# JakeKurtz/MC-Path-Tracer

Hardware: AMD Instinct MI355X
Metric: Mray/s (extend+shade) at 1080p x256spp depth5; fraction of HBM roofline (higher is better)
Workload: dtype f32

## Files before the change

include/mcpt.h:

```cpp
#ifndef MCPT_H
#define MCPT_H
#include <stdint.h>

#ifdef __cplusplus
extern "C" {
#endif

#define MCPT_ABI_VERSION 1

enum {
    MCPT_OK = 0,
    MCPT_E_INVALID = -1,
    MCPT_E_HIP = -2,
    MCPT_E_IO = -3,
    MCPT_E_NOMEM = -4,
    MCPT_E_NODEVICE = -5
};

typedef struct mcpt_config {
    uint64_t seed;
    int32_t spp;
    int32_t max_depth;
    int32_t rr_depth;
    int32_t tile_w;
// ... 71 lines not shown
    float *Ld;
    float *light_o, *light_d, *bvis_o, *bvis_d;
    uint8_t *queued;
} mcpt_path_view;

typedef struct mcpt_soa_view {
    const float *ray_o;
    const float *ray_d;
    float *hit_pos_t;
    float *hit_nrm_mat;
    int32_t *hit_tri;
    uint8_t *visible;
    uint32_t *steps;
    mcpt_path_view *paths;
} mcpt_soa_view;

typedef struct mcpt_ctx mcpt_ctx;
typedef struct mcpt_scene mcpt_scene;

int mcpt_create(int device, const mcpt_config *cfg, mcpt_ctx **out);
void mcpt_destroy(mcpt_ctx *ctx);
const char *mcpt_last_error(const mcpt_ctx *ctx);
int mcpt_scene_upload(mcpt_ctx *ctx, const mcpt_scene_desc *desc);
#define MCPT_GPU_BVH_LBVH 0
#define MCPT_GPU_BVH_PLOC 1
int mcpt_scene_upload_gpu_bvh(mcpt_ctx *ctx, const mcpt_scene_desc *desc);
int mcpt_set_gpu_bvh_builder(mcpt_ctx *ctx, int32_t builder);
int mcpt_camera_set(mcpt_ctx *ctx, const mcpt_camera *cam);
int mcpt_film_resize(mcpt_ctx *ctx, uint32_t w, uint32_t h, uint32_t tile_w, uint32_t tile_h);
int mcpt_film_clear(mcpt_ctx *ctx);
int mcpt_set_path_slots(mcpt_ctx *ctx, uint32_t slots);
int mcpt_set_trace_partitions(mcpt_ctx *ctx, uint32_t nparts);
int mcpt_set_work_counters(mcpt_ctx *ctx, int32_t on);
int mcpt_set_skip_discarded(mcpt_ctx *ctx, int32_t on);
int mcpt_set_tiles(mcpt_ctx *ctx, const uint32_t *tile_xy, uint32_t ntiles);
int mcpt_set_compact_paths(mcpt_ctx *ctx, int32_t on);
int mcpt_wavefront_step(mcpt_ctx *ctx, uint32_t tile_x, uint32_t tile_y, mcpt_stage_stats *st);
int mcpt_iterate(mcpt_ctx *ctx, uint32_t iterations, mcpt_stage_stats *st);
int mcpt_render(mcpt_ctx *ctx, mcpt_stage_stats *st);
int mcpt_stage_run(mcpt_ctx *ctx, int stage, const mcpt_soa_view *in, mcpt_soa_view *out, uint32_t n);
int mcpt_film_read(mcpt_ctx *ctx, float *Ld_rgb, uint32_t *samples);
int mcpt_film_read_device(mcpt_ctx *ctx, void *d_Ld_rgb, void *d_samples);
int mcpt_film_pack_tiles(mcpt_ctx *ctx, void *d_out, uint32_t *npix);
int mcpt_film_unpack_tiles(mcpt_ctx *ctx, const void *d_in, const uint32_t *tile_xy, uint32_t ntiles);
int mcpt_film_tonemap_rgba8(mcpt_ctx *ctx, float exposure, uint8_t *out);
int mcpt_film_size(const mcpt_ctx *ctx, uint32_t *w, uint32_t *h);
int mcpt_gather(mcpt_ctx *const *ctxs, int32_t n, int32_t root);
int mcpt_film_write_png(mcpt_ctx *ctx, float exposure, const char *path);
int mcpt_film_write_pfm(mcpt_ctx *ctx, const char *path);
int mcpt_image_write_png(const char *path, uint32_t w, uint32_t h, const uint8_t *rgba8);
int mcpt_image_write_pfm(const char *path, uint32_t w, uint32_t h, const float *rgb);
int mcpt_guides_render(mcpt_ctx *ctx, uint32_t nsamples);
int mcpt_guides_read(mcpt_ctx *ctx, float *albedo_rgb, float *normal_xyz, float *depth, uint32_t *count);
typedef struct mcpt_denoise_params {
    int32_t passes;
    float sigma_color;
    float sigma_normal, sigma_albedo, sigma_depth;
} mcpt_denoise_params;
int mcpt_denoise_default_params(mcpt_denoise_params *p);
int mcpt_denoise_run(mcpt_ctx *ctx, uint32_t w, uint32_t h, const float *rgb, const uint32_t *samples,
                     const float *albedo, const float *normal, const float *depth, const mcpt_denoise_params *p,
                     float *out_rgb);
int mcpt_film_denoise(mcpt_ctx *ctx, const mcpt_denoise_params *p);
int mcpt_denoised_read(mcpt_ctx *ctx, float *rgb);
int mcpt_denoised_read_device(mcpt_ctx *ctx, void *d_rgb);
int mcpt_denoised_tonemap_rgba8(mcpt_ctx *ctx, float exposure, uint8_t *out);
int mcpt_denoised_write_png(mcpt_ctx *ctx, float exposure, const char *path);
int mcpt_debug_denoise_ms(const mcpt_ctx *ctx, float *out10);
typedef struct mcpt_denoise_guided_params {
    int32_t passes;
    float sigma_lum;
    float lum_eps;
    float sigma_color;
    float sigma_normal, sigma_albedo, sigma_depth;
} mcpt_denoise_guided_params;
int mcpt_denoise_guided_default_params(mcpt_denoise_guided_params *p);
int mcpt_denoise_guided_run(mcpt_ctx *ctx, uint32_t w, uint32_t h, const float *rgb, const uint32_t *samples,
                            const float *variance, const float *albedo, const float *normal, const float *depth,
                            const mcpt_denoise_guided_params *p, float *out_rgb, float *out_variance);
int mcpt_film_denoise_guided(mcpt_ctx *ctx, const mcpt_denoise_guided_params *p);
int mcpt_denoised_variance_read(mcpt_ctx *ctx, float *var);
int mcpt_set_sample_budget(mcpt_ctx *ctx, const uint32_t *budget);
int mcpt_sample_budget_read(mcpt_ctx *ctx, uint32_t *out);
int mcpt_set_spp(mcpt_ctx *ctx, int32_t spp);
int mcpt_film_error(mcpt_ctx *ctx);
int mcpt_film_error_read(mcpt_ctx *ctx, float *out4);
int mcpt_error_run(mcpt_ctx *ctx, uint32_t w, uint32_t h, uint32_t slots, const float *Ld_slots,
                   const uint32_t *samples_slots, float *out4);
int mcpt_debug_film_read_slot(mcpt_ctx *ctx, uint32_t slot, float *Ld_rgb, uint32_t *samples);
typedef struct mcpt_sample_budget_params {
    float target_rel_err;
    float lum_floor;
    uint32_t min_spp, max_spp;
} mcpt_sample_budget_params;
int mcpt_sample_budget_default_params(mcpt_sample_budget_params *p);
int mcpt_budget_from_error(mcpt_ctx *ctx, const mcpt_sample_budget_params *p, uint64_t *out3);
int64_t mcpt_debug_adaptive_bytes(const mcpt_ctx *ctx);
int mcpt_debug_adaptive_ms(const mcpt_ctx *ctx, float *out2);
int mcpt_set_seed(mcpt_ctx *ctx, uint64_t seed);
int mcpt_camera_view_proj(const mcpt_camera *cam, float *out16);
typedef struct mcpt_temporal_params {
    float pos_tol;
    float nrm_tol;
    float max_history;
    float alpha_min;
} mcpt_temporal_params;
int mcpt_temporal_default_params(mcpt_temporal_params *p);
int mcpt_film_temporal(mcpt_ctx *ctx, const mcpt_temporal_params *p);
int mcpt_temporal_reset(mcpt_ctx *ctx);
int mcpt_temporal_read(mcpt_ctx *ctx, float *rgb, float *nsamples, float *variance, float *position);
int mcpt_temporal_denoise(mcpt_ctx *ctx, const mcpt_denoise_guided_params *p);
int mcpt_temporal_run(mcpt_ctx *ctx, uint32_t w, uint32_t h, const float *rgb, const uint32_t *samples,
                      const float *variance, const float *position, const float *normal, const float *depth,
                      const float *hcol, const float *hpos, const float *hnrm, const float *vp_prev16,
                      const mcpt_temporal_params *p, float *out_col, float *out_vl, float *out_hcol, float *out_hpos,
                      float *out_hnrm);
int64_t mcpt_debug_temporal_bytes(const mcpt_ctx *ctx);
int mcpt_debug_temporal_ms(const mcpt_ctx *ctx, float *out1);
typedef struct mcpt_variance_params {
    int32_t radius;
    float sigma_normal, sigma_albedo, sigma_depth;
    float min_neff;
} mcpt_variance_params;
int mcpt_variance_default_params(mcpt_variance_params *p);
int mcpt_variance_run(mcpt_ctx *ctx, uint32_t w, uint32_t h, const float *rgb, const uint32_t *samples,
                      const float *variance, const float *albedo, const float *normal, const float *depth,
                      const mcpt_variance_params *p, float *out_variance);
int mcpt_set_variance_fill(mcpt_ctx *ctx, const mcpt_variance_params *p);
int mcpt_debug_variance_ms(const mcpt_ctx *ctx, float *out1);
int mcpt_sync(mcpt_ctx *ctx);
int mcpt_device_name(mcpt_ctx *ctx, char *buf, int32_t len);
int mcpt_debug_queue_rays(mcpt_ctx *ctx, int which, float *ray_o, float *ray_d, uint32_t *n_inout);
float mcpt_debug_last_stage_ms(const mcpt_ctx *ctx);
int mcpt_debug_tiny_lds_stack(mcpt_ctx *ctx, int32_t on);
float mcpt_debug_last_build_ms(const mcpt_ctx *ctx);
float mcpt_debug_last_env_build_ms(const mcpt_ctx *ctx);
int mcpt_debug_env_tables(mcpt_ctx *ctx, float *marginal_y, float *conds_y, float *pdf, int32_t *flags);
int mcpt_debug_node_layout(const mcpt_ctx *ctx);
typedef struct mcpt_bvh_info {
    int32_t npairs;
    int32_t root_ref;
    int32_t depth;
    int32_t width;
    int32_t layout;
    int32_t ntri;
    int32_t tri_f4;
    int32_t gpu_built;
    int32_t rounds;
    float root_mn[3], root_mx[3];
    float cull_p;
} mcpt_bvh_info;
int mcpt_debug_bvh_read(mcpt_ctx *ctx, float *nodes, float *tris, mcpt_bvh_info *info);
int mcpt_debug_occ_stats(const mcpt_ctx *ctx, uint64_t *resolved, int32_t *enabled);
int mcpt_debug_ray_counts(const mcpt_ctx *ctx, uint64_t *out);
int mcpt_debug_primary_stats(const mcpt_ctx *ctx, double *out4);
int mcpt_debug_discard_stats(const mcpt_ctx *ctx, uint64_t *out4);
int mcpt_debug_trace_profile(mcpt_ctx *ctx, uint64_t *out12, int reset);
int mcpt_debug_shade_sections(mcpt_ctx *ctx, uint64_t *out, int n, int reset);
int mcpt_debug_quot(mcpt_ctx *ctx, const float *a, const float *b, uint32_t n, float *out);
int mcpt_debug_hbm_copy(mcpt_ctx *ctx, uint64_t bytes, uint32_t iters, double *gbps);

mcpt_scene *mcpt_scene_new(void);
void mcpt_scene_free(mcpt_scene *s);
int mcpt_scene_load_glb(mcpt_scene *s, const char *path, const float *xform16);
int mcpt_scene_add_mesh(mcpt_scene *s, int32_t ntri, const float *v0, const float *v1, const float *v2,
                        const float *n0, const float *n1, const float *n2, const float *base_rgb);
int mcpt_scene_set_env_hdr(mcpt_scene *s, const char *path, int32_t mode);
#define MCPT_ENV_DEVICE_TABLES 1
int mcpt_scene_set_env_hdr_ex(mcpt_scene *s, const char *path, int32_t mode, uint32_t flags);
int mcpt_scene_set_env_color(mcpt_scene *s, const float *rgb, float ls);
int mcpt_scene_add_dir_light(mcpt_scene *s, const float *dir, const float *rgb, float ls);
int mcpt_scene_transform(mcpt_scene *s, const float *xform16);
int mcpt_scene_make_proxy(mcpt_scene *s, int32_t config_id, const char *asset_dir);
int mcpt_scene_build(mcpt_scene *s, int32_t max_prims_in_node);
#define MCPT_BVH_REFERENCE 0
#define MCPT_BVH_SAH3 1
typedef struct mcpt_bvh_params {
    int32_t builder;
    int32_t max_prims;
    int32_t buckets;
    float trav_cost;
    float isect_cost;
} mcpt_bvh_params;
int mcpt_scene_build_ex(mcpt_scene *s, const mcpt_bvh_params *p);
int mcpt_scene_get_desc(const mcpt_scene *s, mcpt_scene_desc *out);
int mcpt_scene_bvh_depth(const mcpt_scene *s);
int mcpt_camera_make(const mcpt_camera_params *p, mcpt_camera *out);

#ifdef __cplusplus
}
#endif
#endif
```

mc-path-tracer_amd/csrc/kernels.hip:

```cpp
#include <hip/hip_runtime.h>
#include <stdint.h>
#include <stdlib.h>
#include <string.h>
#include <algorithm>

#include "device/mcpt_core.hpp"
#include "device/primary_beam.hpp"
#include "kernels.hpp"

using namespace mcpt;

namespace mcpt_dev {

template <int NQ>
__device__ inline void block_push(const bool (&want)[NQ], uint32_t* const (&counters)[NQ], uint32_t (&slot)[NQ],
                                  uint32_t (&total)[NQ]) {
    __shared__ uint32_t s_wave[NQ][kBlock / 64];
    __shared__ uint32_t s_base[NQ];
    __shared__ uint32_t s_tot[NQ];
    const int lane = threadIdx.x & 63, wave = threadIdx.x >> 6;
    uint32_t prefix[NQ];
#pragma unroll
    for (int q = 0; q < NQ; q++) {
        uint64_t m = __ballot(want[q]);
// ... 135 lines not shown
    float bx0 = nx ? mxx : mnx, bx1 = nx ? mnx : mxx;
    float by0 = ny ? mxy : mny, by1 = ny ? mny : mxy;
    float bz0 = nz ? mxz : mnz, bz1 = nz ? mnz : mxz;
    float tmin = (bx0 - o.x) * inv.x;
    float tmax = (bx1 - o.x) * inv.x;
    float tymin = (by0 - o.y) * inv.y;
    float tymax = (by1 - o.y) * inv.y;
    float tzmin = (bz0 - o.z) * inv.z;
    float tzmax = (bz1 - o.z) * inv.z;
    bool miss = (tmin > tymax) || (tymin > tmax);
    float a = (tymin > tmin) ? tymin : tmin;
    float b = (tymax < tmax) ? tymax : tmax;
    miss = miss || (a > tzmax) || (tzmin > b);
    t0 = (tzmin > a) ? tzmin : a;
    t1 = (tzmax < b) ? tzmax : b;
    return !miss;
}
constexpr float K_INF_F = __builtin_huge_valf();
#ifndef MCPT_OCC_LAYOUT
#define MCPT_OCC_LAYOUT 0
#endif
constexpr int kEnd = -1;

__device__ inline float cull_iota(const DevScene& sc, V3 d, V3 inv) {
    const float ax = __builtin_fabsf(inv.x), ay = __builtin_fabsf(inv.y), az = __builtin_fabsf(inv.z);
    if (!(ax < K_INF_F && ay < K_INF_F && az < K_INF_F)) return -K_INF_F;
    const float n2 = d.x * d.x + d.y * d.y + d.z * d.z;
    if (!sc.cull_ok || !(n2 <= kCullNormMax)) return -3.4028235e38f;
    const float io = __builtin_fmaxf(__builtin_fmaxf(ax, ay), az) * kCullSlackF;
    return io * sc.cull_p <= 1.f ? io : -io;
}
__device__ inline bool keep_box(float t0, float t1, float m, float cut, float& key) {
    key = t0 - __builtin_fabsf(m);
    return !(m >= 0.f && __builtin_fmaf(t1, kCullBehindF, m) < 0.f) && !(key > cut);
}

typedef float f2v __attribute__((ext_vector_type(2)));
__device__ inline void pair_slab(float4 qx, float4 qy, float4 qz, V3 o, V3 inv, float& t0a, float& t1a, float& t0b,
                                 float& t1b) {
    const f2v ox = {o.x, o.x}, oy = {o.y, o.y}, oz = {o.z, o.z};
    const f2v ix = {inv.x, inv.x}, iy = {inv.y, inv.y}, iz = {inv.z, inv.z};
    const f2v ax = (f2v{qx.x, qx.y} - ox) * ix, bx = (f2v{qx.z, qx.w} - ox) * ix;
    const f2v ay = (f2v{qy.x, qy.y} - oy) * iy, by = (f2v{qy.z, qy.w} - oy) * iy;
    const f2v az = (f2v{qz.x, qz.y} - oz) * iz, bz = (f2v{qz.z, qz.w} - oz) * iz;
    t0a = __builtin_fmaxf(__builtin_fmaxf(__builtin_fminf(ax.x, bx.x), __builtin_fminf(ay.x, by.x)),
                          __builtin_fminf(az.x, bz.x));
    t1a = __builtin_fminf(__builtin_fminf(__builtin_fmaxf(ax.x, bx.x), __builtin_fmaxf(ay.x, by.x)),
                          __builtin_fmaxf(az.x, bz.x));
    t0b = __builtin_fmaxf(__builtin_fmaxf(__builtin_fminf(ax.y, bx.y), __builtin_fminf(ay.y, by.y)),
                          __builtin_fminf(az.y, bz.y));
    t1b = __builtin_fminf(__builtin_fminf(__builtin_fmaxf(ax.y, bx.y), __builtin_fmaxf(ay.y, by.y)),
                          __builtin_fmaxf(az.y, bz.y));
}

__device__ inline void quad_axis(const float4& mn, const float4& mx, float o, float inv, float (&lo)[4],
                                 float (&hi)[4], bool first) {
    const f2v oo = {o, o}, ii = {inv, inv};
    const f2v a0 = (f2v{mn.x, mn.y} - oo) * ii, a1 = (f2v{mn.z, mn.w} - oo) * ii;
    const f2v b0 = (f2v{mx.x, mx.y} - oo) * ii, b1 = (f2v{mx.z, mx.w} - oo) * ii;
    const float l[4] = {__builtin_fminf(a0.x, b0.x), __builtin_fminf(a0.y, b0.y), __builtin_fminf(a1.x, b1.x),
                        __builtin_fminf(a1.y, b1.y)};
    const float h[4] = {__builtin_fmaxf(a0.x, b0.x), __builtin_fmaxf(a0.y, b0.y), __builtin_fmaxf(a1.x, b1.x),
                        __builtin_fmaxf(a1.y, b1.y)};
#pragma unroll
    for (int k = 0; k < 4; k++) {
        lo[k] = first ? l[k] : __builtin_fmaxf(lo[k], l[k]);
        hi[k] = first ? h[k] : __builtin_fminf(hi[k], h[k]);
    }
}

__device__ inline f2v pk_slab(f2v q, f2v p) {
    f2v r;
    __asm__("v_pk_add_f32 %0, %1, %2 op_sel_hi:[1,0] neg_lo:[0,1] neg_hi:[0,1]\n\t"
            "v_pk_mul_f32 %0, %0, %2 op_sel:[0,1] op_sel_hi:[1,1]"
            : "=&v"(r)
            : "v"(q), "v"(p));
    return r;
}
__device__ inline void box_t(float ax, float bx, float ay, float by, float az, float bz, float& t0, float& t1) {
    float m0, m1, m2, n0, n1, n2;
    __asm__("v_min_f32 %2, %8, %9\n\t"
            "v_min_f32 %3, %10, %11\n\t"
            "v_min_f32 %4, %12, %13\n\t"
            "v_max_f32 %5, %8, %9\n\t"
            "v_max_f32 %6, %10, %11\n\t"
            "v_max_f32 %7, %12, %13\n\t"
            "v_max3_f32 %0, %2, %3, %4\n\t"
            "v_min3_f32 %1, %5, %6, %7"
            : "=v"(t0), "=v"(t1), "=&v"(m0), "=&v"(m1), "=&v"(m2), "=&v"(n0), "=&v"(n1), "=&v"(n2)
            : "v"(ax), "v"(bx), "v"(ay), "v"(by), "v"(az), "v"(bz));
}
__device__ inline void pair_slab2(float4 qx, float4 qy, float4 qz, f2v px, f2v py, f2v pz, float& t0a, float& t1a,
                                  float& t0b, float& t1b) {
    const f2v ax = pk_slab(f2v{qx.x, qx.y}, px), bx = pk_slab(f2v{qx.z, qx.w}, px);
    const f2v ay = pk_slab(f2v{qy.x, qy.y}, py), by = pk_slab(f2v{qy.z, qy.w}, py);
    const f2v az = pk_slab(f2v{qz.x, qz.y}, pz), bz = pk_slab(f2v{qz.z, qz.w}, pz);
    box_t(ax.x, bx.x, ay.x, by.x, az.x, bz.x, t0a, t1a);
    box_t(ax.y, bx.y, ay.y, by.y, az.y, bz.y, t0b, t1b);
}
__device__ inline float vmin(float a, float b) {
    float r;
    __asm__("v_min_f32 %0, %1, %2" : "=v"(r) : "v"(a), "v"(b));
    return r;
}
__device__ inline float vmax(float a, float b) {
    float r;
    __asm__("v_max_f32 %0, %1, %2" : "=v"(r) : "v"(a), "v"(b));
    return r;
}
__device__ inline void quad_axis2(const float4& mn, const float4& mx, f2v p, float (&lo)[4], float (&hi)[4], bool first) {
    const f2v a0 = pk_slab(f2v{mn.x, mn.y}, p), a1 = pk_slab(f2v{mn.z, mn.w}, p);
    const f2v b0 = pk_slab(f2v{mx.x, mx.y}, p), b1 = pk_slab(f2v{mx.z, mx.w}, p);
    const float l[4] = {vmin(a0.x, b0.x), vmin(a0.y, b0.y), vmin(a1.x, b1.x), vmin(a1.y, b1.y)};
    const float h[4] = {vmax(a0.x, b0.x), vmax(a0.y, b0.y), vmax(a1.x, b1.x), vmax(a1.y, b1.y)};
#pragma unroll
    for (int k = 0; k < 4; k++) {
        lo[k] = first ? l[k] : vmax(lo[k], l[k]);
        hi[k] = first ? h[k] : vmin(hi[k], h[k]);
    }
}

__device__ inline bool ray_misses_scene(const DevScene& sc, V3 o, V3 d) {
    if (!(d.x == d.x && d.y == d.y && d.z == d.z) || (d.x == 0.f && d.y == 0.f && d.z == 0.f)) return true;
    if (o.x >= sc.root_mn[0] && o.x <= sc.root_mx[0] && o.y >= sc.root_mn[1] && o.y <= sc.root_mx[1] &&
        o.z >= sc.root_mn[2] && o.z <= sc.root_mx[2])
        return false;
    const V3 inv = v3(1.f / d.x, 1.f / d.y, 1.f / d.z);
    const float m = sc.root_w * cull_iota(sc, d, inv);
    float t0, t1, key;
    return !(slab(sc.root_mn[0], sc.root_mn[1], sc.root_mn[2], sc.root_mx[0], sc.root_mx[1], sc.root_mx[2], o, inv,
                  inv.x < 0.f, inv.y < 0.f, inv.z < 0.f, t0, t1) &&
             keep_box(t0, t1, m, K_INF_F, key));
}

__device__ inline void hit_record(const DevScene& sc, V3 o, V3 d, int tri, V3& pos, V3& nrm, int& mat, float& t_out) {
    const float4* tp = sc.tri + kTriF4 * tri;
    const float4 w0 = tp[0], w1 = tp[1], w2 = tp[2];
    const float4* sp4 = sc.tri_sh + 3 * tri;
    const float4 s0 = sp4[0], s1 = sp4[1], s2 = sp4[2];
    __asm__ volatile("" ::"v"(w0.x), "v"(w0.y), "v"(w0.z), "v"(w0.w), "v"(w1.x), "v"(w1.y), "v"(w1.z), "v"(w1.w),
                     "v"(w2.x), "v"(s0.x), "v"(s0.y), "v"(s0.z), "v"(s0.w), "v"(s1.x), "v"(s1.y), "v"(s1.z),
                     "v"(s1.w), "v"(s2.x), "v"(s2.y));
    float t, u, v;
    tri_test(o, d, v3(w0.x, w0.y, w0.z), v3(w0.w, w1.x, w1.y), v3(w1.z, w1.w, w2.x), t, u, v);
    const V3 n0 = v3(s0.x, s0.y, s0.z), n1 = v3(s0.w, s1.x, s1.y), n2 = v3(s1.z, s1.w, s2.x);
    const float w = (1.f - u) - v;
    nrm = normalize((n1 * u + n2 * v) + n0 * w);
    nrm = normalize(nrm);
    pos = o + d * t;
    mat = __float_as_int(s2.y);
    t_out = t;
}

__device__ inline uint32_t occ_index(const DevScene& sc, V3 o, V3 d) {
    const float gm = (float)(sc.occ_g - 1), bm = (float)(sc.occ_b - 1), hb = 0.5f * (float)sc.occ_b;
    const uint32_t cx = (uint32_t)__builtin_fminf(__builtin_fmaxf((o.x - sc.root_mn[0]) * sc.occ_inv[0], 0.f), gm);
    const uint32_t cy = (uint32_t)__builtin_fminf(__builtin_fmaxf((o.y - sc.root_mn[1]) * sc.occ_inv[1], 0.f), gm);
    const uint32_t cz = (uint32_t)__builtin_fminf(__builtin_fmaxf((o.z - sc.root_mn[2]) * sc.occ_inv[2], 0.f), gm);
    const float ax = __builtin_fabsf(d.x), ay = __builtin_fabsf(d.y), az = __builtin_fabsf(d.z);
    uint32_t face;
    float u, v, m;
    if (ax >= ay && ax >= az) {
        face = d.x < 0.f ? 1u : 0u; u = d.y; v = d.z; m = ax;
    } else if (ay >= az) {
        face = d.y < 0.f ? 3u : 2u; u = d.x; v = d.z; m = ay;
    } else {
        face = d.z < 0.f ? 5u : 4u; u = d.x; v = d.y; m = az;
    }
    const float r = hb * __builtin_amdgcn_rcpf(m);
    const uint32_t ub = (uint32_t)__builtin_fminf(__builtin_fmaxf(u * r + hb, 0.f), bm);
    const uint32_t vb = (uint32_t)__builtin_fminf(__builtin_fmaxf(v * r + hb, 0.f), bm);
    const uint32_t G = (uint32_t)sc.occ_g, B = (uint32_t)sc.occ_b;
#if MCPT_OCC_LAYOUT == 1
    return (((face * B + ub) * B + vb) * G + cz) * G * G + cy * G + cx;
#else
    return ((((cz * G + cy) * G + cx) * 6u + face) * B + ub) * B + vb;
#endif
}

__device__ inline bool occ_test(V3 o, V3 d, V3 inv, float io, float4 bmn, float4 bmx, float4 r2, float4 r3) {
    const float ax = (bmn.x - o.x) * inv.x, bx = (bmx.x - o.x) * inv.x;
    const float ay = (bmn.y - o.y) * inv.y, by = (bmx.y - o.y) * inv.y;
    const float az = (bmn.z - o.z) * inv.z, bz = (bmx.z - o.z) * inv.z;
    const float t0 = __builtin_fmaxf(__builtin_fmaxf(__builtin_fminf(ax, bx), __builtin_fminf(ay, by)),
                                     __builtin_fminf(az, bz));
    const float t1 = __builtin_fminf(__builtin_fminf(__builtin_fmaxf(ax, bx), __builtin_fmaxf(ay, by)),
                                     __builtin_fmaxf(az, bz));
    float key;
    if (!(t0 <= t1) || !keep_box(t0, t1, bmn.w * io, K_INF_F, key)) return false;
    float th;
    return tri_test_t(o, d, v3(bmx.w, r2.x, r2.y), v3(r2.z, r2.w, r3.x), v3(r3.y, r3.z, r3.w), th) && !(th < 0.f) &&
           th < K_HUGE;
}
__device__ inline uint2 occ_entry(const DevScene& sc, uint32_t cell) {
    const uint2* e = reinterpret_cast<const uint2*>(sc.occ) + cell;
    if constexpr (MCPT_NT & 16) {
        typedef uint32_t u2v_t __attribute__((ext_vector_type(2)));
        const u2v_t v = __builtin_nontemporal_load(reinterpret_cast<const u2v_t*>(e));
        return make_uint2(v.x, v.y);
    } else {
        return *e;
    }
}
__device__ inline bool occ_hit1(const DevScene& sc, V3 o, V3 d, uint2 e) {
    const bool v0 = e.x < sc.ntri, v1 = e.y < sc.ntri;
    if (!(v0 || v1)) return false;
    const float4* p0 = sc.occ_rec + kOccRecF4 * (size_t)(v0 ? e.x : 0u);
    const float4* p1 = sc.occ_rec + kOccRecF4 * (size_t)(v1 ? e.y : 0u);
    const float4 bn0 = p0[0], bx0 = p0[1], r20 = p0[2], r30 = p0[3];
    const float4 bn1 = p1[0], bx1 = p1[1], r21 = p1[2], r31 = p1[3];
    const V3 inv = v3(1.f / d.x, 1.f / d.y, 1.f / d.z);
    if (!(__builtin_fabsf(inv.x) < K_INF_F && __builtin_fabsf(inv.y) < K_INF_F && __builtin_fabsf(inv.z) < K_INF_F))
        return false;
    const float io = cull_iota(sc, d, inv);
    return (v0 && occ_test(o, d, inv, io, bn0, bx0, r20, r30)) || (v1 && occ_test(o, d, inv, io, bn1, bx1, r21, r31));
}

struct MatOut {
    bool want_ext, want_l, want_b, trivial_ext, vis_ray, need_cb;
    bool skip_ext;
    bool doomed_inplace;
    uint32_t trivial_any;
    uint2 el, eb;
    V3 n, wo, wi_b;
    int matid, light_id;
    uint32_t flags;
    float rrz;
};

template <bool FIXED>
__device__ inline MatOut material(const ShadeArgs& a, uint32_t pid, uint32_t pix, uint32_t sidx, uint32_t len,
                                 V3 beta_store, int32_t htri, float4* stage, bool occ_on, bool no_cont) {
    const DevScene& sc = a.scene;
    const uint2 none = make_uint2(kOccEmpty, kOccEmpty);
    MatOut mo{};
    mo.el = mo.eb = none;
    MCPT_MARK("m_hit");
    const Rng r{rng_key(a.seed, pix, sidx), len};
    const V3 ro = xyz(ld_s(a.p.ray_o + pid)), rdir = xyz(ld_s(a.p.ray_d + pid));
    V3 pos, n;
    int mat;
    float t_hit;
    hit_record(sc, ro, rdir, htri, pos, n, mat, t_hit);
    const V3 wo = -rdir;
    const Mat m = load_mat(sc.mats + 8 * mat);
    uint32_t nf = 0;
    V3 rr;
    if (no_cont) {
        rr = v3(0.f, 0.f, 0.f);
        st_s(a.p.beta + pid, f4(beta_store, 0.f));
        mo.skip_ext = true;
    } else {
        MCPT_MARK("m_cont");
        V3 wi_s = brdf_sample_wi<FIXED>(m, n, wo, r, SL_CONT_E0, r(SL_CONT_LOBE) < 0.5f);
        float pdf_s;
        V3 f_s;
        brdf_f_pdf(m, n, wi_s, wo, f_s, pdf_s);
        if ((f_s.x == 0.f && f_s.y == 0.f && f_s.z == 0.f) || pdf_s == 0.f) nf |= F_FZERO;
        rr = f_s / pdf_s;
        const V3 new_o = pos + n * 0.001f;
        st_s(a.p.beta + pid, f4(beta_store, rr.x));
        bool doomed = false;
        if (FIXED || !a.skip) {
            doomed = len + 1u > (uint32_t)a.max_depth;
            if (!doomed && len + 1u > (uint32_t)a.rr_depth) {
                const Rng r1{r.key, len + 1u};
                float q;
                doomed = rr_terminates(r1, FIXED ? (beta_store * rr).y : beta_store.y, q);
            }
        }
        if (doomed && a.skip) {
            mo.skip_ext = true;
        } else {
            st_s(a.p.ray_o + pid, f4(new_o, 0.f));
            st_s(a.p.ray_d + pid, f4(wi_s, 0.f));
            mo.want_ext = true;
            if (ray_misses_scene(sc, new_o, wi_s)) {
                a.p.hit_tri[pid] = -1;
                mo.want_ext = false;
                mo.trivial_ext = true;
                mo.doomed_inplace = doomed;
            }
        }
    }
    MCPT_MARK("m_light");
    int l_id = (int)(r(SL_LIGHT) * (float)(sc.nlights - 0) + (float)0);
    const int light_id = (l_id == sc.nlights) ? 0 : l_id;
    const bool delta = light_id > 0;
    const float sel = FIXED ? 1.f / (float)sc.nlights : 1.f;
    {
        V3 ldir, Li_l;
        float pdfl_x;
        const float4* lt = sc.env.ltab[FIXED ? 1 : 0];
        if (light_id == 0 && lt) {
            int cx, cy;
            env_cell<FIXED>(sc.env, r, cx, cy);
            const float4 t0 = lt[(int64_t)cy * (sc.env.w + 1) + cx + 1];
            const float2 rs = sc.env.lrow[FIXED ? 1 : 0][cy], cs = sc.env.lcol[FIXED ? 1 : 0][cx + 1];
            ldir = v3(cs.y * rs.x, rs.y, cs.x * rs.x);
            pdfl_x = t0.w;
            Li_l = xyz(t0);
        } else {
            if (light_id == 0) ldir = env_dir<FIXED>(sc.env, r);
            else ldir = ld3(sc.dirs + 7 * (light_id - 1), 0);
            light_L_pdf<FIXED>(sc, light_id, ldir, Li_l, pdfl_x);
        }
        V3 f_l;
        float pdf_bl;
        brdf_f_pdf(m, n, ldir, wo, f_l, pdf_bl);
        if (FIXED) pdfl_x = pdfl_x * sel;
        float pdfb_y = !delta ? pdf_bl : (FIXED ? 0.f : 1.f);
        float wL = power_heuristic(pdfl_x, pdfb_y);
        V3 cL = ((f_l * Li_l) * wL) / pdfl_x;
        if (wL > 0.f && pdfl_x > 0.f) nf |= F_CONDL;
        st_s(a.p.nee0 + pid, f4(cL, rr.y));
        const V3 so_l = pos + n * 0.01f;
        if (ray_misses_scene(sc, so_l, ldir)) {
            a.p.vis[2 * pid] = 1;
            mo.trivial_any++;
        } else {
            stage[0 * kBlock + threadIdx.x] = f4(so_l, __uint_as_float(2 * pid));
            stage[1 * kBlock + threadIdx.x] = f4(ldir, 0.f);
            mo.want_l = true;
            if (occ_on) mo.el = occ_entry(sc, occ_index(sc, so_l, ldir));
        }
    }
    MCPT_MARK("m_bsdir");
    if (!delta) {
        const V3 wi_b = brdf_sample_wi<FIXED>(m, n, wo, r, SL_MAT_E0, r(SL_MAT_LOBE) < 0.5f);
        const V3 so_b = pos + wi_b * 0.001f;
        nf |= F_HASVIS;
        mo.vis_ray = true;
        mo.need_cb = true;
        mo.wi_b = wi_b;
        if (ray_misses_scene(sc, so_b, wi_b)) {
            a.p.vis[2 * pid + 1] = 1;
            mo.trivial_any++;
        } else {
            if (occ_on) mo.eb = occ_entry(sc, occ_index(sc, so_b, wi_b));
            stage[2 * kBlock + threadIdx.x] = f4(so_b, __uint_as_float(2 * pid + 1));
            stage[3 * kBlock + threadIdx.x] = f4(wi_b, 0.f);
            mo.want_b = true;
        }
    }
    MCPT_MARK("m_ret");
    mo.n = n;
    mo.wo = wo;
    mo.matid = mat;
    mo.light_id = light_id;
    mo.rrz = rr.z;
    mo.flags = nf | ((len + 1) << F_LEN_SHIFT) | (sidx << F_SIDX_SHIFT);
    return mo;
}
template <bool FIXED>
__device__ inline void material_brdf_terms(const ShadeArgs& a, uint32_t pid, const MatOut& mo) {
    const DevScene& sc = a.scene;
    V3 cB = v3(0.f, 0.f, 0.f);
    uint32_t nf = mo.flags;
    if (mo.need_cb) {
        const Mat m = load_mat(sc.mats + 8 * mo.matid);
        V3 f_b;
        float pdfb_x;
        brdf_f_pdf(m, mo.n, mo.wi_b, mo.wo, f_b, pdfb_x);
        V3 Li_b;
        float pdfl_y;
        light_L_pdf<FIXED>(sc, mo.light_id, mo.wi_b, Li_b, pdfl_y);
        if (FIXED) pdfl_y = pdfl_y * (1.f / (float)sc.nlights);
        float wB = power_heuristic(pdfb_x, pdfl_y);
        cB = ((f_b * Li_b) * wB) / pdfb_x;
        if (wB > 0.f && pdfb_x > 0.f) nf |= F_CONDB;
    }
    st_s(a.p.nee1 + pid, f4(cB, mo.rrz));
    st_s(a.p.flags + pid, nf);
}

#ifndef MCPT_SHADE_WPE
#define MCPT_SHADE_WPE 8
#endif
#if MCPT_SHADE_WPE > 0
#define MCPT_SHADE_ATTR __attribute__((amdgpu_waves_per_eu(MCPT_SHADE_WPE, MCPT_SHADE_WPE)))
#else
#define MCPT_SHADE_ATTR
#endif
#ifndef MCPT_MAT_WPE
#define MCPT_MAT_WPE 4
#endif
#ifdef MCPT_MAT_WPE
#define MCPT_MAT_ATTR __attribute__((amdgpu_waves_per_eu(MCPT_MAT_WPE, MCPT_MAT_WPE)))
#else
#define MCPT_MAT_ATTR
#endif
struct VBlk { int x0, y0; uint32_t loc0, sr, li0, done; };
__device__ inline VBlk vblock_of(const ShadeArgs& a, int vb) {
    const int tile_px = a.tile_w * a.tile_h;
    const int bpt = (tile_px + kBlock - 1) / kBlock;
    const int per_slot = a.ntiles * bpt;
    const int slot = a.slots > 1 ? vb / per_slot : 0;
    const int bs = vb - slot * per_slot;
    const int tile = bs / bpt;
    const int bib = bs - tile * bpt;
    const int li0 = bib * kBlock;
    const int2 t = a.tiles[tile];
    VBlk r;
    if (a.tile_w % kBlock == 0) {
        const int row = li0 / a.tile_w;
        r.x0 = t.x * a.tile_w + (li0 - row * a.tile_w);
        r.y0 = t.y * a.tile_h + row;
    } else {
        r.x0 = t.x * a.tile_w;
        r.y0 = t.y * a.tile_h;
    }
    r.loc0 = a.compact ? (uint32_t)(a.tile_base ? a.tile_base[tile] : tile) * (uint32_t)tile_px + (uint32_t)li0 : 0u;
    r.sr = (uint32_t)slot | ((uint32_t)min(tile_px - li0, kBlock) << 8);
    r.li0 = (uint32_t)li0;
    const uint32_t ntx = (uint32_t)((a.W + a.tile_w - 1) / a.tile_w), nty = (uint32_t)((a.H + a.tile_h - 1) / a.tile_h);
    r.done = (((uint32_t)slot * nty + (uint32_t)t.y) * ntx + (uint32_t)t.x) * (uint32_t)bpt + (uint32_t)bib;
    return r;
}
__device__ inline uint32_t udiv_small(uint32_t n, uint32_t d, float rcp) {
    uint32_t q = (uint32_t)((float)n * rcp);
    if (n - __umul24(q, d) >= d) q++;
    return q;
}

template <bool FIXED, bool MAP>
__device__ __attribute__((always_inline)) inline void shade_vblock(const ShadeArgs& a, int vb, const VBlk& v) {
    const DevScene& sc = a.scene;
    const int slot = (int)(v.sr & 0xffu);
    const int lane = threadIdx.x & 63;
    bool valid = (int)threadIdx.x < (int)(v.sr >> 8);
    uint32_t pid = 0, pix = 0;
    int x = 0, y = 0;
    if (valid) {
        if (a.tile_w % kBlock == 0) {
            x = v.x0 + (int)threadIdx.x;
            y = v.y0;
        } else {
            const int li = (int)v.li0 + (int)threadIdx.x;
            x = v.x0 + li % a.tile_w;
            y = v.y0 + li / a.tile_w;
        }
        valid = x < a.W - 1 && y < a.H - 1;
        pix = (uint32_t)y * (uint32_t)a.W + (uint32_t)x;
        pid = (uint32_t)slot * a.npx + (a.compact ? v.loc0 + threadIdx.x : pix);
    }
    MCPT_MARK("load");
    bool gen_ext = false, gen_trivial = false, gen_prim = false, prim_res = false, cont = false;
    bool no_cont = false;
    bool dd = false, dd_vis = false;
    bool d_logic = false, d_nee = false, d_gen = false;
    (void)d_logic; (void)d_nee; (void)d_gen;
    uint32_t cont_len = 0, cont_sidx = 0;
    int32_t cont_htri = -1;
    V3 beta_store = v3(0.f, 0.f, 0.f);
    bool bg = false;
    V3 bg_film = v3(0.f, 0.f, 0.f), bg_dir = bg_film;
    bool finished = true;
    if (valid) {
        const uint32_t fl = ld_s(a.p.flags + pid);
        const int32_t htri = ld_s(a.p.hit_tri + pid);
        const float4 b4 = ld_s(a.p.beta + ((((fl >> F_LEN_SHIFT) & 0xffu) > 1u) ? pid : 0u));
        const uint32_t len = (fl >> F_LEN_SHIFT) & 0xffu;
        const bool need_rd = len == 1 && htri < 0;
        const bool need_nee = len <= (uint32_t)a.max_depth && len > 1;
        const bool need_ld = !(fl & F_DEAD) && (need_rd || need_nee);
        const V3 ld4 = ld3f4(a.p.Ld + (need_ld ? pid : 0u));
        const V3 rd = ld3f4(a.p.ray_d + (need_rd ? pid : 0u));
        const float4 n0 = ld_s(a.p.nee0 + (need_nee ? pid : 0u)), n1 = ld_s(a.p.nee1 + (need_nee ? pid : 0u));
        const uchar2 vv = reinterpret_cast<const uchar2*>(a.p.vis)[need_nee ? pid : 0u];
        bool dead = (fl & F_DEAD) != 0;
        uint32_t spp;
        if constexpr (MAP) spp = a.budget[pix];
        else spp = (uint32_t)a.spp;
        uint32_t sidx = fl >> F_SIDX_SHIFT;
        uint32_t samples = a.slots > 1 ? udiv_small(sidx - (uint32_t)slot, (uint32_t)a.slots, a.slots_rcp) : sidx;
        if (!dead && sidx < spp) {
            MCPT_MARK("logic");
            d_logic = true;
            d_nee = need_nee;
            const Rng r{rng_key(a.seed, pix, sidx), len};
            const bool found = htri >= 0;
            const V3 B = len == 1 ? v3(1.f, 1.f, 1.f) : xyz(b4);
            V3 film = ld4;
            bool terminate = false;
            beta_store = B;
            if (len == 1) {
                if (found) {
                    film = film + v3(0.f, 0.f, 0.f) * B;
                } else {
                    bg = true;
                    bg_film = film;
                    bg_dir = rd;
// ... 30 lines not shown
                            __float_as_uint(film.y) != __float_as_uint(ld4.y) ||
                            __float_as_uint(film.z) != __float_as_uint(ld4.z)))
                st_s(a.p.Ld + pid, f4(film, 0.f));
            if (a.skip && !terminate) {
                if (len + 1u > (uint32_t)a.max_depth) {
                    int l_id = (int)(r(SL_LIGHT) * (float)(sc.nlights - 0) + (float)0);
                    dd = true;
                    dd_vis = !(((l_id == sc.nlights) ? 0 : l_id) > 0);
                    terminate = true;
                } else if (!FIXED && len + 1u > (uint32_t)a.rr_depth) {
                    const Rng r1{r.key, len + 1u};
                    float q;
                    no_cont = rr_terminates(r1, beta_store.y, q);
                }
            }
            if (terminate) {
                dead = true;
                samples++;
                sidx += (uint32_t)a.slots;
                st_s(a.p.samples + pid, samples);
            } else {
                cont = true;
                cont_len = len;
                cont_sidx = sidx;
                cont_htri = htri;
            }
        }
        uint32_t nflags = fl;
        if (dead) nflags = F_DEAD | (sidx << F_SIDX_SHIFT);
        if (dead && sidx < spp) {
            MCPT_MARK("generate");
            d_gen = true;
            V3 new_o = ld3f4(a.cam_px + pix), new_d;
            if (a.cam.lens_radius > 0.f) {
                const Rng r0{rng_key(a.seed, pix, sidx), 0u};
                gen_ray_lens(a.cam, new_o, r0, new_o, new_d);
            } else {
                new_d = ld3f4(a.cam_dir + pix);
            }
            nflags = (1u << F_LEN_SHIFT) | (sidx << F_SIDX_SHIFT);
            st_s(a.p.ray_o + pid, f4(new_o, 0.f));
            st_s(a.p.ray_d + pid, f4(new_d, 0.f));
            gen_ext = true;
            if (ray_misses_scene(sc, new_o, new_d)) {
                a.p.hit_tri[pid] = -1;
                gen_ext = false;
                gen_trivial = true;
            } else if (a.prim_cnt) {
                const uint32_t pc = a.prim_cnt[pix];
                if (pc != 0u && __builtin_fminf(__builtin_fminf(__builtin_fabsf(new_d.x), __builtin_fabsf(new_d.y)),
                                                __builtin_fabsf(new_d.z)) >= 1e-30f) {
                    gen_ext = false;
                    prim_res = true;
                    if (pc == 1u) {
                        a.p.hit_tri[pid] = -1;
                        gen_trivial = true;
                    } else {
                        gen_prim = true;
                    }
                }
            }
        }
        MCPT_MARK("flags");
        if (!cont && nflags != fl) st_s(a.p.flags + pid, nflags);
        finished = dead && !(sidx < spp);
    }
    SHADE_DIAG(SD_WAVES, true);
    SHADE_DIAG(SD_VALID, valid);
    SHADE_DIAG(SD_LOGIC, d_logic);
    SHADE_DIAG(SD_NEE, d_nee);
    SHADE_DIAG(SD_GEN, d_gen);
    SHADE_DIAG(SD_CONT, cont);
    SHADE_DIAG(SD_BG, bg);
    MCPT_MARK("push");
    const int shard = vb % kShards;
    uint32_t* sc_ctr = a.cnt->shard[shard];
    {
        bool want[3] = {gen_ext, cont, gen_prim};
        uint32_t* ctr[3] = {sc_ctr + C_EXT, sc_ctr + C_MAT, sc_ctr + C_PRIM};
        uint32_t slot[3], total[3];
        block_push<3>(want, ctr, slot, total);
        if (gen_ext) st_q(a.ext_q + shard * a.ext_cap + slot[0], pid);
        if (gen_prim) a.prim_q[shard * a.ext_cap + slot[2]] = make_uint2(pid, pix);
        if (cont) {
            const uint32_t qi = shard * a.ext_cap + slot[1];
            st_s(a.mat_rec + qi, make_uint4(pid, pix, cont_sidx | (no_cont ? kRecNoCont : 0u) | (cont_len << kRecLenShift),
                                            (uint32_t)cont_htri));
            st_s(a.mat_beta + qi, f4(beta_store, 0.f));
        }
    }
    uint32_t n_ext = ((gen_ext || gen_trivial || gen_prim) ? 1u : 0u) + (dd ? 1u : 0u);
    for (int off = 32; off > 0; off >>= 1) n_ext += __shfl_xor(n_ext, off);
    if (lane == 0 && n_ext) atomicAdd(sc_ctr + C_EXT_RAYS, n_ext);
    if (a.skip) {
        const uint32_t n_dd = (uint32_t)__popcll(__ballot(dd)), n_ddv = (uint32_t)__popcll(__ballot(dd_vis));
        if (lane == 0 && n_dd) {
            atomicAdd(sc_ctr + C_ANY_RAYS, n_dd + n_ddv);
            if (n_ddv) atomicAdd(sc_ctr + C_VIS, n_ddv);
            atomicAdd(sc_ctr + C_SKIP_EXT, n_dd);
            atomicAdd(sc_ctr + C_SKIP_ANY, n_dd + n_ddv);
            atomicAdd(sc_ctr + C_SKIP_MAT, n_dd);
        }
    }
    if (a.prim_cnt) {
        const uint32_t n_prim = (uint32_t)__popcll(__ballot(prim_res));
        if (lane == 0 && n_prim) atomicAdd(sc_ctr + C_PRIM_RAYS, n_prim);
    }
    MCPT_MARK("background");
    if (bg) {
        const int nbg = FIXED ? 1 : sc.nlights;
        V3 film = bg_film;
        for (int i = 0; i < nbg; i++) film = film + env_L(sc.env, bg_dir) * v3(1.f, 1.f, 1.f);
        if (__float_as_uint(film.x) != __float_as_uint(bg_film.x) || __float_as_uint(film.y) != __float_as_uint(bg_film.y) ||
            __float_as_uint(film.z) != __float_as_uint(bg_film.z))
            a.p.Ld[pid] = f4(film, 0.f);
    }
    MCPT_MARK("done");
    if (a.blk_done && __syncthreads_and(finished ? 1 : 0) && threadIdx.x == 0) a.blk_done[v.done] = 1;
    MCPT_MARK("end");
}

template <bool FIXED, bool MAP>
__global__ __launch_bounds__(kBlock) MCPT_SHADE_ATTR void k_shade(ShadeArgs a) {
    if (a.cnt->idle) return;
    __shared__ uint64_t s_live[kBlock / 64];
    const uint32_t G = gridDim.x, nvb = a.shade_vblocks;
    const uint32_t mine = (nvb - blockIdx.x + G - 1) / G;
    const uint32_t k = threadIdx.x;
    bool live = false;
    __shared__ VBlk s_vb[kBlock];
    if (k < mine) {
        const VBlk v = vblock_of(a, (int)(blockIdx.x + k * G));
        live = !a.blk_done || a.blk_done[v.done] == 0;
        s_vb[k] = v;
    }
    const uint64_t m = __ballot(live);
    if ((threadIdx.x & 63) == 0) s_live[threadIdx.x >> 6] = m;
    __syncthreads();
    for (uint32_t j = 0; j < mine; j++) {
        if (!((s_live[j >> 6] >> (j & 63)) & 1ull)) continue;
        shade_vblock<FIXED, MAP>(kernarg_fresh<ShadeArgs>(), (int)(blockIdx.x + j * G), s_vb[j]);
    }
}

template <bool FIXED>
__global__ __launch_bounds__(kBlock) MCPT_MAT_ATTR void k_material(ShadeArgs a_kernarg) {
    (void)a_kernarg;
    const ShadeArgs& a = kernarg_fresh<ShadeArgs>();
    if (a.cnt->idle) return;
    const uint32_t shard = blockIdx.x % kShards, w_in = blockIdx.x / kShards, bps = gridDim.x / kShards;
    uint32_t* sc_ctr = a.cnt->shard[shard];
    const uint32_t n = sc_ctr[C_MAT];
    const int lane = threadIdx.x & 63;
    uint32_t n_ext = 0, n_any = 0, n_vis = 0, n_occ = 0, occ_try = 0, n_skip = 0, n_inpl = 0;
    const bool occ_on = a.scene.occ && a.scene.occ_gate[0] == 0 && a.scene.occ_gate[2] != 0;
    __shared__ float4 s_any[4][kBlock];
    for (uint32_t base = w_in * kBlock; base < n; base += bps * kBlock) {
        const ShadeArgs& a = kernarg_fresh<ShadeArgs>();
        const uint32_t i = base + threadIdx.x;
        MatOut mo{};
        uint32_t mpid = 0;
        bool occ_l = false, occ_b = false, try_l = false, try_b = false;
        if (i < n) {
            const uint4 q = ld_s(a.mat_rec + shard * a.ext_cap + i);
            const float4 b4 = ld_s(a.mat_beta + shard * a.ext_cap + i);
            mpid = q.x;
            mo = material<FIXED>(a, mpid, q.y, q.z & (kRecNoCont - 1u), q.z >> kRecLenShift, xyz(b4), (int32_t)q.w,
                                 &s_any[0][0], occ_on, (q.z & kRecNoCont) != 0u);
            MCPT_MARK("m_occ");
            if (occ_on) {
                try_l = mo.want_l;
                try_b = mo.want_b;
                const V3 ol = xyz(s_any[0][threadIdx.x]), dl = xyz(s_any[1][threadIdx.x]);
                const V3 ob = xyz(s_any[2][threadIdx.x]), db = xyz(s_any[3][threadIdx.x]);
                if (mo.want_l) occ_l = occ_hit1(a.scene, ol, dl, mo.el);
                if (mo.want_b) occ_b = occ_hit1(a.scene, ob, db, mo.eb);
                if (occ_l) {
                    a.p.vis[2 * mpid] = 0;
                    mo.want_l = false;
                    mo.trivial_any++;
                }
                if (occ_b) {
                    a.p.vis[2 * mpid + 1] = 0;
                    mo.want_b = false;
                    mo.need_cb = false;
                    mo.trivial_any++;
                }
            }
            MCPT_MARK("m_bterms");
            material_brdf_terms<FIXED>(a, mpid, mo);
        }
        MCPT_MARK("m_push");
        bool want[3] = {mo.want_ext, mo.want_l, mo.want_b};
        uint32_t* ctr[3] = {sc_ctr + C_EXT, sc_ctr + C_ANY, sc_ctr + C_ANY};
        uint32_t slot[3], total[3];
        block_push<3>(want, ctr, slot, total);
        if (mo.want_ext) st_q(a.ext_q + shard * a.ext_cap + slot[0], mpid);
        if (mo.want_l) {
            const uint32_t k = shard * a.any_cap + slot[1];
            if constexpr (MCPT_NT & 8) {
                st_s(a.p.sray_o + k, s_any[0][threadIdx.x]);
                st_s(a.p.sray_d + k, s_any[1][threadIdx.x]);
            } else {
                a.p.sray_o[k] = s_any[0][threadIdx.x];
                a.p.sray_d[k] = s_any[1][threadIdx.x];
            }
        }
        if (mo.want_b) {
            const uint32_t k = shard * a.any_cap + slot[2];
            if constexpr (MCPT_NT & 8) {
                st_s(a.p.sray_o + k, s_any[2][threadIdx.x]);
                st_s(a.p.sray_d + k, s_any[3][threadIdx.x]);
            } else {
                a.p.sray_o[k] = s_any[2][threadIdx.x];
                a.p.sray_d[k] = s_any[3][threadIdx.x];
            }
        }
        MCPT_MARK("m_count");
        n_occ += (uint32_t)(__popcll(__ballot(occ_l)) + __popcll(__ballot(occ_b)));
        occ_try += (uint32_t)(__popcll(__ballot(try_l)) + __popcll(__ballot(try_b)));
        n_ext += (uint32_t)__popcll(__ballot(mo.want_ext || mo.trivial_ext || mo.skip_ext));
        n_skip += (uint32_t)__popcll(__ballot(mo.skip_ext));
        n_inpl += (uint32_t)__popcll(__ballot(mo.doomed_inplace));
        n_any += (uint32_t)(__popcll(__ballot(mo.want_l)) + __popcll(__ballot(mo.want_b)) +
                            __popcll(__ballot(mo.trivial_any >= 1u)) + __popcll(__ballot(mo.trivial_any >= 2u)));
        n_vis += (uint32_t)__popcll(__ballot(mo.vis_ray));
    }
    if (lane == 0) {
        if (n_ext) atomicAdd(sc_ctr + C_EXT_RAYS, n_ext);
        if (n_any) atomicAdd(sc_ctr + C_ANY_RAYS, n_any);
        if (n_vis) atomicAdd(sc_ctr + C_VIS, n_vis);
        if (n_occ) atomicAdd(sc_ctr + C_OCC, n_occ);
        if (occ_try) atomicAdd(sc_ctr + C_OCC_TRY, occ_try);
        if (n_skip) atomicAdd(sc_ctr + C_SKIP_EXT, n_skip);
        if (n_inpl) atomicAdd(sc_ctr + C_SKIP_INPLACE, n_inpl);
    }
}

__device__ inline uint32_t wave_scan_incl(uint32_t x) {
    x += (uint32_t)__builtin_amdgcn_update_dpp(0, (int)x, 0x111, 0xf, 0xf, false);
    x += (uint32_t)__builtin_amdgcn_update_dpp(0, (int)x, 0x112, 0xf, 0xf, false);
    x += (uint32_t)__builtin_amdgcn_update_dpp(0, (int)x, 0x114, 0xf, 0xf, false);
    x += (uint32_t)__builtin_amdgcn_update_dpp(0, (int)x, 0x118, 0xf, 0xf, false);
    x += (uint32_t)__builtin_amdgcn_update_dpp(0, (int)x, 0x142, 0xa, 0xf, false);
    x += (uint32_t)__builtin_amdgcn_update_dpp(0, (int)x, 0x143, 0xc, 0xf, false);
    return x;
}

__device__ inline void wave_stats(uint32_t* stats, int lane, uint32_t nodes, uint32_t tests, uint32_t hits) {
    if (!stats) return;
    for (int off = 32; off > 0; off >>= 1) {
        nodes += __shfl_xor(nodes, off);
        tests += __shfl_xor(tests, off);
        hits += __shfl_xor(hits, off);
    }
    if (lane == 0) {
        uint32_t* st = stats + (blockIdx.x % kShards) * C_WORDS;
        atomicAdd(st + 0, nodes);
        atomicAdd(st + 1, tests);
        atomicAdd(st + 2, hits);
    }
}

#ifndef MCPT_NODE_STEPS
#define MCPT_NODE_STEPS 4
#endif
#ifndef MCPT_TRI_SHARE
#define MCPT_TRI_SHARE 0
#endif
constexpr int kShareMaxStack = 8;
constexpr int kNodeSteps = MCPT_NODE_STEPS;
#ifndef MCPT_GRAB_MAX
#define MCPT_GRAB_MAX 0
#endif
constexpr int kGrabMax = MCPT_GRAB_MAX;
#ifndef MCPT_ANY_FIRST
#define MCPT_ANY_FIRST 0
#endif
constexpr bool kAnyFirst = MCPT_ANY_FIRST != 0;
#ifndef MCPT_NODE_MIN_LANES2
#define MCPT_NODE_MIN_LANES2 32
#endif
#ifndef MCPT_NODE_MIN_LANES2_DEEP
#define MCPT_NODE_MIN_LANES2_DEEP 0
#endif
#ifndef MCPT_NODE_MIN_LANES4
#define MCPT_NODE_MIN_LANES4 24
#endif

#ifndef MCPT_TRACE_WPE
#define MCPT_TRACE_WPE 7
#endif
#ifndef MCPT_TRACE_WPE_DEEP
#define MCPT_TRACE_WPE_DEEP 7
#endif
#ifndef MCPT_TRACE_WPE4
#define MCPT_TRACE_WPE4 6
#endif
#define MCPT_TRACE_WPE_OF(kW, kS) \
    ((kW) == 4 ? MCPT_TRACE_WPE4 : ((kS) > ::mcpt_dev::kLdsStack ? MCPT_TRACE_WPE_DEEP : MCPT_TRACE_WPE))
#define MCPT_TRACE_ATTR \
    __attribute__((amdgpu_waves_per_eu(MCPT_TRACE_WPE_OF(kW, kLdsStack), MCPT_TRACE_WPE_OF(kW, kLdsStack))))
template <int kW, int kLdsStack, bool kCount>
__global__ __launch_bounds__(kTraceBlock) MCPT_TRACE_ATTR void k_trace(TraceArgs a) {
    if (a.idle && *a.idle) return;
    constexpr bool kShare = MCPT_TRI_SHARE != 0 && kLdsStack <= kShareMaxStack;
    __shared__ int2 stk[kLdsStack][kTraceBlock];
    __shared__ uint64_t s_key[kShare ? kTraceBlock : 1];
    const int lane = threadIdx.x;
    const uint32_t nsh = (uint32_t)a.nshards, nparts = a.nparts;
    uint32_t home = 0;
    if (nparts > 1) {
        uint32_t xcc;
        __asm__ volatile("s_getreg_b32 %0, hwreg(HW_REG_XCC_ID)" : "=s"(xcc));
        const uint32_t nd = a.ndies >= 1 && a.ndies <= nparts && nparts % a.ndies == 0 ? a.ndies : nparts;
        home = (xcc & 15u) % nd + nd * ((blockIdx.x / nd) % (nparts / nd));
    }
    __shared__ uint32_t s_tot[kMaxParts];
    if (lane < kMaxParts) s_tot[lane] = 0;
    __syncthreads();
    if ((uint32_t)lane < nsh) {
        uint32_t n = 0;
#pragma unroll
        for (int k = 0; k < 2; k++) {
            const TraceSet& ts = a.set[k];
            n += ts.count_ptr ? ts.count_ptr[lane * C_WORDS] : (lane == 0 ? ts.count : 0u);
        }
        if (n) atomicAdd(&s_tot[lane % nparts], n);
    }
    __syncthreads();
    __shared__ uint32_t s_pre[129];
    uint32_t part = home, spart = 0, T = 0;
    uint32_t* grab = a.grab;
    bool more = false;
    auto enter = [&](uint32_t p) {
        part = __builtin_amdgcn_readfirstlane(p);
        spart = __builtin_amdgcn_readfirstlane(nsh > part ? (nsh - part + nparts - 1) / nparts : 0u);
        uint32_t base = 0;
#pragma unroll 1
        for (uint32_t h = 0; h < 2; h++) {
            const uint32_t e = (uint32_t)lane + 64u * h;
            const bool k1 = kAnyFirst ? e < spart : e >= spart;
            const uint32_t j = e >= spart ? e - spart : e;
            uint32_t ne = 0;
            if (e < 2 * spart) {
                const TraceSet& ts = k1 ? a.set[1] : a.set[0];
                const uint32_t sh = part + j * nparts;
                ne = ts.count_ptr ? ts.count_ptr[sh * C_WORDS] : (sh == 0 ? ts.count : 0u);
            }
            const uint32_t inc = wave_scan_incl(ne);
            s_pre[e] = base + inc - ne;
            base += __builtin_amdgcn_readlane(inc, 63);
        }
        T = __builtin_amdgcn_readfirstlane(base);
        if (lane == 0) s_pre[128] = T;
        __syncthreads();
        grab = a.grab + part * C_WORDS;
        more = T > 0;
    };
    enter(home);
    const DevScene& sc = a.scene;
    const bool occ_rec = sc.occ && sc.occ_gate[0] <= 1u;

    uint32_t tot_n = 0, tot_t = 0, tot_h = 0, tot_n1 = 0, tot_t1 = 0, tot_h1 = 0;
    uint32_t ph[kPhaseWords] = {};
    uint64_t drained = 0;
    for (;;) {
    uint32_t buf_lo = 0, buf_hi = 0, last_p = 0;
    bool act = false;
    uint32_t rid = 0;
    f2v px = {0.f, 0.f}, py = px, pz = px;
    V3 d = v3(0.f, 0.f, 0.f);
#define RAY_O v3(px.x, py.x, pz.x)
#define RAY_INV v3(px.y, py.y, pz.y)
    int ref = kEnd, leaf = kEnd, sp = 0, tri = -1;
    float best = K_HUGE, cut = K_HUGE, io = K_INF_F;
    uint32_t bsid = 0;
    int2 spill[kMaxStack - kLdsStack];
    auto pop = [&]() -> int {
        while (sp > 0) {
            sp--;
            int2 e;
            if (sp < kLdsStack) {
                e = stk[sp][lane];
            } else {
                e = spill[sp - kLdsStack];
// ... 529 lines not shown
__global__ void k_cam_table(mcpt::CamView cam, int W, int H, float4* px, float4* dir) {
    const uint32_t i = blockIdx.x * blockDim.x + threadIdx.x;
    if (i >= (uint32_t)W * (uint32_t)H) return;
    const int x = (int)(i % (uint32_t)W), y = (int)(i / (uint32_t)W);
    V3 o, d;
    gen_ray_pixel(cam, W, H, x, y, o, d);
    px[i] = f4(cam.lens_radius > 0.f ? gen_ray_focal(cam, o, d) : o, 0.f);
    dir[i] = f4(d, 0.f);
}
void launch_cam_table(const mcpt::CamView& cam, int W, int H, float4* px, float4* dir, hipStream_t s) {
    const uint32_t n = (uint32_t)W * (uint32_t)H;
    if (n) hipLaunchKernelGGL(k_cam_table, dim3((n + 255) / 256), dim3(256), 0, s, cam, W, H, px, dir);
}

__global__ void k_env_pack(float4* tex, const float* __restrict__ pdf, size_t n) {
    const size_t i = (size_t)blockIdx.x * blockDim.x + threadIdx.x;
    if (i < n) tex[i].w = pdf[i];
}
void launch_env_pack(float4* tex, const float* pdf, size_t n, hipStream_t s) {
    if (n) hipLaunchKernelGGL(k_env_pack, dim3((unsigned)((n + 255) / 256)), dim3(256), 0, s, tex, pdf, n);
}

template <bool FIXED>
__global__ void k_env_table(EnvView e, float4* out, float2* row, float2* col) {
    const int i = blockIdx.x * blockDim.x + threadIdx.x;
    const int W1 = e.w + 1;
    if (i < e.h) {
        float st, ct;
        spherical_theta(env_cell_v<FIXED>(e, i), st, ct);
        row[i] = make_float2(st, ct);
    }
    if (i < W1) {
        const int x = i - 1;
        float sp, cp;
        spherical_phi(env_cell_u<FIXED>(e, FIXED && x < 0 ? 0 : x), sp, cp);
        col[i] = make_float2(sp, cp);
    }
    if (i >= W1 * e.h) return;
    const int y = i / W1, x = i - y * W1 - 1;
    const V3 d = env_cell_dir<FIXED>(e, FIXED && x < 0 ? 0 : x, y);
    V3 L;
    float pdf;
    env_L_pdf<FIXED>(e, d, L, pdf);
    out[i] = make_float4(L.x, L.y, L.z, pdf);
}
void launch_env_table(const EnvView& e, bool fixed_mode, float4* out, float2* row, float2* col, hipStream_t s) {
    const int n = (e.w + 1) * e.h;
    if (fixed_mode) hipLaunchKernelGGL(k_env_table<true>, dim3((n + 255) / 256), dim3(256), 0, s, e, out, row, col);
    else hipLaunchKernelGGL(k_env_table<false>, dim3((n + 255) / 256), dim3(256), 0, s, e, out, row, col);
}

__global__ void k_hit_record(HitRecordArgs a) {
    const uint32_t i = blockIdx.x * blockDim.x + threadIdx.x;
    if (i >= a.n) return;
    const int tri = a.tri[i];
    if (tri < 0) {
        a.hit_p[i] = make_float4(0.f, 0.f, 0.f, K_HUGE);
        a.hit_n[i] = make_float4(0.f, 0.f, 0.f, __int_as_float(-1));
        a.scene_tri[i] = -1;
        return;
    }
    a.scene_tri[i] = __float_as_int(a.scene.tri[kTriF4 * tri + 2].y);
    V3 pos, nrm;
    int mat;
    float t;
    hit_record(a.scene, xyz(a.ro[i]), xyz(a.rd[i]), tri, pos, nrm, mat, t);
    a.hit_p[i] = make_float4(pos.x, pos.y, pos.z, t);
    a.hit_n[i] = make_float4(nrm.x, nrm.y, nrm.z, __int_as_float(mat));
}

__global__ void k_clear(ClearArgs a) {
    const uint32_t i = blockIdx.x * blockDim.x + threadIdx.x;
    if (i >= a.n) return;
    a.flags[i] = F_DEAD | ((i / a.npx) << F_SIDX_SHIFT);
    a.samples[i] = 0;
    a.Ld[i] = make_float4(0.f, 0.f, 0.f, 0.f);
}

__global__ void k_resolve(ResolveArgs a) {
    const uint32_t i = blockIdx.x * blockDim.x + threadIdx.x;
    if (i >= a.n) return;
    uint32_t o = i;
    if (a.tiles) {
        const uint32_t tpx = (uint32_t)(a.tile_w * a.tile_h), ti = i / tpx, li = i - ti * tpx;
        const int2 t = a.tiles[ti];
        const uint32_t x = (uint32_t)t.x * a.tile_w + li % (uint32_t)a.tile_w, y = (uint32_t)t.y * a.tile_h + li / (uint32_t)a.tile_w;
        if (x >= (uint32_t)a.W || y >= (uint32_t)a.H) return;
        o = y * (uint32_t)a.W + x;
    }
    float4 L = a.Ld[i];
    uint32_t n = a.samples[i];
    for (int k = 1; k < a.slots; k++) {
        const float4 l = a.Ld[(size_t)k * a.n + i];
        L = make_float4(L.x + l.x, L.y + l.y, L.z + l.z, 0.f);
        n += a.samples[(size_t)k * a.n + i];
    }
    a.out_Ld[o] = L;
    a.out_samples[o] = n;
}

__global__ void k_tonemap(TonemapArgs a) {
    const uint32_t i = blockIdx.x * blockDim.x + threadIdx.x;
    if (i >= a.n) return;
    float4 L = a.Ld[i];
    float s = (float)a.samples[i];
    V3 c = v3(L.x / s, L.y / s, L.z / s);
    c = c * a.exposure;
    c = v3(c.x / (c.x + 1.0f), c.y / (c.y + 1.0f), c.z / (c.z + 1.0f));
    float cc[3] = {255 * c.x, 255 * c.y, 255 * c.z};
    uchar4 o;
    unsigned char b[3];
    for (int k = 0; k < 3; k++) {
        float v = cc[k];
        b[k] = (v == v && v >= 0.f && v < 4294967296.f) ? (unsigned char)(unsigned int)v : (unsigned char)0;
    }
    o.x = b[0]; o.y = b[1]; o.z = b[2]; o.w = 255;
    a.out[i] = o;
}

#ifndef MCPT_OCC_BACKOFF0
#define MCPT_OCC_BACKOFF0 15
#endif
__global__ void k_accumulate(CounterBlock* c, uint32_t nparts, uint32_t* occ_gate) {
    if (c->idle) return;
    const int t = threadIdx.x;
    uint32_t v[C_STATS + 6];
#pragma unroll
    for (int k = 0; k < C_STATS + 6; k++) {
        v[k] = c->shard[t][k];
        c->shard[t][k] = 0;
    }
    c->last_ext_shard[t] = v[C_EXT];
    __shared__ uint32_t s_part[kMaxParts];
    if (t < kMaxParts) s_part[t] = 0;
    __syncthreads();
    atomicAdd(&s_part[t % nparts], v[C_EXT] + v[C_ANY]);
    __syncthreads();
    uint32_t g = 0;
    if (t < kMaxParts) g = c->grab[t][0];
    const bool short_part = t < (int)nparts && g < s_part[t];
#pragma unroll
    for (int k = 0; k < C_STATS + 6; k++)
        for (int off = 32; off > 0; off >>= 1) v[k] += __shfl_xor(v[k], off);
    if (__ballot(short_part) != 0 && t == 0) c->trace_short += 1;
    if (t < kMaxParts) c->grab[t][0] = 0;
    uint32_t phw[kPhaseWords];
#pragma unroll
    for (int k = 0; k < kPhaseWords; k++) {
        phw[k] = c->shard[t][C_PH + k];
        c->shard[t][C_PH + k] = 0;
        for (int off = 32; off > 0; off >>= 1) phw[k] += __shfl_xor(phw[k], off);
    }
    uint32_t er = c->shard[t][C_EXT_RAYS], ar = c->shard[t][C_ANY_RAYS], oc = c->shard[t][C_OCC],
             ot = c->shard[t][C_OCC_TRY], pr = c->shard[t][C_PRIM_RAYS];
    const int skw[4] = {C_SKIP_EXT, C_SKIP_ANY, C_SKIP_MAT, C_SKIP_INPLACE};
    uint32_t sk[4];
#pragma unroll
    for (int k = 0; k < 4; k++) {
        sk[k] = c->shard[t][skw[k]];
        if (sk[k]) c->shard[t][skw[k]] = 0;
        for (int off = 32; off > 0; off >>= 1) sk[k] += __shfl_xor(sk[k], off);
    }
    c->shard[t][C_PRIM] = 0;
    c->shard[t][C_PRIM_RAYS] = 0;
    c->shard[t][C_EXT_RAYS] = 0;
    c->shard[t][C_ANY_RAYS] = 0;
    c->shard[t][C_MAT] = 0;
    c->shard[t][C_OCC] = 0;
    c->shard[t][C_OCC_TRY] = 0;
    for (int off = 32; off > 0; off >>= 1) {
        er += __shfl_xor(er, off);
        ar += __shfl_xor(ar, off);
        oc += __shfl_xor(oc, off);
        ot += __shfl_xor(ot, off);
        pr += __shfl_xor(pr, off);
    }
    if (t == 0) {
        c->tot_ext += er;
        c->tot_prim += pr;
        for (int k = 0; k < 4; k++) c->tot_skip[k] += sk[k];
        c->tot_any += ar;
        c->tot_occ += oc;
        if (occ_gate) {
            if (occ_gate[0]) {
                occ_gate[0]--;
            } else if (!occ_gate[2]) {
                if (v[C_ANY]) occ_gate[2] = 1;
            } else if (ot >= 4096u) {
                if ((unsigned long long)oc * kOccMinRate < ot) {
                    occ_gate[1] = occ_gate[1] ? min(2u * occ_gate[1] + 1u, 255u) : (uint32_t)MCPT_OCC_BACKOFF0;
                    occ_gate[0] = occ_gate[1];
                } else {
                    occ_gate[1] = 0;
                }
            }
        }
        c->tot_vis += v[C_VIS];
        c->tot_ext_q += v[C_EXT];
        c->tot_any_q += v[C_ANY];
        c->last_ext = v[C_EXT];
        c->last_live = er;
        if (er == 0) c->idle = 1;
        for (int k = 0; k < 6; k++) c->tot_stats[k] += v[C_STATS + k];
        for (int k = 0; k < kPhaseWords; k++) c->tot_phase[k] += phw[k];
    }
}

__global__ void k_pack(PackArgs a) {
    const int tile_px = a.tile_w * a.tile_h;
    const uint32_t i = blockIdx.x * blockDim.x + threadIdx.x;
    if (i >= (uint32_t)(a.ntiles * tile_px)) return;
    const int tile = i / tile_px, li = i % tile_px;
    int2 t = a.tiles[tile];
    int x = t.x * a.tile_w + li % a.tile_w, y = t.y * a.tile_h + li / a.tile_w;
    float4 o = make_float4(0.f, 0.f, 0.f, __uint_as_float(0u));
    if (x < a.W && y < a.H) {
        uint32_t pid = (uint32_t)y * a.W + x;
        float4 L = a.Ld[pid];
        o = make_float4(L.x, L.y, L.z, __uint_as_float(a.samples[pid]));
    }
    a.out[i] = o;
}

__global__ void k_unpack(UnpackArgs a) {
    const int tile_px = a.tile_w * a.tile_h;
    const uint32_t i = blockIdx.x * blockDim.x + threadIdx.x;
    if (i >= (uint32_t)(a.ntiles * tile_px)) return;
    const int tile = i / tile_px, li = i % tile_px;
    const int2 t = a.tiles[tile];
    const int x = t.x * a.tile_w + li % a.tile_w, y = t.y * a.tile_h + li / a.tile_w;
    if (x >= a.W || y >= a.H) return;
    const uint32_t pid = (uint32_t)y * a.W + x;
    const float4 v = a.in[i];
    a.Ld[pid] = make_float4(v.x, v.y, v.z, 0.f);
    a.samples[pid] = __float_as_uint(v.w);
}

static uint32_t env_u32(const char* name, int def, int lo, int hi) {
    const char* e = getenv(name);
    int v = e ? atoi(e) : def;
    return (uint32_t)std::min(hi, std::max(lo, v));
}
int launch_geometry(int dev, LaunchGeom& g) {
    int cus = 0, nx = 1, per_cu = 0, mat0 = 0, mat1 = 0, sh0 = 0;
    if (hipDeviceGetAttribute(&cus, hipDeviceAttributeMultiprocessorCount, dev) != hipSuccess) return -1;
    if (hipDeviceGetAttribute(&nx, hipDeviceAttributeNumberOfXccs, dev) != hipSuccess) nx = 1;
    int occ[2][2] = {};
    if (hipOccupancyMaxActiveBlocksPerMultiprocessor(&occ[0][0], k_trace<2, kLdsStack, false>, kTraceBlock, 0) != hipSuccess ||
        hipOccupancyMaxActiveBlocksPerMultiprocessor(&occ[0][1], k_trace<2, kLdsStackDeep, false>, kTraceBlock, 0) != hipSuccess ||
        hipOccupancyMaxActiveBlocksPerMultiprocessor(&occ[1][0], k_trace<4, kLdsStack, false>, kTraceBlock, 0) != hipSuccess ||
        hipOccupancyMaxActiveBlocksPerMultiprocessor(&occ[1][1], k_trace<4, kLdsStackDeep, false>, kTraceBlock, 0) != hipSuccess ||
        hipOccupancyMaxActiveBlocksPerMultiprocessor(&mat0, k_material<false>, kBlock, 0) != hipSuccess ||
        hipOccupancyMaxActiveBlocksPerMultiprocessor(&mat1, k_material<true>, kBlock, 0) != hipSuccess ||
        hipOccupancyMaxActiveBlocksPerMultiprocessor(&sh0, k_shade<false, false>, kBlock, 0) != hipSuccess)
        return -1;
    if (cus <= 0) cus = 256;
    per_cu = 32;
    if (const char* e = getenv("MCPT_TRACE_WAVES")) per_cu = atoi(e);
    if (per_cu <= 0) per_cu = 16;
    for (int w = 0; w < 2; w++)
        for (int k = 0; k < 2; k++) g.trace_waves[w][k] = (uint32_t)(cus * std::max(1, std::min(per_cu, occ[w][k])));
    g.ndies = (uint32_t)std::max(1, nx);
    g.trace_parts = env_u32("MCPT_TRACE_PARTS", std::min(kMaxParts, 2 * std::max(1, nx)), 1, kMaxParts);
    if (const char* e = getenv("MCPT_MAT_BLOCKS_PER_CU")) {
        const int m = atoi(e);
        if (m > 0) { mat0 = std::min(mat0, m); mat1 = std::min(mat1, m); }
    }
    g.mat_blocks[0] = (uint32_t)std::max(1, cus * std::max(1, mat0) / kShards) * (uint32_t)kShards;
    g.mat_blocks[1] = (uint32_t)std::max(1, cus * std::max(1, mat1) / kShards) * (uint32_t)kShards;
    int prim = 0;
    if (hipOccupancyMaxActiveBlocksPerMultiprocessor(&prim, k_primary, kBlock, 0) != hipSuccess) return -1;
    g.prim_blocks = (uint32_t)std::max(1, cus * std::max(1, prim) / kShards) * (uint32_t)kShards;
    g.shade_grid = (uint32_t)std::max(1, cus * std::max(1, sh0)) * env_u32("MCPT_SHADE_GRID", 16, 0, 1024);
    if (getenv("MCPT_SHADE_WGS")) g.shade_grid = env_u32("MCPT_SHADE_WGS", 0, 1, 1 << 30);
    g.refill_min = env_u32("MCPT_REFILL_MIN", 0, 0, 64);
    g.tri_min = env_u32("MCPT_TRI_MIN", 16, 0, 64);
    return 0;
}
static uint32_t shade_grid(uint32_t nblocks, const LaunchGeom& g) {
    uint32_t G = g.shade_grid ? std::min(nblocks, g.shade_grid) : nblocks;
    return std::max(G, (nblocks + kBlock - 1) / kBlock);
}
void launch_shade(const ShadeArgs& args, int nblocks, const LaunchGeom& g, bool fixed_mode, hipStream_t s) {
    ShadeArgs a = args;
    a.shade_vblocks = (uint32_t)nblocks;
    const uint32_t G = shade_grid((uint32_t)nblocks, g);
    if (fixed_mode) {
        if (a.budget) hipLaunchKernelGGL((k_shade<true, true>), dim3(G), dim3(kBlock), 0, s, a);
        else hipLaunchKernelGGL((k_shade<true, false>), dim3(G), dim3(kBlock), 0, s, a);
        hipLaunchKernelGGL(k_material<true>, dim3(g.mat_blocks[1]), dim3(kBlock), 0, s, a);
    } else {
        if (a.budget) hipLaunchKernelGGL((k_shade<false, true>), dim3(G), dim3(kBlock), 0, s, a);
        else hipLaunchKernelGGL((k_shade<false, false>), dim3(G), dim3(kBlock), 0, s, a);
        hipLaunchKernelGGL(k_material<false>, dim3(g.mat_blocks[0]), dim3(kBlock), 0, s, a);
    }
}
void launch_shade_stage(bool material_stage, const ShadeArgs& args, int nblocks, const LaunchGeom& g, bool fixed_mode,
                        hipStream_t s) {
    ShadeArgs a = args;
    a.shade_vblocks = (uint32_t)nblocks;
    if (!material_stage) {
        const uint32_t G = shade_grid((uint32_t)nblocks, g);
        if (fixed_mode) hipLaunchKernelGGL((k_shade<true, false>), dim3(G), dim3(kBlock), 0, s, a);
        else hipLaunchKernelGGL((k_shade<false, false>), dim3(G), dim3(kBlock), 0, s, a);
    } else {
        if (fixed_mode) hipLaunchKernelGGL(k_material<true>, dim3(g.mat_blocks[1]), dim3(kBlock), 0, s, a);
        else hipLaunchKernelGGL(k_material<false>, dim3(g.mat_blocks[0]), dim3(kBlock), 0, s, a);
    }
}
void launch_trace(const TraceArgs& args, const LaunchGeom& g, hipStream_t s) {
    if (args.nshards <= 0) return;
    TraceArgs a = args;
    a.tri_min = g.tri_min;
    a.nparts = std::min<uint32_t>(kMaxParts, std::max<uint32_t>(1, g.trace_parts));
    a.ndies = g.ndies;
    const uint32_t nsh = (uint32_t)a.nshards;
    const int w = a.scene.width == 4 ? 1 : 0, k = a.scene.depth > kDeepTree ? 1 : 0;
    static const uint32_t kRefill[2][2] = {{20u, 32u}, {24u, 24u}};
    a.refill_min = g.refill_min ? g.refill_min : kRefill[w][k];
    const uint32_t wps = std::max<uint32_t>(1, g.trace_waves[w][k] / nsh);
    const dim3 grid(wps * nsh), block(kTraceBlock);
    if (a.tiny_stack) {
        if (w == 0) hipLaunchKernelGGL((k_trace<2, kLdsStackTiny, false>), grid, block, 0, s, a);
        else hipLaunchKernelGGL((k_trace<4, kLdsStackTiny, false>), grid, block, 0, s, a);
        return;
    }
    if (a.set[0].stats || a.set[1].stats) {
        if (w == 0 && k == 0) hipLaunchKernelGGL((k_trace<2, kLdsStack, true>), grid, block, 0, s, a);
        else if (w == 0) hipLaunchKernelGGL((k_trace<2, kLdsStackDeep, true>), grid, block, 0, s, a);
        else if (k == 0) hipLaunchKernelGGL((k_trace<4, kLdsStack, true>), grid, block, 0, s, a);
        else hipLaunchKernelGGL((k_trace<4, kLdsStackDeep, true>), grid, block, 0, s, a);
        return;
    }
    if (w == 0 && k == 0) hipLaunchKernelGGL((k_trace<2, kLdsStack, false>), grid, block, 0, s, a);
    else if (w == 0) hipLaunchKernelGGL((k_trace<2, kLdsStackDeep, false>), grid, block, 0, s, a);
    else if (k == 0) hipLaunchKernelGGL((k_trace<4, kLdsStack, false>), grid, block, 0, s, a);
    else hipLaunchKernelGGL((k_trace<4, kLdsStackDeep, false>), grid, block, 0, s, a);
}
__global__ void k_quot(const float* a, const float* b, float* out, uint32_t n) {
    const uint32_t i = blockIdx.x * blockDim.x + threadIdx.x;
    if (i >= n) return;
    float q0, q1, q2;
    quot3(a[i], 1.0f, -a[i], b[i], q0, q1, q2);
    out[i] = q0;
}
void launch_quot(const float* a, const float* b, float* out, uint32_t n, hipStream_t s) {
    if (n) hipLaunchKernelGGL(k_quot, dim3((n + 255) / 256), dim3(256), 0, s, a, b, out, n);
}

__global__ __launch_bounds__(256) void k_copy(const float4* __restrict__ src, float4* __restrict__ dst, size_t n) {
    const size_t i = (size_t)blockIdx.x * blockDim.x + threadIdx.x;
    if (i < n) dst[i] = src[i];
}
void launch_copy(const float4* src, float4* dst, size_t n, hipStream_t s) {
    if (n) hipLaunchKernelGGL(k_copy, dim3((unsigned)((n + 255) / 256)), dim3(256), 0, s, src, dst, n);
}

int wave_times(unsigned long long* out, int n) {
    (void)out;
    (void)n;
    return 0;
}
int trace_profile(unsigned long long* out, int reset) {
    (void)out;
    (void)reset;
    return 0;
}
__global__ void k_occ_records(DevScene sc, uint32_t nnodes, float4* out) {
    const uint32_t i = blockIdx.x * blockDim.x + threadIdx.x;
    auto put = [&](int ref, float mnx, float mny, float mnz, float mxx, float mxy, float mxz, float w) {
        if (ref >= 0 || ref == kEnd) return;
        const uint32_t off = (uint32_t)ref & 0xffffffu, cnt = (((uint32_t)ref >> 24) & 7u) + 1u;
        for (uint32_t k = off; k < off + cnt && k < sc.ntri; k++) {
            const float4* tr = sc.tri + kTriF4 * (size_t)k;
            const float4 a = tr[0], b = tr[1], c = tr[2];
            float4* o = out + kOccRecF4 * (size_t)k;
            o[0] = make_float4(mnx, mny, mnz, w);
            o[1] = make_float4(mxx, mxy, mxz, a.x);
            o[2] = make_float4(a.y, a.z, a.w, b.x);
            o[3] = make_float4(b.y, b.z, b.w, c.x);
        }
    };
    if (i == 0 && sc.root_ref < 0)
        put(sc.root_ref, sc.root_mn[0], sc.root_mn[1], sc.root_mn[2], sc.root_mx[0], sc.root_mx[1], sc.root_mx[2],
            sc.root_w);
    if (i >= nnodes) return;
    if (sc.width == 4) {
        const float4* nd = sc.nodes + 8 * (size_t)i;
        const float4 mnx = nd[0], mxx = nd[1], mny = nd[2], mxy = nd[3], mnz = nd[4], mxz = nd[5], rf = nd[6], wq = nd[7];
        const float* a0 = &mnx.x; const float* a1 = &mxx.x; const float* b0 = &mny.x;
        const float* b1 = &mxy.x; const float* c0 = &mnz.x; const float* c1 = &mxz.x; const float* r = &rf.x;
        const float* w = &wq.x;
        for (int k = 0; k < 4; k++) put(__float_as_int(r[k]), a0[k], b0[k], c0[k], a1[k], b1[k], c1[k], w[k]);
    } else {
        const float4* nd = sc.nodes + 4 * (size_t)i;
        const float4 q0 = nd[0], q1 = nd[1], q2 = nd[2], q3 = nd[3];
        put(__float_as_int(q3.x), q0.x, q1.x, q2.x, q0.z, q1.z, q2.z, q3.z);
        put(__float_as_int(q3.y), q0.y, q1.y, q2.y, q0.w, q1.w, q2.w, q3.w);
    }
}

__global__ void k_cull_tri(const float4* tri, uint32_t ntri, float* tw, uint32_t* pmax, int plane) {
    const uint32_t i = blockIdx.x * blockDim.x + threadIdx.x;
    if (i >= ntri) return;
    const float4* r = tri + kTriF4 * (size_t)i;
    const float4 r0 = r[0], r1 = r[1], r2 = r[2];
    double far;
    tw[i] = cull_to_float_up(cull_tri_margin(v3(r0.w, r1.x, r1.y), v3(r1.z, r1.w, r2.x), &far, plane != 0));
    if (far > 0.0) atomicMax(pmax, __float_as_uint(cull_to_float_up(far)));
}
__global__ void k_cull_pairs(float4* nodes, uint32_t npairs, const float* tw, uint32_t ntri) {
    const uint32_t i = blockIdx.x * blockDim.x + threadIdx.x;
    if (i >= npairs) return;
    const float4 q3 = nodes[4 * (size_t)i + 3];
    float w[2];
#pragma unroll
    for (int k = 0; k < 2; k++) {
        const int ref = __float_as_int(k ? q3.y : q3.x);
        float v = 0.f;
        if (ref >= 0) {
            const float4 c = nodes[4 * (size_t)ref + 3];
            v = __builtin_fmaxf(c.z, c.w);
        } else if (ref != kEnd) {
            const uint32_t off = (uint32_t)ref & 0xffffffu, cnt = (((uint32_t)ref >> 24) & 7u) + 1u;
            for (uint32_t t = off; t < off + cnt && t < ntri; t++) v = __builtin_fmaxf(v, tw[t]);
        }
        w[k] = v;
    }
    nodes[4 * (size_t)i + 3] = make_float4(q3.x, q3.y, w[0], w[1]);
}
__global__ void k_cull_zero(float4* nodes, uint32_t npairs) {
    const uint32_t i = blockIdx.x * blockDim.x + threadIdx.x;
    if (i >= npairs) return;
    float4 q3 = nodes[4 * (size_t)i + 3];
    q3.z = q3.w = 0.f;
    nodes[4 * (size_t)i + 3] = q3;
}
void launch_cull_margins(float4* nodes, uint32_t npairs, const float4* tri, uint32_t ntri, float* tri_w,
                         uint32_t* pmax, int passes, bool plane, hipStream_t s) {
    if (ntri) hipLaunchKernelGGL(k_cull_tri, dim3((ntri + 255) / 256), dim3(256), 0, s, tri, ntri, tri_w, pmax, plane ? 1 : 0);
    if (!npairs) return;
    hipLaunchKernelGGL(k_cull_zero, dim3((npairs + 255) / 256), dim3(256), 0, s, nodes, npairs);
    for (int p = 0; p < passes; p++)
        hipLaunchKernelGGL(k_cull_pairs, dim3((npairs + 255) / 256), dim3(256), 0, s, nodes, npairs, tri_w, ntri);
}
__global__ void k_occ_probes(DevScene sc, float4* ro, float4* rd, uint32_t nkeys) {
    const uint32_t key = blockIdx.x * blockDim.x + threadIdx.x;
    if (key >= nkeys) return;
    const uint32_t G = (uint32_t)sc.occ_g, B = (uint32_t)sc.occ_b;
    uint32_t t = key, cx, cy, cz, face, ub, vb;
#if MCPT_OCC_LAYOUT == 1
    cx = t % G; t /= G; cy = t % G; t /= G; cz = t % G; t /= G; vb = t % B; t /= B; ub = t % B; face = t / B;
#else
    vb = t % B; t /= B; ub = t % B; t /= B; face = t % 6u; t /= 6u; cx = t % G; t /= G; cy = t % G; cz = t / G;
#endif
    const uint32_t c[3] = {cx, cy, cz};
    float o[3];
    for (int k = 0; k < 3; k++)
        o[k] = sc.occ_inv[k] > 0.f ? sc.root_mn[k] + ((float)c[k] + 0.5f) / sc.occ_inv[k] : sc.root_mn[k];
    const float hb = 0.5f * (float)B;
    const float u = ((float)ub + 0.5f) / hb - 1.f, v = ((float)vb + 0.5f) / hb - 1.f;
    const float sg = (face & 1u) ? -1.f : 1.f;
    float d[3];
    if (face < 2u) { d[0] = sg; d[1] = u; d[2] = v; }
    else if (face < 4u) { d[0] = u; d[1] = sg; d[2] = v; }
    else { d[0] = u; d[1] = v; d[2] = sg; }
    const float inv_n = 1.f / __builtin_sqrtf(d[0] * d[0] + d[1] * d[1] + d[2] * d[2]);
    ro[key] = make_float4(o[0], o[1], o[2], 0.f);
    rd[key] = make_float4(d[0] * inv_n, d[1] * inv_n, d[2] * inv_n, 0.f);
}
void launch_occ_probes(const DevScene& sc, float4* ro, float4* rd, uint32_t nkeys, hipStream_t s) {
    if (nkeys == 0) return;
    hipLaunchKernelGGL(k_occ_probes, dim3((nkeys + 255) / 256), dim3(256), 0, s, sc, ro, rd, nkeys);
}
void launch_occ_records(const DevScene& sc, uint32_t nnodes, float4* rec, hipStream_t s) {
    hipLaunchKernelGGL(k_occ_records, dim3(nnodes / 256 + 1), dim3(256), 0, s, sc, nnodes, rec);
}
void launch_clear(const ClearArgs& a, hipStream_t s) {
    if (a.n == 0) return;
    hipLaunchKernelGGL(k_clear, dim3((a.n + 255) / 256), dim3(256), 0, s, a);
}
void launch_hit_record(const HitRecordArgs& a, hipStream_t s) {
    if (a.n == 0) return;
    hipLaunchKernelGGL(k_hit_record, dim3((a.n + 255) / 256), dim3(256), 0, s, a);
}
void launch_resolve(const ResolveArgs& a, hipStream_t s) {
    if (a.n == 0) return;
    hipLaunchKernelGGL(k_resolve, dim3((a.n + 255) / 256), dim3(256), 0, s, a);
}
void launch_tonemap(const TonemapArgs& a, hipStream_t s) {
    if (a.n == 0) return;
    hipLaunchKernelGGL(k_tonemap, dim3((a.n + 255) / 256), dim3(256), 0, s, a);
}
void launch_accumulate(CounterBlock* c, uint32_t nparts, uint32_t* occ_gate, hipStream_t s) {
    hipLaunchKernelGGL(k_accumulate, dim3(1), dim3(kShards), 0, s, c, std::min<uint32_t>(kMaxParts, std::max<uint32_t>(1, nparts)),
                       occ_gate);
}
void launch_unpack(const UnpackArgs& a, hipStream_t s) {
    const uint32_t n = (uint32_t)(a.ntiles * a.tile_w * a.tile_h);
    if (n) hipLaunchKernelGGL(k_unpack, dim3((n + 255) / 256), dim3(256), 0, s, a);
}
void launch_pack(const PackArgs& a, hipStream_t s) {
    uint32_t n = (uint32_t)(a.ntiles * a.tile_w * a.tile_h);
    if (n == 0) return;
    hipLaunchKernelGGL(k_pack, dim3((n + 255) / 256), dim3(256), 0, s, a);
}

}
```

mc-path-tracer_amd/csrc/kernels.hpp:

```cpp
#pragma once
#include <hip/hip_runtime.h>
#include <stdint.h>

#include "device/adaptive.hpp"
#include "device/denoise.hpp"
#include "device/mcpt_core.hpp"
#include "device/temporal.hpp"
#include "device/variance.hpp"

namespace mcpt_dev {

constexpr int kBlock = 256;
constexpr int kTraceBlock = 64;
#ifndef MCPT_LDS_STACK
#define MCPT_LDS_STACK 8
#endif
constexpr int kLdsStack = MCPT_LDS_STACK;
#ifndef MCPT_LDS_STACK_DEEP
#define MCPT_LDS_STACK_DEEP 10
#endif
constexpr int kLdsStackDeep = MCPT_LDS_STACK_DEEP;
constexpr int kLdsStackTiny = 2;
#ifndef MCPT_DEEP_TREE
#define MCPT_DEEP_TREE 20
#endif
constexpr int kDeepTree = MCPT_DEEP_TREE;
constexpr int kMaxStack = 64;

enum : uint32_t {
    F_DEAD = 1u,
    F_LEN_SHIFT = 1,
    F_CONDL = 1u << 9,
    F_CONDB = 1u << 10,
    F_FZERO = 1u << 11,
    F_HASVIS = 1u << 12,
    F_SIDX_SHIFT = 13
};
constexpr uint32_t kMaxSpp = 1u << (32 - F_SIDX_SHIFT);
constexpr int kRecLenShift = 24;
static_assert(kMaxSpp <= (1u << kRecLenShift), "sample index and len share a record word");
constexpr uint32_t kRecNoCont = 1u << 23;
static_assert(kMaxSpp <= kRecNoCont && kRecNoCont < (1u << kRecLenShift), "the mark lies between sample index and len");

__host__ __device__ constexpr int shade_blocks_per_tile(int tile_px, int slots) {
    return (tile_px + kBlock - 1) / kBlock * slots;
}

#ifndef MCPT_TRI_F4
#define MCPT_TRI_F4 3
#endif
constexpr int kTriF4 = MCPT_TRI_F4;

struct DevScene {
    const float4* nodes;
    const float4* tri;
    const float4* tri_sh;
    float root_mn[3], root_mx[3];
    int root_ref;
    int depth;
    int width;
    int nlights;
    const float* mats;
    const float* dirs;
    mcpt::EnvView env;
    uint32_t* occ;
    uint32_t* occ_gate;
    const float4* occ_rec;
    uint32_t ntri;
    int occ_g, occ_b;
    float occ_inv[3];
    float cull_p, root_w;
    int cull_ok;
};
constexpr uint32_t kOccEmpty = 0xffffffffu;
constexpr uint32_t kOccWays = 2;
constexpr uint32_t kOccGateWords = 3;
constexpr uint32_t kOccMinRate = 10;
__host__ __device__ constexpr size_t occ_entries(int g, int b) { return (size_t)g * g * g * 6 * b * b * kOccWays; }

struct DevPaths {
    float4 *ray_o, *ray_d, *sray_o, *sray_d, *beta, *nee0, *nee1, *Ld;
    int32_t* hit_tri;
    uint32_t *flags, *samples;
    uint8_t* vis;
};

constexpr int kShards = 64;
constexpr int kMaxParts = kShards;
enum : int { C_EXT = 0, C_ANY = 1, C_VIS = 2, C_STATS = 3, C_EXT_RAYS = 9, C_ANY_RAYS = 10, C_MAT = 11, C_OCC = 12,
              C_OCC_TRY = 13, C_PH = 14, C_SKIP_INPLACE = 25, C_PRIM = 26, C_PRIM_RAYS = 27, C_SKIP_EXT = 28,
              C_SKIP_ANY = 29, C_SKIP_MAT = 30, C_WORDS = 32 };
enum : int {
    PH_TRIPS = 0,
    PH_REFILLS = 1,
    PH_REFILL_LANES = 2,
    PH_NODE_ITERS = 3,
    PH_TRI_PHASES = 4,
    PH_TRI_LANES = 5,
    PH_TRIP_NODE = 6,
    PH_TRIP_LEAF = 7,
    PH_TRIP_IDLE = 8,
    PH_FINISH_TRIPS = 9,
    PH_POP_ITERS = 10,
    kPhaseWords = 11
};
struct CounterBlock {
    uint32_t shard[kShards][C_WORDS];
    uint32_t last_ext, last_live;
    uint32_t trace_short;
    uint32_t idle;
    uint32_t pad[28];
    uint32_t last_ext_shard[kShards];
    uint32_t grab[kMaxParts][C_WORDS];
    unsigned long long tot_ext, tot_any, tot_vis, tot_occ;
    unsigned long long tot_stats[6];
    unsigned long long tot_ext_q, tot_any_q;
    unsigned long long tot_phase[kPhaseWords];
    unsigned long long tot_prim;
    unsigned long long tot_skip[4];
};
static_assert(C_PH + kPhaseWords <= C_SKIP_INPLACE, "counter words overlap");

constexpr char kPrimaryHitsEnv[] = "MCPT_PRIMARY_HITS";
constexpr int kPrimLine = 16;
constexpr int kPrimK = kPrimLine;

struct ShadeArgs {
    DevScene scene;
    mcpt::CamView cam;
    DevPaths p;
    const int2* tiles;
    int ntiles, tile_w, tile_h, W, H;
    int spp, max_depth, rr_depth;
    int slots;
    float slots_rcp;
    uint32_t npx;
    int compact;
    const int* tile_base;
    uint64_t seed;
    uint32_t *ext_q, *any_q;
    uint4* mat_rec;
    float4* mat_beta;
    uint32_t ext_cap, any_cap;
    CounterBlock* cnt;
    uint8_t* blk_done;
    uint32_t shade_vblocks;
    const float4* cam_px;
    const float4* cam_dir;
    const uint8_t* prim_cnt;
    const uint32_t* prim_list;
    uint2* prim_q;
    int skip;
    const uint32_t* budget;
};
struct PrimaryBuildArgs {
    DevScene scene;
    mcpt::CamView cam;
    int W, H;
    const float4 *cam_px, *cam_dir;
    uint8_t* cnt;
    uint32_t* list;
    uint32_t* stats;
};

struct TraceSet {
    const float4 *ro, *rd;
    const uint32_t* queue;
    const uint32_t* count_ptr;
    uint32_t count;
    uint32_t shard_cap;
    uint32_t* stats;
    uint32_t* ray_steps;
    int prefiltered;
    int ray_at_slot;
};
struct TraceArgs {
    DevScene scene;
    TraceSet set[2];
    int nshards;
    int32_t* hit_tri;
    uint8_t* vis;
    uint32_t refill_min;
    uint32_t tri_min;
    uint32_t nparts;
    uint32_t ndies;
    uint32_t* grab;
    const uint32_t* idle;
    int tiny_stack;
    uint32_t* phase;
};

struct HitRecordArgs { DevScene scene; const float4 *ro, *rd; const int32_t* tri; float4 *hit_p, *hit_n; int32_t* scene_tri; uint32_t n; };
struct ClearArgs { uint32_t* flags; uint32_t* samples; float4* Ld; uint32_t n, npx; };
struct ResolveArgs {
    const float4* Ld; const uint32_t* samples; float4* out_Ld; uint32_t* out_samples; uint32_t n; int slots;
    const int2* tiles; int tile_w, tile_h, W, H;
};
struct TonemapArgs { const float4* Ld; const uint32_t* samples; uchar4* out; float exposure; uint32_t n; };
struct PackArgs { const float4* Ld; const uint32_t* samples; const int2* tiles; int ntiles, tile_w, tile_h, W, H; float4* out; };
struct UnpackArgs { const float4* in; const int2* tiles; int ntiles, tile_w, tile_h, W, H; float4* Ld; uint32_t* samples; };

struct LaunchGeom {
    uint32_t trace_waves[2][2];
    uint32_t trace_parts;
    uint32_t ndies;
    uint32_t mat_blocks[2];
    uint32_t prim_blocks;
    uint32_t shade_grid;
    uint32_t refill_min, tri_min;
};
int launch_geometry(int device, LaunchGeom& g);
void launch_shade(const ShadeArgs& a, int nblocks, const LaunchGeom& g, bool fixed_mode, hipStream_t s);
void launch_shade_stage(bool material_stage, const ShadeArgs& a, int nblocks, const LaunchGeom& g, bool fixed_mode,
                        hipStream_t s);
void launch_trace(const TraceArgs& a, const LaunchGeom& g, hipStream_t s);
void launch_primary(const ShadeArgs& a, const LaunchGeom& g, hipStream_t s);
void launch_primary_build(const PrimaryBuildArgs& a, hipStream_t s);
void launch_clear(const ClearArgs& a, hipStream_t s);
constexpr int kOccRecF4 = 4;
void launch_occ_records(const DevScene& sc, uint32_t nnodes, float4* rec, hipStream_t s);
void launch_occ_probes(const DevScene& sc, float4* ro, float4* rd, uint32_t nkeys, hipStream_t s);
void launch_cull_margins(float4* nodes, uint32_t npairs, const float4* tri, uint32_t ntri, float* tri_w,
                         uint32_t* pmax, int passes, bool plane, hipStream_t s);
void launch_env_pack(float4* tex, const float* pdf, size_t n, hipStream_t s);
void launch_env_table(const mcpt::EnvView& e, bool fixed_mode, float4* out, float2* row, float2* col, hipStream_t s);
size_t env_build_scratch_floats(int W, int H);
void launch_env_build(const float4* tex, int W, int H, float* scratch, float* marginal_y, float* conds_y,
                      float* pdf, hipStream_t s);
void launch_env_guides(const float* marginal_y, const float* conds_y, int W, int H, uint16_t* gm, uint16_t* gc,
                       uint32_t* bad, hipStream_t s);

struct LbvhInput { int ntri; const float *v0, *v1, *v2; const float4 *d_tri, *d_sh; };
struct LbvhOutput {
    float4 *nodes = nullptr, *tri = nullptr, *tri_sh = nullptr;
    int nnodes = 0, root_ref = 0, depth = 0, rounds = 0;
    float root_mn[3], root_mx[3];
};
__host__ __device__ constexpr uint32_t ploc_pack(uint32_t height, uint32_t count) {
    return (height < 255u ? height : 255u) | (count << 8);
}
__host__ __device__ constexpr uint32_t ploc_height(uint32_t h) { return h & 0xffu; }
__host__ __device__ constexpr uint32_t ploc_count(uint32_t h) { return h >> 8; }
__host__ __device__ constexpr uint32_t ploc_merge(uint32_t a, uint32_t b) {
    return ploc_pack((ploc_height(a) > ploc_height(b) ? ploc_height(a) : ploc_height(b)) + 1u,
                     ploc_count(a) + ploc_count(b) + 1u);
}
int build_lbvh(const LbvhInput& in, LbvhOutput& out, hipStream_t s);
int build_ploc(const LbvhInput& in, LbvhOutput& out, hipStream_t s);
int trace_profile(unsigned long long* out, int reset);
int wave_times(unsigned long long* out, int n);
int shade_sections(unsigned long long* out, int n, int reset);
void launch_cam_table(const mcpt::CamView& cam, int W, int H, float4* px, float4* dir, hipStream_t s);
void launch_quot(const float* a, const float* b, float* out, uint32_t n, hipStream_t s);
void launch_copy(const float4* src, float4* dst, size_t n, hipStream_t s);
void launch_hit_record(const HitRecordArgs& a, hipStream_t s);
void launch_tonemap(const TonemapArgs& a, hipStream_t s);
void launch_resolve(const ResolveArgs& a, hipStream_t s);
void launch_accumulate(CounterBlock* c, uint32_t nparts, uint32_t* occ_gate, hipStream_t s);
void launch_pack(const PackArgs& a, hipStream_t s);
void launch_unpack(const UnpackArgs& a, hipStream_t s);

constexpr char kDenoiseLdsEnv[] = "MCPT_DENOISE_LDS_MAX";
constexpr char kGuideChunkEnv[] = "MCPT_GUIDE_CHUNK_BYTES";
struct DenoiseArgs {
    mcpt::DenoisePass k;
    int W, H;
    const float4 *col, *gd, *al;
    float4* out;
};
struct DenoisePrepArgs {
    const float4* Ld; const uint32_t* samples; const float4 *g_alb, *g_nz;
    const float *rgb, *normal, *albedo, *depth;
    float4 *col, *gd, *al; uint32_t n;
};
struct GuideArgs {
    mcpt::CamView cam;
    const float4 *cam_px, *cam_dir;
    int W, H;
    uint64_t seed;
    uint32_t p0, np, s0, ns;
    float4 *ro, *rd;
    const float4 *hit_p, *hit_n;
    const float* mats;
    float4 *g_alb, *g_nz;
};
struct DenoiseGuidedArgs : DenoiseArgs {
    mcpt::DenoiseVar v;
};
struct DenoiseGuidedPrepArgs : DenoisePrepArgs {
    const float4* err;
    const float* variance;
    float2* vl;
};
void launch_denoise_pass(const DenoiseGuidedArgs& a, int lds_max_stride, hipStream_t s);
void launch_denoise_prep(const DenoiseGuidedPrepArgs& a, hipStream_t s);
void launch_guide_rays(const GuideArgs& a, hipStream_t s);
void launch_guide_accum(const GuideArgs& a, hipStream_t s);

struct OwnMap {
    const int32_t* own;
    int compact, tile_w, tile_h, W, H;
};
struct FilmErrorArgs {
    const float4* Ld; const uint32_t* samples; size_t stride; int slots;
    OwnMap m;
    float4* out;
};
struct BudgetArgs {
    const float4* err;
    OwnMap m;
    mcpt::BudgetParams p;
    uint32_t* budget;
    unsigned long long* cnt;
};
struct SlotImageArgs {
    const float4* Ld; const uint32_t* samples;
    OwnMap m;
    float4* out_Ld; uint32_t* out_samples;
};
void launch_film_error(const FilmErrorArgs& a, hipStream_t s);
void launch_budget(const BudgetArgs& a, hipStream_t s);
void launch_slot_image(const SlotImageArgs& a, hipStream_t s);

struct TemporalArgs {
    int W, H;
    mcpt::TemporalParams k;
    float vp_prev[16];
    const uint32_t* samples;
    const float4 *Ld, *err, *g_alb, *g_nz, *cam_px, *cam_dir;
    mcpt::CamView cam;
    const float *rgb, *variance, *position, *normal, *depth;
    const float4 *hcol, *hpos, *hnrm;
    float4* col;
    float2* vl;
    float4 *out_hcol, *out_hpos, *out_hnrm;
    const float2* vfill;
};
struct TemporalPrepArgs {
    const float4* tcol; const float2* tvl; const float4 *g_alb, *g_nz;
    float4 *col, *gd, *al; float2* vl; uint32_t n;
};
void launch_temporal(const TemporalArgs& a, hipStream_t s);
void launch_temporal_prep(const TemporalPrepArgs& a, hipStream_t s);

struct VarianceArgs {
    mcpt::VariancePass k;
    int W, H;
    const float4 *col, *gd, *al;
    float2* vl;
};
void launch_variance_spatial(const VarianceArgs& a, hipStream_t s);

}
```

mc-path-tracer_amd/csrc/runtime.cpp:

```cpp
#include <cstdio>
#include <functional>

#include "runtime_internal.hpp"

extern "C" {

const char* mcpt_last_error(const mcpt_ctx* c) { return c ? c->err.c_str() : mcpt_host::global_error(); }

int mcpt_create(int device, const mcpt_config* cfg, mcpt_ctx** out) {
    if (!out) return set_err(nullptr, MCPT_E_INVALID, "out is null");
    *out = nullptr;
    int n = 0;
    if (hipGetDeviceCount(&n) != hipSuccess || n <= 0)
        return set_err(nullptr, MCPT_E_NODEVICE, "no HIP device visible (the backend has no CPU fallback)");
    if (device < 0 || device >= n) return set_err(nullptr, MCPT_E_INVALID, "device index out of range");
    hipDeviceProp_t prop;
    if (hipGetDeviceProperties(&prop, device) != hipSuccess)
        return set_err(nullptr, MCPT_E_HIP, "hipGetDeviceProperties failed");
    if (strncmp(prop.gcnArchName, "gfx950", 6) != 0)
        return set_err(nullptr, MCPT_E_NODEVICE, std::string("device is ") + prop.gcnArchName + ", code objects are gfx950 only");
    mcpt_ctx* c = new mcpt_ctx();
    c->device = device;
    c->num_cu = prop.multiProcessorCount;
    snprintf(c->devname, sizeof(c->devname), "%s (%s, %d CUs)", prop.name, prop.gcnArchName, prop.multiProcessorCount);
// ... 398 lines not shown
            std::vector<float> leaf_w;
            if (proot >= 0 && npairs > 0) {
                HIPCHK(c, hipMemcpyAsync(&rq, dn + 4 * (size_t)proot + 3, sizeof(rq), hipMemcpyDeviceToHost, c->stream));
            } else if (proot < 0) {
                const uint32_t off = (uint32_t)proot & 0xffffffu, cnt = (((uint32_t)proot >> 24) & 7u) + 1u;
                leaf_w.resize(cnt);
                HIPCHK(c, hipMemcpyAsync(leaf_w.data(), tw + off, cnt * sizeof(float), hipMemcpyDeviceToHost, c->stream));
            }
            HIPCHK(c, hipStreamSynchronize(c->stream));
            memcpy(&cull_p, &pb, 4);
            root_w = proot >= 0 ? std::fmax(rq.z, rq.w) : 0.f;
            for (float w : leaf_w) root_w = std::fmax(root_w, w);
            free_list(c->tmp_bufs);
        }
    }
    if ((rc = dupload(c, c->scene_bufs, &dm, d->mat_params, (size_t)d->nmat * 8))) return rc;
    if ((rc = dupload(c, c->scene_bufs, &dd, d->dir_params, (size_t)d->ndir * 7))) return rc;
    s.nodes = dn; s.tri = dt; s.tri_sh = dsh; s.mats = dm; s.dirs = dd;
    const size_t tree_pairs = gpu_bvh ? (size_t)lb.nnodes : pn.size() / 4;
    uint32_t nnodes = (uint32_t)tree_pairs;
    int width = tree_pairs * 64 > ((size_t)32 << 20) ? 4 : 2;
    if (const char* we = getenv("MCPT_BVH_WIDTH"))
        if ((we[0] == '2' || we[0] == '4') && we[1] == 0) width = we[0] - '0';
    int quad_root = 0, quad_push = 0;
    if (width == 4) {
        std::vector<float4> pairs;
        int proot;
        if (gpu_bvh && d->ntri > 0) {
            pairs.resize((size_t)lb.nnodes * 4);
            if (lb.nnodes) HIPCHK(c, hipMemcpy(pairs.data(), lb.nodes, pairs.size() * sizeof(float4), hipMemcpyDeviceToHost));
            proot = lb.root_ref;
        } else {
            pairs.resize(pn.size());
            if (!pn.empty()) HIPCHK(c, hipMemcpy(pairs.data(), dn, pairs.size() * sizeof(float4), hipMemcpyDeviceToHost));
            proot = N > 0 ? ref_of(0) : 0;
        }
        std::vector<float4> quads;
        int max_push = 0;
        if (d->ntri > 0) {
            pairs_to_quads(pairs, proot, quads, quad_root, max_push);
            if (max_push > kMaxStack) return set_err(c, MCPT_E_INVALID, "4-wide BVH needs more than 64 stack entries");
            quad_push = max_push;
            float4* dq;
            if ((rc = dupload(c, c->scene_bufs, &dq, quads.data(), quads.size()))) return rc;
            s.nodes = dq;
            nnodes = (uint32_t)(quads.size() / 8);
        }
    }
    s.nlights = 1 + d->ndir;
    if (gpu_bvh && d->ntri > 0) {
        for (int k = 0; k < 3; k++) { s.root_mn[k] = lb.root_mn[k]; s.root_mx[k] = lb.root_mx[k]; }
        s.root_ref = width == 4 ? (lb.root_ref < 0 ? lb.root_ref : quad_root) : lb.root_ref;
    } else if (N > 0) {
        for (int k = 0; k < 3; k++) { s.root_mn[k] = d->bmin[k]; s.root_mx[k] = d->bmax[k]; }
        s.root_ref = width == 4 ? (ref_of(0) < 0 ? ref_of(0) : quad_root) : ref_of(0);
    } else {
        for (int k = 0; k < 3; k++) { s.root_mn[k] = 1.f; s.root_mx[k] = -1.f; }
        s.root_ref = 0;
    }
    s.env.mode = d->env_mode;
    for (int k = 0; k < 3; k++) s.env.color[k] = d->env_color[k];
    s.env.ls = d->env_ls;
    s.env.w = d->env_w;
    s.env.h = d->env_h;
    s.env.tex = nullptr;
    s.env.guide_m = s.env.guide_c = nullptr;
    s.env.ltab[0] = s.env.ltab[1] = nullptr;
    s.env.lrow[0] = s.env.lrow[1] = nullptr;
    s.env.lcol[0] = s.env.lcol[1] = nullptr;
    if (d->env_mode == 1) {
        float4* tx;
        float *my, *cy, *pd;
        const int W = d->env_w, H = d->env_h;
        size_t WH = (size_t)W * H;
        if ((rc = dupload(c, c->scene_bufs, &tx, reinterpret_cast<const float4*>(d->env_tex), WH))) return rc;
        c->env_device_built = !d->env_marginal_y;
        c->last_env_build_ms = 0.f;
        if (!c->env_device_built) {
            if ((rc = dupload(c, c->scene_bufs, &my, d->env_marginal_y, (size_t)H))) return rc;
            if ((rc = dupload(c, c->scene_bufs, &cy, d->env_conds_y, WH))) return rc;
            if ((rc = dupload(c, c->scene_bufs, &pd, d->env_pdf, WH))) return rc;
        } else {
            if ((rc = dalloc(c, c->scene_bufs, &my, (size_t)H)) || (rc = dalloc(c, c->scene_bufs, &cy, WH)) ||
                (rc = dalloc(c, c->scene_bufs, &pd, WH)))
                return rc;
            float* scratch = nullptr;
            hipError_t e = hipMalloc(&scratch, mcpt_dev::env_build_scratch_floats(W, H) * sizeof(float));
            if (e != hipSuccess) return set_err(c, MCPT_E_NOMEM, std::string("hipMalloc: ") + hipGetErrorString(e));
            HIPCHK(c, hipEventRecord(ev(c, 0), c->stream));
            mcpt_dev::launch_env_build(tx, W, H, scratch, my, cy, pd, c->stream);
            HIPCHK(c, hipEventRecord(ev(c, 1), c->stream));
            e = hipGetLastError();
            if (e == hipSuccess) e = hipStreamSynchronize(c->stream);
            (void)hipFree(scratch);
            if (e != hipSuccess) return set_err(c, MCPT_E_HIP, std::string("env build: ") + hipGetErrorString(e));
            float ms = 0.f;
            HIPCHK(c, hipEventElapsedTime(&ms, ev(c, 0), ev(c, 1)));
            c->last_env_build_ms = ms;
        }
        s.env.tex = tx; s.env.marginal_y = my; s.env.conds_y = cy; s.env.pdf = pd;
        mcpt_dev::launch_env_pack(tx, pd, WH, c->stream);
        HIPCHK(c, hipGetLastError());
        s.env.guide_m = s.env.guide_c = nullptr;
        c->env_guides = false;
        if (W <= 65535 && H <= 65535) {
            const size_t G1 = mcpt::kEnvGuide + 1;
            uint16_t *dgm, *dgc;
            uint32_t* dbad;
            if ((rc = dalloc(c, c->scene_bufs, &dgm, G1)) || (rc = dalloc(c, c->scene_bufs, &dgc, (size_t)H * G1)) ||
                (rc = dalloc(c, c->scene_bufs, &dbad, 1)))
                return rc;
            HIPCHK(c, hipMemsetAsync(dbad, 0, sizeof(uint32_t), c->stream));
            mcpt_dev::launch_env_guides(my, cy, W, H, dgm, dgc, dbad, c->stream);
            HIPCHK(c, hipGetLastError());
            uint32_t bad = 1;
            HIPCHK(c, hipMemcpyAsync(&bad, dbad, sizeof(bad), hipMemcpyDeviceToHost, c->stream));
            HIPCHK(c, hipStreamSynchronize(c->stream));
            bool ok = bad == 0;
            if (const char* g = std::getenv("MCPT_ENV_GUIDES")) ok = ok && g[0] != '0';
            if (ok) {
                s.env.guide_m = dgm;
                s.env.guide_c = dgc;
                c->env_guides = true;
            }
        }
        if ((size_t)(d->env_w + 1) * d->env_h < ((size_t)1 << 28)) {
            const size_t ne = (size_t)(d->env_w + 1) * d->env_h;
            float4 *lt0, *lt1;
            float2 *rc0, *rc1;
            const size_t nrc = (size_t)d->env_h + d->env_w + 1;
            if ((rc = dalloc(c, c->scene_bufs, &lt0, ne)) || (rc = dalloc(c, c->scene_bufs, &lt1, ne)) ||
                (rc = dalloc(c, c->scene_bufs, &rc0, nrc)) || (rc = dalloc(c, c->scene_bufs, &rc1, nrc)))
                return rc;
            launch_env_table(s.env, false, lt0, rc0, rc0 + d->env_h, c->stream);
            launch_env_table(s.env, true, lt1, rc1, rc1 + d->env_h, c->stream);
            HIPCHK(c, hipGetLastError());
            HIPCHK(c, hipStreamSynchronize(c->stream));
            s.env.ltab[0] = lt0;
            s.env.ltab[1] = lt1;
            s.env.lrow[0] = rc0;
            s.env.lrow[1] = rc1;
            s.env.lcol[0] = rc0 + d->env_h;
            s.env.lcol[1] = rc1 + d->env_h;
        }
    }
    s.depth = width == 4 ? quad_push : c->pair_depth;
    s.width = width;
    s.cull_p = cull_p;
    s.root_w = root_w;
    s.cull_ok = cull_ok ? 1 : 0;
    s.ntri = (uint32_t)d->ntri;
    s.occ = nullptr;
    s.occ_rec = nullptr;
    {
        int G = 24, B = 12;
        if (const char* e = getenv("MCPT_OCC_G")) G = atoi(e);
        if (const char* e = getenv("MCPT_OCC_B")) B = atoi(e);
        const bool occ_want = G > 0 && G <= 64 && B > 0 && B <= 64 && (uint64_t)G * G * G * 6 * B * B <= 0xffffffffull;
        float4* lbx = nullptr;
        if (d->ntri > 0 && c->occ_nest_ok && (occ_want || c->prim.on)) {
            void* q = nullptr;
            if (hipMalloc(&q, kOccRecF4 * (size_t)d->ntri * sizeof(float4)) == hipSuccess) {
                c->scene_bufs.push_back(q);
                lbx = (float4*)q;
            } else {
                (void)hipGetLastError();
                if (occ_want) return set_err(c, MCPT_E_NOMEM, "hipMalloc: occluder records");
            }
        }
        if (lbx) {
            HIPCHK(c, hipMemsetAsync(lbx, 0xff, kOccRecF4 * (size_t)d->ntri * sizeof(float4), c->stream));
            launch_occ_records(s, nnodes, lbx, c->stream);
            HIPCHK(c, hipGetLastError());
            HIPCHK(c, hipStreamSynchronize(c->stream));
            s.occ_rec = lbx;
        }
        if (occ_want && lbx) {
            uint32_t* occ;
            const size_t ne = occ_entries(G, B);
            if ((rc = dalloc(c, c->scene_bufs, &occ, ne + kOccGateWords))) return rc;
            HIPCHK(c, hipMemsetAsync(occ, 0xff, ne * sizeof(uint32_t), c->stream));
            HIPCHK(c, hipMemsetAsync(occ + ne, 0, kOccGateWords * sizeof(uint32_t), c->stream));
            HIPCHK(c, hipStreamSynchronize(c->stream));
            s.occ = occ;
            s.occ_gate = occ + ne;
            c->occ_entries_n = ne;
            s.occ_g = G;
            s.occ_b = B;
            for (int k = 0; k < 3; k++) {
                const float ext = s.root_mx[k] - s.root_mn[k];
                s.occ_inv[k] = ext > 0.f && ext < 3.4e38f ? (float)G / ext : 0.f;
            }
        }
    }
    c->scene = s;
    c->scene_gen++;
    c->tp.ok = false;
    c->ntri = d->ntri;
    c->occ_init = nullptr;
    if (s.occ) {
        const char* pe = getenv("MCPT_OCC_PREFILL");
        if (!(pe && pe[0] == '0' && pe[1] == 0)) {
            const uint32_t nkeys = (uint32_t)(c->occ_entries_n / kOccWays);
            float4 *pro, *prd;
            uint8_t* pvis;
            free_list(c->tmp_bufs);
            if ((rc = dalloc(c, c->tmp_bufs, &pro, nkeys)) || (rc = dalloc(c, c->tmp_bufs, &prd, nkeys)) ||
                (rc = dalloc(c, c->tmp_bufs, &pvis, nkeys)) || (rc = dalloc(c, c->scene_bufs, &c->occ_init, c->occ_entries_n)))
                return rc;
            launch_occ_probes(s, pro, prd, nkeys, c->stream);
            TraceArgs ta{};
            ta.scene = s;
            ta.nshards = 1;
            TraceSet& ts = ta.set[1];
            ts.ro = pro;
            ts.rd = prd;
            ts.count = nkeys;
            ts.shard_cap = nkeys;
            ta.vis = pvis;
            ta.grab = &c->cnt->grab[0][0];
            launch_trace(ta, c->geom, c->stream);
            HIPCHK(c, hipMemsetAsync(c->cnt->grab, 0, sizeof(c->cnt->grab), c->stream));
            HIPCHK(c, hipMemcpyAsync(c->occ_init, s.occ, c->occ_entries_n * sizeof(uint32_t), hipMemcpyDeviceToDevice,
                                     c->stream));
            const uint32_t warm[kOccGateWords] = {0u, 0u, 1u};
            HIPCHK(c, hipMemcpyAsync(s.occ_gate, warm, sizeof(warm), hipMemcpyHostToDevice, c->stream));
            HIPCHK(c, hipGetLastError());
            HIPCHK(c, hipStreamSynchronize(c->stream));
            free_list(c->tmp_bufs);
        }
    }
    if (c->has_scene_before) c->film_stale = true;
    c->has_scene = true;
    return MCPT_OK;
}

int mcpt_scene_upload(mcpt_ctx* c, const mcpt_scene_desc* d) { return scene_upload(c, d, false); }
int mcpt_scene_upload_gpu_bvh(mcpt_ctx* c, const mcpt_scene_desc* d) { return scene_upload(c, d, true); }
int mcpt_set_gpu_bvh_builder(mcpt_ctx* c, int32_t builder) {
    if (!c || (builder != MCPT_GPU_BVH_LBVH && builder != MCPT_GPU_BVH_PLOC))
        return set_err(c, MCPT_E_INVALID, "unknown GPU BVH builder");
    c->gpu_bvh_builder = builder;
    return MCPT_OK;
}
float mcpt_debug_last_build_ms(const mcpt_ctx* c) { return c ? c->last_build_ms : -1.f; }
float mcpt_debug_last_env_build_ms(const mcpt_ctx* c) { return c ? c->last_env_build_ms : -1.f; }

int mcpt_debug_env_tables(mcpt_ctx* c, float* marginal_y, float* conds_y, float* pdf, int32_t* flags) {
    if (!c) return set_err(c, MCPT_E_INVALID, "null context");
    if (!c->has_scene || c->scene.env.mode != 1 || !c->scene.env.tex) return set_err(c, MCPT_E_INVALID, "no HRDI scene uploaded");
    const mcpt::EnvView& e = c->scene.env;
    const size_t WH = (size_t)e.w * e.h;
    HIPCHK(c, hipSetDevice(c->device));
    HIPCHK(c, hipStreamSynchronize(c->stream));
    if (marginal_y) HIPCHK(c, hipMemcpy(marginal_y, e.marginal_y, (size_t)e.h * sizeof(float), hipMemcpyDeviceToHost));
    if (conds_y) HIPCHK(c, hipMemcpy(conds_y, e.conds_y, WH * sizeof(float), hipMemcpyDeviceToHost));
    if (pdf) HIPCHK(c, hipMemcpy(pdf, e.pdf, WH * sizeof(float), hipMemcpyDeviceToHost));
    if (flags) *flags = (c->env_device_built ? 1 : 0) | (c->env_guides ? 2 : 0);
    return MCPT_OK;
}
int mcpt_debug_node_layout(const mcpt_ctx* c) { return c ? c->node_layout : MCPT_E_INVALID; }
int mcpt_debug_bvh_read(mcpt_ctx* c, float* nodes, float* tris, mcpt_bvh_info* info) {
    if (!c) return set_err(c, MCPT_E_INVALID, "null context");
    if (!c->has_scene) return set_err(c, MCPT_E_INVALID, "no scene uploaded");
    const DevScene& s = c->scene;
    if (info) {
        info->npairs = (int32_t)c->pair_count;
        info->root_ref = c->pair_root;
        info->depth = c->pair_depth;
        info->width = s.width;
        info->layout = c->node_layout;
        info->ntri = (int32_t)s.ntri;
        info->tri_f4 = kTriF4;
        info->gpu_built = c->pair_gpu_built ? 1 : 0;
        info->rounds = c->ploc_rounds;
        for (int k = 0; k < 3; k++) { info->root_mn[k] = s.root_mn[k]; info->root_mx[k] = s.root_mx[k]; }
        info->cull_p = s.cull_p;
    }
    HIPCHK(c, hipSetDevice(c->device));
    HIPCHK(c, hipStreamSynchronize(c->stream));
    if (nodes && c->pair_count)
        HIPCHK(c, hipMemcpy(nodes, c->pair_nodes, (size_t)c->pair_count * 4 * sizeof(float4), hipMemcpyDeviceToHost));
    if (tris && s.ntri)
        HIPCHK(c, hipMemcpy(tris, s.tri, (size_t)s.ntri * kTriF4 * sizeof(float4), hipMemcpyDeviceToHost));
    return MCPT_OK;
}
int mcpt_debug_ray_counts(const mcpt_ctx* c, uint64_t* out) {
    if (!c || !out) return MCPT_E_INVALID;
    const CounterBlock& t = c->totals;
    const bool ok = c->totals_ok;
    out[0] = ok ? t.tot_ext : 0;
    out[1] = ok ? t.tot_ext_q : 0;
    out[2] = ok ? t.tot_any : 0;
    out[3] = ok ? t.tot_any_q : 0;
    out[4] = ok ? t.tot_occ : 0;
    return MCPT_OK;
}
int mcpt_debug_primary_stats(const mcpt_ctx* c, double* out4) {
    if (!c || !out4) return MCPT_E_INVALID;
    out4[0] = c->prim.ok ? (double)c->prim.lists : 0.0;
    out4[1] = c->prim.ok ? (double)c->prim.over : 0.0;
    out4[2] = c->totals_ok ? (double)c->totals.tot_prim : 0.0;
    out4[3] = (double)c->prim.build_ms;
    return (int)std::min<uint64_t>(c->prim.builds, 0x7fffffffull);
}
int mcpt_debug_discard_stats(const mcpt_ctx* c, uint64_t* out4) {
    if (!c || !out4) return MCPT_E_INVALID;
    for (int k = 0; k < 4; k++) out4[k] = c->totals_ok ? c->totals.tot_skip[k] : 0;
    return MCPT_OK;
}
int mcpt_debug_occ_stats(const mcpt_ctx* c, uint64_t* resolved, int32_t* enabled) {
    if (!c) return MCPT_E_INVALID;
    if (resolved) *resolved = c->totals_ok ? c->totals.tot_occ : 0;
    if (enabled) *enabled = c->scene.occ != nullptr;
    return MCPT_OK;
}

int mcpt_camera_set(mcpt_ctx* c, const mcpt_camera* cam) {
    if (!c || !cam) return set_err(c, MCPT_E_INVALID, "null argument");
    mcpt::CamView nc = c->cam;
    memcpy(nc.ivp, cam->inv_view_proj, sizeof(nc.ivp));
    memcpy(nc.iv, cam->inv_view, sizeof(nc.iv));
    nc.lens_radius = cam->lens_radius;
    nc.focal = cam->focal;
    if (c->has_cam && memcmp(&nc, &c->cam, sizeof(nc)) != 0) c->film_stale = true;
    c->cam = nc;
    c->has_cam = true;
    return MCPT_OK;
}

static int set_tiles_internal(mcpt_ctx* c, const std::vector<int2>& t) {
    const uint32_t nblocks = (uint32_t)t.size() * (uint32_t)shade_blocks_per_tile((int)(c->tile_w * c->tile_h), (int)c->slots);
    c->ext_cap = std::max<uint32_t>(1, (nblocks + kShards - 1) / kShards) * kBlock;
    c->any_cap = 2 * c->ext_cap;
    const size_t need = (size_t)kShards * c->ext_cap;
    if (need > c->queue_alloc) {
        HIPCHK(c, hipStreamSynchronize(c->stream));
        if (c->ext_q) (void)hipFree(c->ext_q);
        if (c->any_q) (void)hipFree(c->any_q);
        if (c->mat_q) (void)hipFree(c->mat_q);
        if (c->any_ray) (void)hipFree(c->any_ray);
        c->ext_q = c->any_q = c->mat_q = nullptr;
        c->any_ray = nullptr;
        c->queue_alloc = 0;
        if (hipMalloc(&c->ext_q, need * sizeof(uint32_t)) != hipSuccess ||
            hipMalloc(&c->any_q, 2 * need * sizeof(uint32_t)) != hipSuccess ||
            hipMalloc(&c->mat_q, need * 8 * sizeof(uint32_t)) != hipSuccess ||
            hipMalloc(&c->any_ray, 4 * need * sizeof(float4)) != hipSuccess)
            return set_err(c, MCPT_E_NOMEM, "queue allocation failed");
        c->queue_alloc = need;
    }
    c->p.sray_o = c->any_ray;
    c->p.sray_d = c->any_ray + 2 * c->queue_alloc;
    if (t.size() > c->tiles_cap) {
        if (c->tiles) HIPCHK(c, hipFree(c->tiles));
        c->tiles = nullptr;
        HIPCHK(c, hipMalloc(&c->tiles, std::max<size_t>(t.size(), 1) * sizeof(int2)));
        c->tiles_cap = (uint32_t)t.size();
    }
    if (!t.empty()) HIPCHK(c, hipMemcpyAsync(c->tiles, t.data(), t.size() * sizeof(int2), hipMemcpyHostToDevice, c->stream));
    HIPCHK(c, hipStreamSynchronize(c->stream));
    c->tiles_h = t;
    return MCPT_OK;
}
static std::vector<int2> all_tiles(const mcpt_ctx* c) {
    std::vector<int2> t;
    uint32_t nx = (c->W + c->tile_w - 1) / c->tile_w, ny = (c->H + c->tile_h - 1) / c->tile_h;
    for (uint32_t y = 0; y < ny; y++)
        for (uint32_t x = 0; x < nx; x++) t.push_back(make_int2((int)x, (int)y));
    return t;
}

int mcpt_film_clear(mcpt_ctx* c) {
    if (!c || !c->P) return set_err(c, MCPT_E_INVALID, "film not allocated");
    HIPCHK(c, hipSetDevice(c->device));
    ClearArgs a{c->p.flags, c->p.samples, c->p.Ld, (uint32_t)(c->npx * c->slots), (uint32_t)c->npx};
    launch_clear(a, c->stream);
    HIPCHK(c, hipGetLastError());
    if (c->compact) {
        HIPCHK(c, hipMemsetAsync(c->film_Ld, 0, c->P * sizeof(float4), c->stream));
        HIPCHK(c, hipMemsetAsync(c->film_samples, 0, c->P * sizeof(uint32_t), c->stream));
    }
    if (c->blk_done) HIPCHK(c, hipMemsetAsync(c->blk_done, 0, c->blk_done_n, c->stream));
    if (c->scene.occ) {
        if (c->occ_init) {
            HIPCHK(c, hipMemcpyAsync(c->scene.occ, c->occ_init, c->occ_entries_n * sizeof(uint32_t),
                                     hipMemcpyDeviceToDevice, c->stream));
            static const uint32_t warm[kOccGateWords] = {0u, 0u, 1u};
            HIPCHK(c, hipMemcpyAsync(c->scene.occ_gate, warm, sizeof(warm), hipMemcpyHostToDevice, c->stream));
        } else {
            HIPCHK(c, hipMemsetAsync(c->scene.occ, 0xff, c->occ_entries_n * sizeof(uint32_t), c->stream));
            HIPCHK(c, hipMemsetAsync(c->scene.occ_gate, 0, kOccGateWords * sizeof(uint32_t), c->stream));
        }
    }
    c->film_stale = false;
    c->unpacked.clear();
    HIPCHK(c, hipMemsetAsync(c->cnt, 0, sizeof(CounterBlock), c->stream));
    HIPCHK(c, hipStreamSynchronize(c->stream));
    memset(&c->totals, 0, sizeof(c->totals));
    memset(c->phase_base, 0, sizeof(c->phase_base));
    c->totals_ok = true;
    return MCPT_OK;
}

static int alloc_film_state(mcpt_ctx* c) {
    HIPCHK(c, hipStreamSynchronize(c->stream));
    free_list(c->film_bufs);
    {
        DevPaths keep{};
        keep.sray_o = c->p.sray_o;
        keep.sray_d = c->p.sray_d;
        c->p = keep;
    }
    c->film_Ld = nullptr;
    c->film_samples = nullptr;
    c->blk_done = nullptr;
    c->blk_done_n = 0;
    const uint32_t w = c->W, h = c->H, tw = c->tile_w, th = c->tile_h;
    const size_t npix = (size_t)w * h;
    const size_t npx = c->compact ? c->tiles_h.size() * (size_t)tw * th : npix;
    const size_t P = npx * c->slots;
    c->npx = 0;
    if (P >= (1ull << 31)) return set_err(c, MCPT_E_INVALID, "film too large for the path slots");
    DevPaths p{};
    int rc;
    if ((rc = dalloc(c, c->film_bufs, &p.ray_o, P)) || (rc = dalloc(c, c->film_bufs, &p.ray_d, P)) ||
        (rc = dalloc(c, c->film_bufs, &p.hit_tri, P)) ||
        (rc = dalloc(c, c->film_bufs, &p.beta, P)) || (rc = dalloc(c, c->film_bufs, &p.nee0, P)) ||
        (rc = dalloc(c, c->film_bufs, &p.nee1, P)) || (rc = dalloc(c, c->film_bufs, &p.Ld, P)) ||
        (rc = dalloc(c, c->film_bufs, &p.flags, P)) || (rc = dalloc(c, c->film_bufs, &p.samples, P)) ||
        (rc = dalloc(c, c->film_bufs, &p.vis, 2 * P)))
        return rc;
    {
        const size_t ntiles = (size_t)((w + tw - 1) / tw) * ((h + th - 1) / th);
        c->blk_done_n = c->slots * ntiles * (size_t)shade_blocks_per_tile((int)(tw * th), 1);
        if ((rc = dalloc(c, c->film_bufs, &c->blk_done, c->blk_done_n))) return rc;
    }
    if ((c->slots > 1 || c->compact) && ((rc = dalloc(c, c->film_bufs, &c->film_Ld, npix)) ||
                                         (rc = dalloc(c, c->film_bufs, &c->film_samples, npix))))
        return rc;
    HIPCHK(c, hipMemset(p.hit_tri, 0xff, P * sizeof(int32_t)));
    HIPCHK(c, hipMemset(p.vis, 0, 2 * P));
    p.sray_o = c->p.sray_o;
    p.sray_d = c->p.sray_d;
    c->p = p;
    c->npx = npx;
    return MCPT_OK;
}

static int film_resize(mcpt_ctx* c, uint32_t w, uint32_t h, uint32_t tw, uint32_t th) {
    if (!c || w == 0 || h == 0 || tw == 0 || th == 0) return set_err(c, MCPT_E_INVALID, "bad film size");
    if ((uint64_t)w * h >= (1ull << 31)) return set_err(c, MCPT_E_INVALID, "film too large");
    if ((uint64_t)tw * th > (1ull << 26)) return set_err(c, MCPT_E_INVALID, "tile too large");
    HIPCHK(c, hipSetDevice(c->device));
    HIPCHK(c, hipStreamSynchronize(c->stream));
    free_list(c->film_bufs);
    c->guides = Guides{};
    c->dn = Denoise{};
    c->P = 0;
    c->npx = 0;
    c->p = DevPaths{};
// ... 1075 lines not shown
```

mc-path-tracer_amd/csrc/runtime_internal.hpp:

```cpp
#pragma once
#include <hip/hip_runtime.h>

#include <algorithm>
#include <cstdlib>
#include <cstring>
#include <string>
#include <vector>

#include "kernels.hpp"
#include "mcpt.h"

using namespace mcpt_dev;

namespace mcpt_host {
void set_global_error(const std::string& e);
const char* global_error();
}

template <class T>
class DevBuf {
    T* p_ = nullptr;
    size_t n_ = 0;

public:
    DevBuf() = default;
    DevBuf(const DevBuf&) = delete;
    DevBuf& operator=(const DevBuf&) = delete;
    DevBuf(DevBuf&& o) noexcept : p_(o.p_), n_(o.n_) { o.p_ = nullptr, o.n_ = 0; }
    DevBuf& operator=(DevBuf&& o) noexcept {
        if (this != &o) {
            reset();
            std::swap(p_, o.p_);
            std::swap(n_, o.n_);
        }
        return *this;
    }
    ~DevBuf() { reset(); }
    void reset() {
        if (p_) (void)hipFree(p_);
        p_ = nullptr;
        n_ = 0;
    }
    bool ensure(size_t count) {
        if (p_ && n_ >= count) return true;
        reset();
        if (hipMalloc((void**)&p_, std::max<size_t>(count * sizeof(T), 16)) != hipSuccess) {
            p_ = nullptr;
            return false;
        }
        n_ = count;
        return true;
    }
    size_t size() const { return n_; }
    size_t bytes() const { return p_ ? std::max<size_t>(n_ * sizeof(T), 16) : 0; }
    T* get() const { return p_; }
    operator T*() const { return p_; }
};

struct ViewKey {
    enum : unsigned { SCENE = 1, SEED = 2, SIZE = 4, CAM = 8 };
    uint64_t scene_gen = 0, seed = 0;
    uint32_t W = 0, H = 0;
    mcpt::CamView cam{};
    bool same(const ViewKey& o, unsigned fields) const {
        return (!(fields & SCENE) || scene_gen == o.scene_gen) && (!(fields & SEED) || seed == o.seed) &&
               (!(fields & SIZE) || (W == o.W && H == o.H)) && (!(fields & CAM) || memcmp(&cam, &o.cam, sizeof(cam)) == 0);
    }
};

struct CamTable {
    DevBuf<float4> tab;
    ViewKey key;
    bool ok = false;
};

struct PrimTable {
    bool on = [] { const char* e = getenv(kPrimaryHitsEnv); return !(e && e[0] == '0' && e[1] == 0); }();
    DevBuf<uint8_t> cnt;
    DevBuf<uint32_t> list, stats;
    DevBuf<uint2> q;
    bool ok = false;
    bool failed = false;
    ViewKey key;
    uint64_t builds = 0;
    uint32_t lists = 0, over = 0;
    float build_ms = 0.f;
    void release() {
        cnt.reset(), list.reset(), stats.reset(), q.reset();
        ok = false;
    }
};

struct Guides {
    DevBuf<float4> alb, nz;
    bool ok = false;
    ViewKey key;
};
struct Denoise {
    DevBuf<float4> col[2], gd, al;
    DevBuf<float2> vl[2];
    int result = -1;
    bool guided = false;
};
struct Adaptive {
    DevBuf<uint32_t> budget;
    bool budget_on = false;
    uint32_t budget_max = 0;
    DevBuf<float4> err4;
    bool err_ok = false;
    DevBuf<int32_t> own_map;
    DevBuf<unsigned long long> bud_cnt;
    size_t bytes() const { return budget.bytes() + err4.bytes() + own_map.bytes() + bud_cnt.bytes(); }
};
struct Temporal {
    DevBuf<float4> h[2][3], col;
    DevBuf<float2> vl;
    int set = 0;
    bool ok = false;
    ViewKey key;
    size_t bytes() const {
        size_t b = col.bytes() + vl.bytes();
        for (const auto& s : h)
            for (const auto& p : s) b += p.bytes();
        return b;
    }
};
struct StageMs {
    float guides = 0.f, dn[9] = {};
    float err = 0.f, budget = 0.f;
    float tp = 0.f;
    float var = 0.f;
};
struct VarianceFill {
    bool on = false;
    mcpt_variance_params p{};
};

struct mcpt_ctx {
    int device = 0;
    hipStream_t stream = nullptr;
    std::string err;
    mcpt_config cfg{};
    char devname[256] = {0};
    int num_cu = 0;
    LaunchGeom geom{};
    uint32_t trace_parts_default = 1;
    std::vector<void*> scene_bufs;
    DevScene scene{};
    bool has_scene = false;
    bool has_scene_before = false;
    int32_t ntri = 0;
    size_t occ_entries_n = 0;
    uint32_t* occ_init = nullptr;
    int pair_depth = 0;
    bool cull_ok = true, occ_nest_ok = true;
    bool count_work = getenv("MCPT_WORK_COUNTERS") != nullptr;
    int node_layout = 0;
    const float4* pair_nodes = nullptr;
    uint32_t pair_count = 0;
    int pair_root = 0, ploc_rounds = 0;
    bool pair_gpu_built = false;
    bool skip_discarded = true;
    mcpt::CamView cam{};
    bool has_cam = false;
    CamTable cam_tab;
    PrimTable prim;
    uint64_t scene_gen = 0;
    bool film_stale = false;
    uint32_t W = 0, H = 0, tile_w = 256, tile_h = 256;
    size_t P = 0;
    uint32_t slots = 1;
    bool compact = false;
    size_t npx = 0;
    float4* film_Ld = nullptr;
    uint32_t* film_samples = nullptr;
    std::vector<void*> film_bufs;
    uint8_t* blk_done = nullptr;
    size_t blk_done_n = 0;
    bool blk_done_off = getenv("MCPT_NO_BLOCK_DONE") != nullptr;
    DevPaths p{};
    uint32_t *ext_q = nullptr, *any_q = nullptr, *mat_q = nullptr;
    float4* any_ray = nullptr;
    uint32_t ext_cap = 0, any_cap = 0;
    size_t queue_alloc = 0;
    CounterBlock* cnt = nullptr;
    CounterBlock* cnt_host = nullptr;
    CounterBlock totals{};
    bool totals_ok = false;
    int2* step_tile = nullptr;
    int2* step_tile_h = nullptr;
    int2* tiles = nullptr;
    std::vector<int2> tiles_h;
    std::vector<int2> unpacked;
    uint32_t tiles_cap = 0;
    std::vector<hipEvent_t> events;
    std::vector<void*> tmp_bufs;
    float last_stage_ms = 0.f;
    float last_build_ms = 0.f;
    float last_env_build_ms = 0.f;
    bool env_device_built = false;
    bool env_guides = false;
    int gpu_bvh_builder = MCPT_GPU_BVH_PLOC;
    bool tiny_stack = false;
    unsigned long long phase_base[kPhaseWords] = {};
    Guides guides;
    Denoise dn;
    Adaptive ad;
    Temporal tp;
    VarianceFill vf;
    StageMs ms;

    ViewKey view() const { return ViewKey{scene_gen, cfg.seed, W, H, cam}; }
};

inline int set_err(mcpt_ctx* c, int rc, const std::string& msg) {
    if (c) c->err = msg;
    mcpt_host::set_global_error(msg);
    return rc;
}
#define HIPCHK(c, x)                                                                          \
    do {                                                                                      \
        hipError_t e_ = (x);                                                                  \
        if (e_ != hipSuccess)                                                                 \
            return set_err((c), MCPT_E_HIP, std::string(#x) + ": " + hipGetErrorString(e_));  \
    } while (0)

inline void free_list(std::vector<void*>& v) {
    for (void* q : v)
        if (q) (void)hipFree(q);
    v.clear();
}
template <class T>
int dalloc(mcpt_ctx* c, std::vector<void*>& list, T** out, size_t count) {
    void* q = nullptr;
    size_t bytes = std::max<size_t>(count * sizeof(T), 16);
    hipError_t e = hipMalloc(&q, bytes);
    if (e != hipSuccess) return set_err(c, MCPT_E_NOMEM, std::string("hipMalloc: ") + hipGetErrorString(e));
    list.push_back(q);
    *out = (T*)q;
    return MCPT_OK;
}
template <class T>
int dupload(mcpt_ctx* c, std::vector<void*>& list, T** out, const T* src, size_t count) {
    int rc = dalloc(c, list, out, count);
    if (rc) return rc;
    if (count) HIPCHK(c, hipMemcpy(*out, src, count * sizeof(T), hipMemcpyHostToDevice));
    return MCPT_OK;
}
struct TmpScope {
    std::vector<void*>& L;
    explicit TmpScope(mcpt_ctx* c) : L(c->tmp_bufs) { free_list(L); }
    ~TmpScope() { free_list(L); }
    TmpScope(const TmpScope&) = delete;
    TmpScope& operator=(const TmpScope&) = delete;
};

hipEvent_t ev(mcpt_ctx* c, size_t i);
int check_ready(mcpt_ctx* c);
int cam_table(mcpt_ctx* c, uint32_t W, uint32_t H, const float4** px, const float4** dir);
int film_view(mcpt_ctx* c, const float4** Ld, const uint32_t** samples);
int read_plane(mcpt_ctx* c, const float4* d, size_t n, float* xyz, float* w);
int tonemap_rgba8(mcpt_ctx* c, const float4* col, const uint32_t* samples, float exposure, uint8_t* out);
```

mc-path-tracer_amd/mcpt/__init__.py:

```python
from __future__ import annotations

import ctypes as C
import os
from dataclasses import dataclass

import numpy as np

_HERE = os.path.dirname(os.path.abspath(__file__))
PKG_DIR = os.path.dirname(_HERE)
REPO_DIR = os.path.dirname(PKG_DIR)
LIB_PATH = os.environ.get("MCPT_LIB") or os.path.join(PKG_DIR, "libmcpt.so")
ASSET_DIR = os.path.join(REPO_DIR, "assets")

MCPT_OK = 0
STAGE_LOGIC, STAGE_GENERATE, STAGE_MATERIAL, STAGE_EXTEND, STAGE_SHADOW = range(5)

_f = C.POINTER(C.c_float)
_i = C.POINTER(C.c_int32)
_u = C.POINTER(C.c_uint32)


class Config(C.Structure):
    _fields_ = [("seed", C.c_uint64), ("spp", C.c_int32), ("max_depth", C.c_int32), ("rr_depth", C.c_int32),
                ("tile_w", C.c_int32), ("tile_h", C.c_int32), ("flags", C.c_int32)]
# ... 19 lines not shown
                ("lens_radius", C.c_float), ("focal", C.c_float)]


class StageStats(C.Structure):
    _fields_ = [("extend_rays", C.c_uint64), ("shadow_rays", C.c_uint64), ("vis_rays", C.c_uint64),
                ("iterations", C.c_uint64), ("live_paths", C.c_uint64), ("ms_total", C.c_float),
                ("ms_shade", C.c_float), ("ms_extend", C.c_float), ("ms_shadow", C.c_float),
                ("ext_nodes", C.c_uint64), ("ext_tests", C.c_uint64), ("ext_hits", C.c_uint64),
                ("any_nodes", C.c_uint64), ("any_tests", C.c_uint64), ("any_hits", C.c_uint64)]

    def as_dict(self) -> dict:
        return {k: getattr(self, k) for k, _ in self._fields_}

    @property
    def rays(self) -> int:
        return int(self.extend_rays + self.shadow_rays + self.vis_rays)


class DenoiseParams(C.Structure):
    _fields_ = [("passes", C.c_int32), ("sigma_color", C.c_float), ("sigma_normal", C.c_float),
                ("sigma_albedo", C.c_float), ("sigma_depth", C.c_float)]


class DenoiseGuidedParams(C.Structure):
    _fields_ = [("passes", C.c_int32), ("sigma_lum", C.c_float), ("lum_eps", C.c_float), ("sigma_color", C.c_float),
                ("sigma_normal", C.c_float), ("sigma_albedo", C.c_float), ("sigma_depth", C.c_float)]


class SampleBudgetParams(C.Structure):
    _fields_ = [("target_rel_err", C.c_float), ("lum_floor", C.c_float), ("min_spp", C.c_uint32), ("max_spp", C.c_uint32)]


class TemporalParams(C.Structure):
    _fields_ = [("pos_tol", C.c_float), ("nrm_tol", C.c_float), ("max_history", C.c_float), ("alpha_min", C.c_float)]


class VarianceParams(C.Structure):
    _fields_ = [("radius", C.c_int32), ("sigma_normal", C.c_float), ("sigma_albedo", C.c_float),
                ("sigma_depth", C.c_float), ("min_neff", C.c_float)]


class BvhInfo(C.Structure):
    _fields_ = [("npairs", C.c_int32), ("root_ref", C.c_int32), ("depth", C.c_int32), ("width", C.c_int32),
                ("layout", C.c_int32), ("ntri", C.c_int32), ("tri_f4", C.c_int32), ("gpu_built", C.c_int32),
                ("rounds", C.c_int32), ("root_mn", C.c_float * 3), ("root_mx", C.c_float * 3), ("cull_p", C.c_float)]


class PathView(C.Structure):
    _fields_ = [("film_w", C.c_uint32), ("film_h", C.c_uint32), ("flags", _u), ("samples", _u), ("hit_tri", _i),
                ("ray_o", _f), ("ray_d", _f), ("beta", _f), ("nee0", _f), ("nee1", _f),
                ("vis", C.POINTER(C.c_uint8)), ("Ld", _f), ("light_o", _f), ("light_d", _f), ("bvis_o", _f),
                ("bvis_d", _f), ("queued", C.POINTER(C.c_uint8))]


class SoaView(C.Structure):
    _fields_ = [("ray_o", _f), ("ray_d", _f), ("hit_pos_t", _f), ("hit_nrm_mat", _f), ("hit_tri", _i),
                ("visible", C.POINTER(C.c_uint8)), ("steps", _u), ("paths", C.POINTER(PathView))]


PATH_FIELDS = {"flags": (np.uint32, 1), "samples": (np.uint32, 1), "hit_tri": (np.int32, 1), "ray_o": (np.float32, 3),
               "ray_d": (np.float32, 3), "beta": (np.float32, 4), "nee0": (np.float32, 4), "nee1": (np.float32, 4),
               "vis": (np.uint8, 2), "Ld": (np.float32, 3), "light_o": (np.float32, 3), "light_d": (np.float32, 3),
               "bvis_o": (np.float32, 3), "bvis_d": (np.float32, 3), "queued": (np.uint8, 1)}
STAGE_BY_NAME = {"logic": STAGE_LOGIC, "generate": STAGE_GENERATE, "material": STAGE_MATERIAL}


def path_view(arrs: dict, n, film=(0, 0)):
    v = PathView()
    v.film_w, v.film_h = film
    keep = {}
    for k, (dt, m) in PATH_FIELDS.items():
        if k in arrs and arrs[k] is not None:
            a = np.ascontiguousarray(arrs[k], dt).reshape(n * m)
            keep[k] = a
            setattr(v, k, a.ctypes.data_as(C.POINTER(np.ctypeslib.as_ctypes_type(dt))))
    v._keep = keep
    return v


ABI = {
    "mcpt_create": (C.c_int, [C.c_int, C.POINTER(Config), C.POINTER(C.c_void_p)]),
    "mcpt_destroy": (None, [C.c_void_p]),
    "mcpt_last_error": (C.c_char_p, [C.c_void_p]),
    "mcpt_scene_upload": (C.c_int, [C.c_void_p, C.POINTER(SceneDesc)]),
    "mcpt_camera_set": (C.c_int, [C.c_void_p, C.POINTER(Camera)]),
    "mcpt_film_resize": (C.c_int, [C.c_void_p, C.c_uint32, C.c_uint32, C.c_uint32, C.c_uint32]),
    "mcpt_film_clear": (C.c_int, [C.c_void_p]),
    "mcpt_set_tiles": (C.c_int, [C.c_void_p, _u, C.c_uint32]),
    "mcpt_set_compact_paths": (C.c_int, [C.c_void_p, C.c_int32]),
    "mcpt_debug_tiny_lds_stack": (C.c_int, [C.c_void_p, C.c_int32]),
    "mcpt_set_path_slots": (C.c_int, [C.c_void_p, C.c_uint32]),
    "mcpt_set_trace_partitions": (C.c_int, [C.c_void_p, C.c_uint32]),
    "mcpt_gather": (C.c_int, [C.POINTER(C.c_void_p), C.c_int32, C.c_int32]),
    "mcpt_wavefront_step": (C.c_int, [C.c_void_p, C.c_uint32, C.c_uint32, C.POINTER(StageStats)]),
    "mcpt_iterate": (C.c_int, [C.c_void_p, C.c_uint32, C.POINTER(StageStats)]),
    "mcpt_render": (C.c_int, [C.c_void_p, C.POINTER(StageStats)]),
    "mcpt_stage_run": (C.c_int, [C.c_void_p, C.c_int, C.POINTER(SoaView), C.POINTER(SoaView), C.c_uint32]),
    "mcpt_film_read": (C.c_int, [C.c_void_p, _f, _u]),
    "mcpt_film_read_device": (C.c_int, [C.c_void_p, C.c_void_p, C.c_void_p]),
    "mcpt_film_pack_tiles": (C.c_int, [C.c_void_p, C.c_void_p, _u]),
    "mcpt_film_unpack_tiles": (C.c_int, [C.c_void_p, C.c_void_p, _u, C.c_uint32]),
    "mcpt_film_tonemap_rgba8": (C.c_int, [C.c_void_p, C.c_float, C.POINTER(C.c_uint8)]),
    "mcpt_guides_render": (C.c_int, [C.c_void_p, C.c_uint32]),
    "mcpt_guides_read": (C.c_int, [C.c_void_p, _f, _f, _f, _u]),
    "mcpt_denoise_default_params": (C.c_int, [C.POINTER(DenoiseParams)]),
    "mcpt_denoise_run": (C.c_int, [C.c_void_p, C.c_uint32, C.c_uint32, _f, _u, _f, _f, _f, C.POINTER(DenoiseParams), _f]),
    "mcpt_film_denoise": (C.c_int, [C.c_void_p, C.POINTER(DenoiseParams)]),
    "mcpt_denoised_read": (C.c_int, [C.c_void_p, _f]),
    "mcpt_denoised_read_device": (C.c_int, [C.c_void_p, C.c_void_p]),
    "mcpt_denoised_tonemap_rgba8": (C.c_int, [C.c_void_p, C.c_float, C.POINTER(C.c_uint8)]),
    "mcpt_denoised_write_png": (C.c_int, [C.c_void_p, C.c_float, C.c_char_p]),
    "mcpt_debug_denoise_ms": (C.c_int, [C.c_void_p, _f]),
    "mcpt_denoise_guided_default_params": (C.c_int, [C.POINTER(DenoiseGuidedParams)]),
    "mcpt_denoise_guided_run": (C.c_int, [C.c_void_p, C.c_uint32, C.c_uint32, _f, _u, _f, _f, _f, _f,
                                          C.POINTER(DenoiseGuidedParams), _f, _f]),
    "mcpt_film_denoise_guided": (C.c_int, [C.c_void_p, C.POINTER(DenoiseGuidedParams)]),
    "mcpt_denoised_variance_read": (C.c_int, [C.c_void_p, _f]),
    "mcpt_set_sample_budget": (C.c_int, [C.c_void_p, _u]),
    "mcpt_sample_budget_read": (C.c_int, [C.c_void_p, _u]),
    "mcpt_set_spp": (C.c_int, [C.c_void_p, C.c_int32]),
    "mcpt_film_error": (C.c_int, [C.c_void_p]),
    "mcpt_film_error_read": (C.c_int, [C.c_void_p, _f]),
    "mcpt_error_run": (C.c_int, [C.c_void_p, C.c_uint32, C.c_uint32, C.c_uint32, _f, _u, _f]),
    "mcpt_debug_film_read_slot": (C.c_int, [C.c_void_p, C.c_uint32, _f, _u]),
    "mcpt_sample_budget_default_params": (C.c_int, [C.POINTER(SampleBudgetParams)]),
    "mcpt_budget_from_error": (C.c_int, [C.c_void_p, C.POINTER(SampleBudgetParams), C.POINTER(C.c_uint64)]),
    "mcpt_debug_adaptive_bytes": (C.c_int64, [C.c_void_p]),
    "mcpt_debug_adaptive_ms": (C.c_int, [C.c_void_p, _f]),
    "mcpt_set_seed": (C.c_int, [C.c_void_p, C.c_uint64]),
    "mcpt_camera_view_proj": (C.c_int, [C.POINTER(Camera), _f]),
    "mcpt_temporal_default_params": (C.c_int, [C.POINTER(TemporalParams)]),
    "mcpt_film_temporal": (C.c_int, [C.c_void_p, C.POINTER(TemporalParams)]),
    "mcpt_temporal_reset": (C.c_int, [C.c_void_p]),
    "mcpt_temporal_read": (C.c_int, [C.c_void_p, _f, _f, _f, _f]),
    "mcpt_temporal_denoise": (C.c_int, [C.c_void_p, C.POINTER(DenoiseGuidedParams)]),
    "mcpt_temporal_run": (C.c_int, [C.c_void_p, C.c_uint32, C.c_uint32, _f, _u, _f, _f, _f, _f, _f, _f, _f, _f,
                                    C.POINTER(TemporalParams), _f, _f, _f, _f, _f]),
    "mcpt_debug_temporal_bytes": (C.c_int64, [C.c_void_p]),
    "mcpt_debug_temporal_ms": (C.c_int, [C.c_void_p, _f]),
    "mcpt_variance_default_params": (C.c_int, [C.POINTER(VarianceParams)]),
    "mcpt_variance_run": (C.c_int, [C.c_void_p, C.c_uint32, C.c_uint32, _f, _u, _f, _f, _f, _f, C.POINTER(VarianceParams), _f]),
    "mcpt_set_variance_fill": (C.c_int, [C.c_void_p, C.POINTER(VarianceParams)]),
    "mcpt_debug_variance_ms": (C.c_int, [C.c_void_p, _f]),
    "mcpt_sync": (C.c_int, [C.c_void_p]),
    "mcpt_device_name": (C.c_int, [C.c_void_p, C.c_char_p, C.c_int32]),
    "mcpt_debug_queue_rays": (C.c_int, [C.c_void_p, C.c_int, _f, _f, _u]),
    "mcpt_debug_last_stage_ms": (C.c_float, [C.c_void_p]),
    "mcpt_debug_last_build_ms": (C.c_float, [C.c_void_p]),
    "mcpt_debug_last_env_build_ms": (C.c_float, [C.c_void_p]),
    "mcpt_debug_env_tables": (C.c_int, [C.c_void_p, _f, _f, _f, _i]),
    "mcpt_debug_node_layout": (C.c_int, [C.c_void_p]),
    "mcpt_debug_bvh_read": (C.c_int, [C.c_void_p, _f, _f, C.POINTER(BvhInfo)]),
    "mcpt_debug_occ_stats": (C.c_int, [C.c_void_p, C.POINTER(C.c_uint64), C.POINTER(C.c_int32)]),
    "mcpt_debug_ray_counts": (C.c_int, [C.c_void_p, C.POINTER(C.c_uint64)]),
    "mcpt_debug_primary_stats": (C.c_int, [C.c_void_p, C.POINTER(C.c_double)]),
    "mcpt_set_work_counters": (C.c_int, [C.c_void_p, C.c_int32]),
    "mcpt_set_skip_discarded": (C.c_int, [C.c_void_p, C.c_int32]),
    "mcpt_debug_discard_stats": (C.c_int, [C.c_void_p, C.POINTER(C.c_uint64)]),
    "mcpt_scene_upload_gpu_bvh": (C.c_int, [C.c_void_p, C.c_void_p]),
    "mcpt_set_gpu_bvh_builder": (C.c_int, [C.c_void_p, C.c_int32]),
    "mcpt_film_size": (C.c_int, [C.c_void_p, C.POINTER(C.c_uint32), C.POINTER(C.c_uint32)]),
    "mcpt_film_write_png": (C.c_int, [C.c_void_p, C.c_float, C.c_char_p]),
    "mcpt_film_write_pfm": (C.c_int, [C.c_void_p, C.c_char_p]),
    "mcpt_image_write_png": (C.c_int, [C.c_char_p, C.c_uint32, C.c_uint32, C.POINTER(C.c_uint8)]),
    "mcpt_image_write_pfm": (C.c_int, [C.c_char_p, C.c_uint32, C.c_uint32, C.POINTER(C.c_float)]),
    "mcpt_debug_trace_profile": (C.c_int, [C.c_void_p, C.POINTER(C.c_uint64), C.c_int]),
    "mcpt_debug_shade_sections": (C.c_int, [C.c_void_p, C.POINTER(C.c_uint64), C.c_int, C.c_int]),
    "mcpt_scene_build_ex": (C.c_int, [C.c_void_p, C.c_void_p]),
    "mcpt_debug_quot": (C.c_int, [C.c_void_p, C.c_void_p, C.c_void_p, C.c_uint32, C.c_void_p]),
    "mcpt_debug_hbm_copy": (C.c_int, [C.c_void_p, C.c_uint64, C.c_uint32, C.POINTER(C.c_double)]),
    "mcpt_scene_new": (C.c_void_p, []),
    "mcpt_scene_free": (None, [C.c_void_p]),
    "mcpt_scene_load_glb": (C.c_int, [C.c_void_p, C.c_char_p, _f]),
    "mcpt_scene_add_mesh": (C.c_int, [C.c_void_p, C.c_int32, _f, _f, _f, _f, _f, _f, _f]),
    "mcpt_scene_set_env_hdr": (C.c_int, [C.c_void_p, C.c_char_p, C.c_int32]),
    "mcpt_scene_set_env_hdr_ex": (C.c_int, [C.c_void_p, C.c_char_p, C.c_int32, C.c_uint32]),
    "mcpt_scene_set_env_color": (C.c_int, [C.c_void_p, _f, C.c_float]),
    "mcpt_scene_add_dir_light": (C.c_int, [C.c_void_p, _f, _f, C.c_float]),
    "mcpt_scene_transform": (C.c_int, [C.c_void_p, _f]),
    "mcpt_scene_make_proxy": (C.c_int, [C.c_void_p, C.c_int32, C.c_char_p]),
    "mcpt_scene_build": (C.c_int, [C.c_void_p, C.c_int32]),
    "mcpt_scene_get_desc": (C.c_int, [C.c_void_p, C.POINTER(SceneDesc)]),
    "mcpt_scene_bvh_depth": (C.c_int, [C.c_void_p]),
    "mcpt_camera_make": (C.c_int, [C.POINTER(CameraParams), C.POINTER(Camera)]),
}

_lib = None


def lib() -> C.CDLL:
    global _lib
    if _lib is None:
        if not os.path.exists(LIB_PATH):
            raise RuntimeError(f"{LIB_PATH} missing: run __graft_entry__.build() (make) first")
        l = C.CDLL(LIB_PATH)
        for name, (res, args) in ABI.items():
            fn = getattr(l, name, None)
            if fn is None and os.environ.get("MCPT_LIB"):
                continue
            if fn is None:
                raise RuntimeError(f"{LIB_PATH} does not export {name}: rebuild it")
            fn.restype = res
            fn.argtypes = args
        _lib = l
    return _lib


class McptError(RuntimeError):
    pass


def _check(rc: int, ctx=None):
    if rc != MCPT_OK:
        msg = lib().mcpt_last_error(ctx)
        raise McptError(f"mcpt error {rc}: {msg.decode() if msg else ''}")


def fptr(a: np.ndarray):
    return a.ctypes.data_as(_f)


class BvhParams(C.Structure):
    _fields_ = [("builder", C.c_int32), ("max_prims", C.c_int32), ("buckets", C.c_int32),
                ("trav_cost", C.c_float), ("isect_cost", C.c_float)]


BVH_REFERENCE, BVH_SAH3 = 0, 1
FLAG_FIXED = 1
FLAG_NO_AUTO_CLEAR = 2
ENV_DEVICE_TABLES = 1


def default_config(spp=16, max_depth=5, rr_depth=3, seed=0x5EED2026, tile=256, fixed=False,
                   auto_clear=True) -> Config:
    flags = (FLAG_FIXED if fixed else 0) | (0 if auto_clear else FLAG_NO_AUTO_CLEAR)
    return Config(seed, spp, max_depth, rr_depth, tile, tile, flags)


def make_camera(position, yaw_deg=-90.0, pitch_deg=0.0, fovy_deg=45.0, aspect=1.0, znear=0.01, zfar=1e4,
                lens_radius=1e-4, focal=35.0) -> Camera:
    p = CameraParams((C.c_float * 3)(*position), yaw_deg, pitch_deg, np.float32(np.radians(np.float32(fovy_deg))),
                     aspect, znear, zfar, lens_radius, focal)
    cam = Camera()
    _check(lib().mcpt_camera_make(C.byref(p), C.byref(cam)))
    return cam


def _arr(ptr, n, dtype):
    if n == 0 or not ptr:
        return np.zeros(0, dtype)
    ct = {np.float32: C.c_float, np.int32: C.c_int32}[dtype]
    return np.ctypeslib.as_array(C.cast(ptr, C.POINTER(ct)), shape=(n,)).copy()


class Scene:

    def __init__(self):
        self.h = lib().mcpt_scene_new()
        if not self.h:
            raise McptError("mcpt_scene_new failed")

    def __del__(self):
        if getattr(self, "h", None):
            try:
                lib().mcpt_scene_free(self.h)
            except Exception:
                pass
            self.h = None

    def _ck(self, rc):
        _check(rc)
        return self

    def load_glb(self, path, xform=None):
        xf = None if xform is None else fptr(np.ascontiguousarray(xform, np.float32).reshape(16))
        return self._ck(lib().mcpt_scene_load_glb(self.h, str(path).encode(), xf))

    def add_mesh(self, v0, v1, v2, n0, n1, n2, base_rgb=(1.0, 1.0, 1.0)):
        arrs = [np.ascontiguousarray(a, np.float32).reshape(-1, 3) for a in (v0, v1, v2, n0, n1, n2)]
        bc = np.asarray(base_rgb, np.float32)
        return self._ck(lib().mcpt_scene_add_mesh(self.h, len(arrs[0]), *[fptr(a) for a in arrs], fptr(bc)))

    def set_env_hdr(self, path, mode=1, device_tables=False):
        if device_tables:
            return self._ck(lib().mcpt_scene_set_env_hdr_ex(self.h, str(path).encode(), mode, ENV_DEVICE_TABLES))
        return self._ck(lib().mcpt_scene_set_env_hdr(self.h, str(path).encode(), mode))

    def set_env_color(self, rgb, ls=1.0):
        return self._ck(lib().mcpt_scene_set_env_color(self.h, fptr(np.asarray(rgb, np.float32)), ls))

    def add_dir_light(self, direction, rgb, ls=1.0):
        return self._ck(lib().mcpt_scene_add_dir_light(self.h, fptr(np.asarray(direction, np.float32)),
                                                       fptr(np.asarray(rgb, np.float32)), ls))

    def transform(self, xform):
        return self._ck(lib().mcpt_scene_transform(self.h, fptr(np.ascontiguousarray(xform, np.float32).reshape(16))))

    def make_proxy(self, config_id, asset_dir=ASSET_DIR):
        return self._ck(lib().mcpt_scene_make_proxy(self.h, config_id, str(asset_dir).encode()))

    def build(self, max_prims=8, builder="reference", buckets=32, trav_cost=1.0, isect_cost=1.0):
        if builder == "reference":
            return self._ck(lib().mcpt_scene_build(self.h, max_prims))
        if builder != "sah3":
            raise ValueError(f"unknown builder {builder!r}")
        p = BvhParams(BVH_SAH3, max_prims, buckets, trav_cost, isect_cost)
        return self._ck(lib().mcpt_scene_build_ex(self.h, C.byref(p)))

    def desc(self) -> SceneDesc:
        d = SceneDesc()
        _check(lib().mcpt_scene_get_desc(self.h, C.byref(d)))
        d._owner = self
        return d

    @property
    def bvh_depth(self) -> int:
        return lib().mcpt_scene_bvh_depth(self.h)

    def arrays(self) -> dict:
        d = self.desc()
        T, N = d.ntri, d.nnodes
        out = {k: _arr(getattr(d, k), 3 * T, np.float32).reshape(T, 3) for k in ("v0", "v1", "v2", "n0", "n1", "n2")}
        out["mat"] = _arr(d.mat, T, np.int32)
        out["bmin"] = _arr(d.bmin, 3 * N, np.float32).reshape(N, 3)
        out["bmax"] = _arr(d.bmax, 3 * N, np.float32).reshape(N, 3)
        for k in ("offset", "nprims", "axis"):
            out[k] = _arr(getattr(d, k), N, np.int32)
        out["mat_params"] = _arr(d.mat_params, 8 * d.nmat, np.float32).reshape(d.nmat, 8)
        out["dir_params"] = _arr(d.dir_params, 7 * d.ndir, np.float32).reshape(d.ndir, 7)
        out["env_mode"] = d.env_mode
        out["env_color"] = np.array(list(d.env_color), np.float32)
        out["env_ls"] = np.float32(d.env_ls)
        W, H = d.env_w, d.env_h
        out["env_tex"] = _arr(d.env_tex, 4 * W * H, np.float32).reshape(H, W, 4)
        out["env_marginal_y"] = _arr(d.env_marginal_y, H, np.float32)
        out["env_conds_y"] = _arr(d.env_conds_y, W * H, np.float32).reshape(H, W) if d.env_conds_y else np.zeros(0, np.float32)
        out["env_pdf"] = _arr(d.env_pdf, W * H, np.float32).reshape(H, W) if d.env_pdf else np.zeros(0, np.float32)
        out["tri_id"] = _arr(d.tri_id, T, np.int32) if d.tri_id else np.arange(T, dtype=np.int32)
        return out


def desc_from_arrays(a: dict) -> SceneDesc:
    keep = {}

    def f(k):
        arr = np.ascontiguousarray(a[k], np.float32)
        keep[k] = arr
        return arr.ctypes.data_as(_f) if arr.size else None

    def i(k):
        arr = np.ascontiguousarray(a[k], np.int32)
        keep[k] = arr
        return arr.ctypes.data_as(_i) if arr.size else None

    d = SceneDesc()
    d.ntri = len(a["mat"])
    d.v0, d.v1, d.v2, d.n0, d.n1, d.n2 = (f(k) for k in ("v0", "v1", "v2", "n0", "n1", "n2"))
    d.mat = i("mat")
    d.nnodes = len(a["nprims"])
    d.bmin, d.bmax = f("bmin"), f("bmax")
    d.offset, d.nprims, d.axis = i("offset"), i("nprims"), i("axis")
    d.nmat = len(a["mat_params"])
    d.mat_params = f("mat_params")
    d.ndir = len(a["dir_params"])
    d.dir_params = f("dir_params")
    d.env_mode = int(a["env_mode"])
    for k in range(3):
        d.env_color[k] = float(a["env_color"][k])
    d.env_ls = float(a["env_ls"])
    tex = np.asarray(a["env_tex"])
    d.env_h, d.env_w = (tex.shape[0], tex.shape[1]) if tex.size else (0, 0)
    d.env_tex, d.env_marginal_y, d.env_conds_y, d.env_pdf = (f(k) for k in ("env_tex", "env_marginal_y", "env_conds_y", "env_pdf"))
    d.tri_id = i("tri_id") if "tri_id" in a and len(a["tri_id"]) else None
    d._keep = keep
    return d


class PathTracer:

    def __init__(self, device=0, config: Config | None = None):
        self.cfg = config or default_config()
        h = C.c_void_p()
        _check(lib().mcpt_create(device, C.byref(self.cfg), C.byref(h)))
        self.h = h
        self.W = self.H = 0

    def close(self):
        if getattr(self, "h", None):
            try:
                lib().mcpt_destroy(self.h)
            except Exception:
                pass
            self.h = None

    __del__ = close

    def _ck(self, rc):
        _check(rc, self.h)

    @property
    def device_name(self) -> str:
        buf = C.create_string_buffer(256)
        self._ck(lib().mcpt_device_name(self.h, buf, 256))
        return buf.value.decode()

    def upload_scene(self, scene, gpu_bvh=False):
        d = scene.desc() if isinstance(scene, Scene) else scene
        if gpu_bvh:
            if gpu_bvh not in (True, "ploc", "lbvh"):
                raise ValueError(f"unknown GPU BVH builder {gpu_bvh!r}")
            self._ck(lib().mcpt_set_gpu_bvh_builder(self.h, 0 if gpu_bvh == "lbvh" else 1))
            self._ck(lib().mcpt_scene_upload_gpu_bvh(self.h, C.byref(d)))
        else:
            self._ck(lib().mcpt_scene_upload(self.h, C.byref(d)))

    def ray_counts(self) -> dict:
        v = (C.c_uint64 * 5)()
        if hasattr(lib(), "mcpt_debug_ray_counts") or not os.environ.get("MCPT_LIB"):
            self._ck(lib().mcpt_debug_ray_counts(self.h, v))
        return dict(zip(("extension", "extension_traversed", "any_hit", "any_hit_traversed", "any_hit_occluder_cache"),
                        [int(x) for x in v]))

    def primary_stats(self) -> dict:
        v = (C.c_double * 4)()
        n = lib().mcpt_debug_primary_stats(self.h, v)
        if n < 0:
            raise McptError(f"mcpt_debug_primary_stats failed ({n})")
        return dict(lists=int(v[0]), overflow=int(v[1]), resolved=int(v[2]), build_ms=float(v[3]), builds=int(n))

    def set_skip_discarded(self, on=True):
        if hasattr(lib(), "mcpt_set_skip_discarded") or not os.environ.get("MCPT_LIB"):
            self._ck(lib().mcpt_set_skip_discarded(self.h, int(bool(on))))

    def discard_stats(self) -> dict:
        v = (C.c_uint64 * 4)()
        if hasattr(lib(), "mcpt_debug_discard_stats") or not os.environ.get("MCPT_LIB"):
            self._ck(lib().mcpt_debug_discard_stats(self.h, v))
        return dict(zip(("extension_untraced", "any_hit_untraced", "evaluations_not_run", "doomed_in_place"),
                        [int(x) for x in v]))

    def occ_stats(self):
        r, e = C.c_uint64(0), C.c_int32(0)
        self._ck(lib().mcpt_debug_occ_stats(self.h, C.byref(r), C.byref(e)))
        return int(r.value), bool(e.value)

    @property
    def last_build_ms(self) -> float:
        return lib().mcpt_debug_last_build_ms(self.h)

    def bvh_read(self):
        bi = BvhInfo()
        self._ck(lib().mcpt_debug_bvh_read(self.h, None, None, C.byref(bi)))
        nodes = np.zeros((bi.npairs, 4, 4), np.float32)
        tris = np.zeros((bi.ntri, bi.tri_f4, 4), np.float32)
        self._ck(lib().mcpt_debug_bvh_read(self.h, fptr(nodes) if nodes.size else None,
                                           fptr(tris) if tris.size else None, C.byref(bi)))
        info = {k: getattr(bi, k) for k, _ in BvhInfo._fields_}
        for k in ("root_mn", "root_mx"):
            info[k] = np.array(list(info[k]), np.float32)
        info["cull_p"] = np.float32(info["cull_p"])
        return nodes, tris, info

    @property
    def last_env_build_ms(self) -> float:
        return lib().mcpt_debug_last_env_build_ms(self.h)

    def env_tables(self, W, H) -> dict:
        my = np.zeros(H, np.float32)
        cy = np.zeros((H, W), np.float32)
        pdf = np.zeros((H, W), np.float32)
        fl = C.c_int32(0)
        self._ck(lib().mcpt_debug_env_tables(self.h, fptr(my), fptr(cy), fptr(pdf), C.byref(fl)))
        return {"marginal_y": my, "conds_y": cy, "pdf": pdf, "device_built": bool(fl.value & 1),
                "guides": bool(fl.value & 2)}

    def set_camera(self, cam: Camera):
        self._ck(lib().mcpt_camera_set(self.h, C.byref(cam)))

    def resize(self, W, H, tile_w=256, tile_h=256):
        self._ck(lib().mcpt_film_resize(self.h, W, H, tile_w, tile_h))
        self.W, self.H, self.tile_w, self.tile_h = W, H, tile_w, tile_h

    def clear(self):
        self._ck(lib().mcpt_film_clear(self.h))

    def set_path_slots(self, slots):
        self._ck(lib().mcpt_set_path_slots(self.h, slots))

    def set_work_counters(self, on=True):
        if hasattr(lib(), "mcpt_set_work_counters") or not os.environ.get("MCPT_LIB"):
            self._ck(lib().mcpt_set_work_counters(self.h, int(bool(on))))

    def set_trace_partitions(self, nparts=0):
        self._ck(lib().mcpt_set_trace_partitions(self.h, nparts))

    def set_compact_paths(self, on=True):
        self._ck(lib().mcpt_set_compact_paths(self.h, int(bool(on))))

    def set_tiny_lds_stack(self, on=True):
        self._ck(lib().mcpt_debug_tiny_lds_stack(self.h, int(bool(on))))

    def set_tiles(self, tiles=None):
        if tiles is None:
            self._ck(lib().mcpt_set_tiles(self.h, None, 0))
        else:
            t = np.ascontiguousarray(tiles, np.uint32).reshape(-1, 2)
            self._ck(lib().mcpt_set_tiles(self.h, t.ctypes.data_as(_u), len(t)))

    def step(self, tile_x, tile_y) -> StageStats:
        st = StageStats()
        self._ck(lib().mcpt_wavefront_step(self.h, tile_x, tile_y, C.byref(st)))
        return st

    def iterate(self, n) -> StageStats:
        st = StageStats()
        self._ck(lib().mcpt_iterate(self.h, n, C.byref(st)))
        return st

    def render(self) -> StageStats:
        st = StageStats()
        self._ck(lib().mcpt_render(self.h, C.byref(st)))
        return st

    def film(self):
        P = self.W * self.H
        Ld = np.zeros(3 * P, np.float32)
        s = np.zeros(P, np.uint32)
        self._ck(lib().mcpt_film_read(self.h, fptr(Ld), s.ctypes.data_as(_u)))
        return Ld.reshape(self.H, self.W, 3), s.reshape(self.H, self.W)

    def tonemap(self, exposure=1.0, denoised=False):
        out = np.zeros(self.W * self.H * 4, np.uint8)
        fn = lib().mcpt_denoised_tonemap_rgba8 if denoised else lib().mcpt_film_tonemap_rgba8
        self._ck(fn(self.h, exposure, out.ctypes.data_as(C.POINTER(C.c_uint8))))
        return out.reshape(self.H, self.W, 4)

    def render_guides(self, n=1):
        self._ck(lib().mcpt_guides_render(self.h, n))

    def guides(self) -> dict:
        P = self.W * self.H
        a, n = np.zeros(3 * P, np.float32), np.zeros(3 * P, np.float32)
        z, cnt = np.zeros(P, np.float32), np.zeros(P, np.uint32)
        self._ck(lib().mcpt_guides_read(self.h, fptr(a), fptr(n), fptr(z), cnt.ctypes.data_as(_u)))
        return {"albedo": a.reshape(self.H, self.W, 3), "normal": n.reshape(self.H, self.W, 3),
                "depth": z.reshape(self.H, self.W), "count": cnt.reshape(self.H, self.W)}

    def denoise(self, **params):
        p = denoise_params(**params) if params else None
        self._ck(lib().mcpt_film_denoise(self.h, C.byref(p) if p is not None else None))

    def denoised(self):
        out = np.zeros(3 * self.W * self.H, np.float32)
        self._ck(lib().mcpt_denoised_read(self.h, fptr(out)))
        return out.reshape(self.H, self.W, 3)

    def denoise_guided(self, **params):
        p = denoise_guided_params(**params) if params else None
        self._ck(lib().mcpt_film_denoise_guided(self.h, C.byref(p) if p is not None else None))

    def denoised_variance(self):
        out = np.zeros(self.W * self.H, np.float32)
        self._ck(lib().mcpt_denoised_variance_read(self.h, fptr(out)))
        return out.reshape(self.H, self.W)

    def write_denoised_png(self, path, exposure=1.0):
        self._ck(lib().mcpt_denoised_write_png(self.h, exposure, os.fsencode(path)))

    def denoise_ms(self) -> dict:
        v = (C.c_float * 10)()
        self._ck(lib().mcpt_debug_denoise_ms(self.h, v))
        return {"guides": float(v[0]), "prepare": float(v[1]), "passes": [float(x) for x in v[2:]]}

    def set_seed(self, seed):
        self._ck(lib().mcpt_set_seed(self.h, int(seed)))
        self.cfg.seed = int(seed)

    def temporal_accumulate(self, **params):
        p = temporal_params(**params) if params else None
        self._ck(lib().mcpt_film_temporal(self.h, C.byref(p) if p is not None else None))

    def temporal(self) -> dict:
        P = self.W * self.H
        rgb, pos = np.zeros(3 * P, np.float32), np.zeros(3 * P, np.float32)
        ns, var = np.zeros(P, np.float32), np.zeros(P, np.float32)
        self._ck(lib().mcpt_temporal_read(self.h, fptr(rgb), fptr(ns), fptr(var), fptr(pos)))
        return {"rgb": rgb.reshape(self.H, self.W, 3), "nsamples": ns.reshape(self.H, self.W),
                "variance": var.reshape(self.H, self.W), "position": pos.reshape(self.H, self.W, 3)}

    def temporal_denoise(self, **params):
        p = denoise_guided_params(**params) if params else None
        self._ck(lib().mcpt_temporal_denoise(self.h, C.byref(p) if p is not None else None))

    def temporal_reset(self):
        self._ck(lib().mcpt_temporal_reset(self.h))

    def temporal_bytes(self) -> int:
        return int(lib().mcpt_debug_temporal_bytes(self.h))
# ... 347 lines not shown
```

Baseline: 10830.

## Precompute complete occlusion-cache cells via beam traversal to resolve shadow rays

Adds a build-time pass that, for each occlusion-cache key (origin cell × direction bin), traverses the BVH with a conservative beam and lists every front-facing triangle the beam can reach. Keys whose list fits are marked 'done', which lets any-hit rays that fall in such a cell be resolved from the cached triangles without a full BVH trace. This targets the cost of any-hit traversal in the shade stage. In exchange it adds a per-key build kernel, a direction-bounds table, extra membership and decode work per ray, and entries can optionally widen to four ways.

Result: faster. 11170 (median of 6 runs) (+3.1%).

```diff
diff --git a/include/mcpt.h b/include/mcpt.h
--- a/include/mcpt.h
+++ b/include/mcpt.h
@@ -247,6 +247,7 @@
 } mcpt_bvh_info;
 int mcpt_debug_bvh_read(mcpt_ctx *ctx, float *nodes, float *tris, mcpt_bvh_info *info);
 int mcpt_debug_occ_stats(const mcpt_ctx *ctx, uint64_t *resolved, int32_t *enabled);
+int mcpt_debug_occ_complete_stats(const mcpt_ctx *ctx, double *out4);
 int mcpt_debug_ray_counts(const mcpt_ctx *ctx, uint64_t *out);
 int mcpt_debug_primary_stats(const mcpt_ctx *ctx, double *out4);
 int mcpt_debug_discard_stats(const mcpt_ctx *ctx, uint64_t *out4);
diff --git a/mc-path-tracer_amd/csrc/device/occ_beam.hpp b/mc-path-tracer_amd/csrc/device/occ_beam.hpp
--- /dev/null
+++ b/mc-path-tracer_amd/csrc/device/occ_beam.hpp
@@ -0,0 +1,169 @@
+#pragma once
+#include "primary_beam.hpp"
+
+namespace mcpt {
+
+constexpr uint32_t kOccDoneBit = 0x80000000u;
+constexpr uint32_t kOccDoneNone = 0x81000000u;
+constexpr uint32_t kOccDoneIndex = 0x01ffffffu;
+MCPT_HD bool occ_word_done(uint32_t w) { return (w >> 25) == 0x40u; }
+
+struct OccGrid {
+    float mn[3], cell[3];
+    int g, b;
+    const float4* dir;
+};
+constexpr int kOccDirF4 = 2;
+
+MCPT_HD void occ_dir_bin(int B, uint32_t face, uint32_t ub, uint32_t vb, float* out) {
+    const double hb = 0.5 * (double)B, s = 1e-5;
+    auto edge = [&](double e, double w) { return e == 0.0 ? 0.0 : e + w; };
+    const double a0 = edge(((double)ub - hb) / hb, -s), a1 = edge(((double)ub + 1.0 - hb) / hb, s);
+    const double b0 = edge(((double)vb - hb) / hb, -s), b1 = edge(((double)vb + 1.0 - hb) / hb, s);
+    const double a2lo = (a0 <= 0.0 && a1 >= 0.0) ? 0.0 : (a0 * a0 < a1 * a1 ? a0 * a0 : a1 * a1);
+    const double a2hi = a0 * a0 > a1 * a1 ? a0 * a0 : a1 * a1;
+    const double b2lo = (b0 <= 0.0 && b1 >= 0.0) ? 0.0 : (b0 * b0 < b1 * b1 ? b0 * b0 : b1 * b1);
+    const double b2hi = b0 * b0 > b1 * b1 ? b0 * b0 : b1 * b1;
+    const double mlo = (1.0 - 1e-4) / __builtin_sqrt(1.0 + a2hi + b2hi), mhi = (1.0 + 1e-4) / __builtin_sqrt(1.0 + a2lo + b2lo);
+    auto hull = [&](double r0, double r1, double& lo, double& hi) {
+        const double p[4] = {r0 * mlo, r0 * mhi, r1 * mlo, r1 * mhi};
+        lo = hi = p[0];
+        for (int k = 1; k < 4; k++) { lo = p[k] < lo ? p[k] : lo; hi = p[k] > hi ? p[k] : hi; }
+    };
+    double ulo, uhi, vlo, vhi;
+    hull(a0, a1, ulo, uhi);
+    hull(b0, b1, vlo, vhi);
+    const double jlo = (face & 1u) ? -mhi : mlo, jhi = (face & 1u) ? -mlo : mhi;
+    double lo[3], hi[3];
+    const int major = (int)(face >> 1), ua = major == 0 ? 1 : 0, va = major == 2 ? 1 : 2;
+    lo[major] = jlo; hi[major] = jhi;
+    lo[ua] = ulo; hi[ua] = uhi;
+    lo[va] = vlo; hi[va] = vhi;
+    for (int k = 0; k < 3; k++) { out[2 * k] = (float)lo[k]; out[2 * k + 1] = (float)hi[k]; }
+}
+inline void occ_dir_table(int B, float4* out) {
+    for (uint32_t f = 0; f < 6u; f++)
+        for (uint32_t u = 0; u < (uint32_t)B; u++)
+            for (uint32_t v = 0; v < (uint32_t)B; v++) {
+                float t[6];
+                occ_dir_bin(B, f, u, v, t);
+                float4* o = out + kOccDirF4 * ((f * B + u) * (size_t)B + v);
+                o[0] = float4{t[0], t[1], t[2], t[3]};
+                o[1] = float4{t[4], t[5], 0.f, 0.f};
+            }
+}
+
+MCPT_HD Iv occ_cell_iv(float mn, float cell, uint32_t c) { return iv_fix(mn + (float)c * cell, mn + (float)(c + 1u) * cell); }
+MCPT_HD Beam occ_key_beam(const OccGrid& g, uint32_t cx, uint32_t cy, uint32_t cz, uint32_t dirbin) {
+    const float4* t = g.dir + kOccDirF4 * (size_t)dirbin;
+    const float4 t0 = t[0], t1 = t[1];
+    Beam b;
+    b.o = Iv3{occ_cell_iv(g.mn[0], g.cell[0], cx), occ_cell_iv(g.mn[1], g.cell[1], cy), occ_cell_iv(g.mn[2], g.cell[2], cz)};
+    b.d = Iv3{iv_fix(t0.x, t0.y), iv_fix(t0.z, t0.w), iv_fix(t1.x, t1.y)};
+    b.ok = true;
+    return b;
+}
+MCPT_HD bool iv_in(Iv a, float v) { return a.lo <= v && v <= a.hi; }
+MCPT_HD bool beam_contains(const Beam& b, V3 o, V3 d) {
+    return iv_in(b.o.x, o.x) && iv_in(b.o.y, o.y) && iv_in(b.o.z, o.z) && iv_in(b.d.x, d.x) && iv_in(b.d.y, d.y) &&
+           iv_in(b.d.z, d.z);
+}
+MCPT_HD bool occ_member(const OccGrid& g, uint32_t cx, uint32_t cy, uint32_t cz, uint32_t dirbin, V3 o, V3 d) {
+    return beam_contains(occ_key_beam(g, cx, cy, cz, dirbin), o, d);
+}
+
+MCPT_HD void occ_inv_axis(Iv d, Iv& inv, bool& con) {
+    const float big = 3.4028235e38f;
+    inv = iv_all();
+    con = false;
+    if (d.lo >= 0.f && d.hi > 0.f) {
+        inv = iv_fix(__builtin_fminf(1.f / d.hi, big), d.lo > 0.f ? __builtin_fminf(1.f / d.lo, big) : big);
+        con = true;
+    } else if (d.hi <= 0.f && d.lo < 0.f) {
+        inv = iv_fix(d.hi < 0.f ? __builtin_fmaxf(1.f / d.hi, -big) : -big, __builtin_fmaxf(1.f / d.lo, -big));
+        con = true;
+    }
+}
+MCPT_HD BeamInv occ_beam_inv(const Beam& b) {
+    BeamInv r;
+    occ_inv_axis(b.d.x, r.x, r.cx);
+    occ_inv_axis(b.d.y, r.y, r.cy);
+    occ_inv_axis(b.d.z, r.z, r.cz);
+    return r;
+}
+
+MCPT_HD void beam_box_range(const Beam& b, const BeamInv& iv, float mnx, float mny, float mnz, float mxx, float mxy,
+                            float mxz, float& t0lo, float& t1hi) {
+    float t0 = -__builtin_huge_valf(), t1 = __builtin_huge_valf(), e, x;
+    if (iv.cx) { beam_slab_axis(mnx, mxx, b.o.x, iv.x, e, x); t0 = __builtin_fmaxf(t0, e); t1 = __builtin_fminf(t1, x); }
+    if (iv.cy) { beam_slab_axis(mny, mxy, b.o.y, iv.y, e, x); t0 = __builtin_fmaxf(t0, e); t1 = __builtin_fminf(t1, x); }
+    if (iv.cz) { beam_slab_axis(mnz, mxz, b.o.z, iv.z, e, x); t0 = __builtin_fmaxf(t0, e); t1 = __builtin_fminf(t1, x); }
+    t0lo = t0;
+    t1hi = t1;
+}
+MCPT_HD float beam_iota_hi(const BeamInv& iv, float cull_p) {
+    float m = __builtin_huge_valf();
+    if (iv.cx && iv.cy && iv.cz) {
+        const float ax = __builtin_fmaxf(__builtin_fabsf(iv.x.lo), __builtin_fabsf(iv.x.hi));
+        const float ay = __builtin_fmaxf(__builtin_fabsf(iv.y.lo), __builtin_fabsf(iv.y.hi));
+        const float az = __builtin_fmaxf(__builtin_fabsf(iv.z.lo), __builtin_fabsf(iv.z.hi));
+        m = __builtin_fmaxf(__builtin_fmaxf(ax, ay), az) * kCullSlackF;
+    }
+    if (cull_p > 0.f) m = __builtin_fminf(m, (1.f / cull_p) * 1.000001f);
+    return m;
+}
+MCPT_HD bool beam_behind_box(float t1hi, float w, float io_hi) {
+    const float m = w * io_hi;
+    return m >= 0.f && __builtin_fmaf(t1hi, kCullBehindF, m) < 0.f;
+}
+
+struct OccTree {
+    const float4* nodes;
+    const float4* tri;
+    int tri_f4;
+    uint32_t ntri;
+    int root_ref;
+    float root_mn[3], root_mx[3];
+    float root_w, cull_p;
+};
+constexpr int kOccListStack = 64;
+constexpr int kOccListBudget = 768;
+
+MCPT_HD int occ_key_list(const OccTree& t, const Beam& b, int ways, uint32_t* out) {
+    const BeamInv iv = occ_beam_inv(b);
+    const float io_hi = beam_iota_hi(iv, t.cull_p);
+    int stack[kOccListStack];
+    int sp = 0, n = 0, budget = kOccListBudget;
+    auto visit = [&](int ref, float mnx, float mny, float mnz, float mxx, float mxy, float mxz, float w) -> int {
+        if (ref == -1) return 0;
+        if (--budget < 0) return -1;
+        float t0lo, t1hi;
+        beam_box_range(b, iv, mnx, mny, mnz, mxx, mxy, mxz, t0lo, t1hi);
+        if (t0lo > t1hi || beam_behind_box(t1hi, w, io_hi)) return 0;
+        if (ref >= 0) {
+            if (sp >= kOccListStack) return -1;
+            stack[sp++] = ref;
+            return 1;
+        }
+        const uint32_t off = (uint32_t)ref & 0xffffffu, cnt = (((uint32_t)ref >> 24) & 7u) + 1u;
+        for (uint32_t k = off; k < off + cnt && k < t.ntri; k++) {
+            const float4* r = t.tri + (size_t)t.tri_f4 * k;
+            const float4 r0 = r[0], r1 = r[1], r2 = r[2];
+            if (beam_backfacing(b, v3(r0.w, r1.x, r1.y), v3(r1.z, r1.w, r2.x))) continue;
+            if (n >= ways) return -1;
+            out[n++] = k;
+        }
+        return 0;
+    };
+    if (visit(t.root_ref, t.root_mn[0], t.root_mn[1], t.root_mn[2], t.root_mx[0], t.root_mx[1], t.root_mx[2], t.root_w) < 0)
+        return -1;
+    while (sp > 0) {
+        const float4* nd = t.nodes + 4 * (size_t)stack[--sp];
+        const float4 q0 = nd[0], q1 = nd[1], q2 = nd[2], q3 = nd[3];
+        if (visit(__builtin_bit_cast(int, q3.x), q0.x, q1.x, q2.x, q0.z, q1.z, q2.z, q3.z) < 0) return -1;
+        if (visit(__builtin_bit_cast(int, q3.y), q0.y, q1.y, q2.y, q0.w, q1.w, q2.w, q3.w) < 0) return -1;
+    }
+    return n;
+}
+
+}
diff --git a/mc-path-tracer_amd/csrc/kernels.hip b/mc-path-tracer_amd/csrc/kernels.hip
--- a/mc-path-tracer_amd/csrc/kernels.hip
+++ b/mc-path-tracer_amd/csrc/kernels.hip
@@ -311,13 +311,13 @@
     t_out = t;
 }
 
-__device__ inline uint32_t occ_index(const DevScene& sc, V3 o, V3 d) {
+__device__ inline void occ_coords(const DevScene& sc, V3 o, V3 d, uint32_t& cx, uint32_t& cy, uint32_t& cz, uint32_t& face,
+                                  uint32_t& ub, uint32_t& vb) {
     const float gm = (float)(sc.occ_g - 1), bm = (float)(sc.occ_b - 1), hb = 0.5f * (float)sc.occ_b;
-    const uint32_t cx = (uint32_t)__builtin_fminf(__builtin_fmaxf((o.x - sc.root_mn[0]) * sc.occ_inv[0], 0.f), gm);
-    const uint32_t cy = (uint32_t)__builtin_fminf(__builtin_fmaxf((o.y - sc.root_mn[1]) * sc.occ_inv[1], 0.f), gm);
-    const uint32_t cz = (uint32_t)__builtin_fminf(__builtin_fmaxf((o.z - sc.root_mn[2]) * sc.occ_inv[2], 0.f), gm);
+    cx = (uint32_t)__builtin_fminf(__builtin_fmaxf((o.x - sc.root_mn[0]) * sc.occ_inv[0], 0.f), gm);
+    cy = (uint32_t)__builtin_fminf(__builtin_fmaxf((o.y - sc.root_mn[1]) * sc.occ_inv[1], 0.f), gm);
+    cz = (uint32_t)__builtin_fminf(__builtin_fmaxf((o.z - sc.root_mn[2]) * sc.occ_inv[2], 0.f), gm);
     const float ax = __builtin_fabsf(d.x), ay = __builtin_fabsf(d.y), az = __builtin_fabsf(d.z);
-    uint32_t face;
     float u, v, m;
     if (ax >= ay && ax >= az) {
         face = d.x < 0.f ? 1u : 0u; u = d.y; v = d.z; m = ax;
@@ -327,9 +327,14 @@
         face = d.z < 0.f ? 5u : 4u; u = d.x; v = d.y; m = az;
     }
     const float r = hb * __builtin_amdgcn_rcpf(m);
-    const uint32_t ub = (uint32_t)__builtin_fminf(__builtin_fmaxf(u * r + hb, 0.f), bm);
-    const uint32_t vb = (uint32_t)__builtin_fminf(__builtin_fmaxf(v * r + hb, 0.f), bm);
+    ub = (uint32_t)__builtin_fminf(__builtin_fmaxf(u * r + hb, 0.f), bm);
+    vb = (uint32_t)__builtin_fminf(__builtin_fmaxf(v * r + hb, 0.f), bm);
+}
+__device__ inline uint32_t occ_index(const DevScene& sc, V3 o, V3 d, uint32_t* packed = nullptr) {
+    uint32_t cx, cy, cz, face, ub, vb;
+    occ_coords(sc, o, d, cx, cy, cz, face, ub, vb);
     const uint32_t G = (uint32_t)sc.occ_g, B = (uint32_t)sc.occ_b;
+    if (packed) *packed = ((face * B + ub) * B + vb) | cx << 15 | cy << 20 | cz << 25;
 #if MCPT_OCC_LAYOUT == 1
     return (((face * B + ub) * B + vb) * G + cz) * G * G + cy * G + cx;
 #else
@@ -351,28 +356,55 @@
     return tri_test_t(o, d, v3(bmx.w, r2.x, r2.y), v3(r2.z, r2.w, r3.x), v3(r3.y, r3.z, r3.w), th) && !(th < 0.f) &&
            th < K_HUGE;
 }
-__device__ inline uint2 occ_entry(const DevScene& sc, uint32_t cell) {
-    const uint2* e = reinterpret_cast<const uint2*>(sc.occ) + cell;
-    if constexpr (MCPT_NT & 16) {
-        typedef uint32_t u2v_t __attribute__((ext_vector_type(2)));
-        const u2v_t v = __builtin_nontemporal_load(reinterpret_cast<const u2v_t*>(e));
-        return make_uint2(v.x, v.y);
-    } else {
-        return *e;
-    }
-}
-__device__ inline bool occ_hit1(const DevScene& sc, V3 o, V3 d, uint2 e) {
-    const bool v0 = e.x < sc.ntri, v1 = e.y < sc.ntri;
-    if (!(v0 || v1)) return false;
-    const float4* p0 = sc.occ_rec + kOccRecF4 * (size_t)(v0 ? e.x : 0u);
-    const float4* p1 = sc.occ_rec + kOccRecF4 * (size_t)(v1 ? e.y : 0u);
-    const float4 bn0 = p0[0], bx0 = p0[1], r20 = p0[2], r30 = p0[3];
-    const float4 bn1 = p1[0], bx1 = p1[1], r21 = p1[2], r31 = p1[3];
+struct OccEnt { uint32_t w[kOccWays]; };
+__device__ inline OccEnt occ_entry(const DevScene& sc, uint32_t cell) {
+    typedef uint32_t uwv_t __attribute__((ext_vector_type(kOccWays)));
+    const uwv_t* e = reinterpret_cast<const uwv_t*>(sc.occ) + cell;
+    uwv_t v;
+    if constexpr (MCPT_NT & 16) v = __builtin_nontemporal_load(e);
+    else v = *e;
+    OccEnt r;
+#pragma unroll
+    for (uint32_t k = 0; k < kOccWays; k++) r.w[k] = v[k];
+    return r;
+}
+enum : int { kOccOpen = 0, kOccHit = 1, kOccMaybe = 2 };
+__device__ inline int occ_hit1(const DevScene& sc, V3 o, V3 d, OccEnt e, bool& done) {
+    done = sc.occ_dir != nullptr;
+    bool any = false;
+#pragma unroll
+    for (uint32_t k = 0; k < kOccWays; k++) done = done && mcpt::occ_word_done(e.w[k]);
+#pragma unroll
+    for (uint32_t k = 0; k < kOccWays; k++) {
+        if (done) e.w[k] &= mcpt::kOccDoneIndex;
+        any = any || e.w[k] < sc.ntri;
+    }
+    if (!(any || done)) return kOccOpen;
     const V3 inv = v3(1.f / d.x, 1.f / d.y, 1.f / d.z);
-    if (!(__builtin_fabsf(inv.x) < K_INF_F && __builtin_fabsf(inv.y) < K_INF_F && __builtin_fabsf(inv.z) < K_INF_F))
-        return false;
+    const bool fin = __builtin_fabsf(inv.x) < K_INF_F && __builtin_fabsf(inv.y) < K_INF_F && __builtin_fabsf(inv.z) < K_INF_F;
     const float io = cull_iota(sc, d, inv);
-    return (v0 && occ_test(o, d, inv, io, bn0, bx0, r20, r30)) || (v1 && occ_test(o, d, inv, io, bn1, bx1, r21, r31));
+#pragma unroll
+    for (uint32_t k = 0; k < kOccWays; k += 2) {
+        const bool v0 = e.w[k] < sc.ntri, v1 = e.w[k + 1] < sc.ntri;
+        if (kOccWays > 2 && !(v0 || v1)) continue;
+        const float4* p0 = sc.occ_rec + kOccRecF4 * (size_t)(v0 ? e.w[k] : 0u);
+        const float4* p1 = sc.occ_rec + kOccRecF4 * (size_t)(v1 ? e.w[k + 1] : 0u);
+        const float4 bn0 = p0[0], bx0 = p0[1], r20 = p0[2], r30 = p0[3];
+        const float4 bn1 = p1[0], bx1 = p1[1], r21 = p1[2], r31 = p1[3];
+        if (!fin) return kOccOpen;
+        if ((v0 && occ_test(o, d, inv, io, bn0, bx0, r20, r30)) || (v1 && occ_test(o, d, inv, io, bn1, bx1, r21, r31)))
+            return kOccHit;
+    }
+    return done && fin && io > 0.f ? kOccMaybe : kOccOpen;
+}
+__device__ inline void occ_member2(const DevScene& sc, V3 ol, V3 dl, uint32_t kl, V3 ob, V3 db, uint32_t kb, bool& m_l,
+                                   bool& m_b) {
+    const mcpt::OccGrid g{{sc.root_mn[0], sc.root_mn[1], sc.root_mn[2]}, {sc.occ_cell[0], sc.occ_cell[1], sc.occ_cell[2]},
+                          sc.occ_g, sc.occ_b, sc.occ_dir};
+    const mcpt::Beam bl = mcpt::occ_key_beam(g, (kl >> 15) & 31u, (kl >> 20) & 31u, kl >> 25, kl & 0x7fffu);
+    const mcpt::Beam bb = mcpt::occ_key_beam(g, (kb >> 15) & 31u, (kb >> 20) & 31u, kb >> 25, kb & 0x7fffu);
+    m_l = mcpt::beam_contains(bl, ol, dl);
+    m_b = mcpt::beam_contains(bb, ob, db);
 }
 
 struct MatOut {
@@ -380,7 +412,8 @@
     bool skip_ext;
     bool doomed_inplace;
     uint32_t trivial_any;
-    uint2 el, eb;
+    OccEnt el, eb;
+    uint32_t kl, kb;
     V3 n, wo, wi_b;
     int matid, light_id;
     uint32_t flags;
@@ -391,9 +424,9 @@
 __device__ inline MatOut material(const ShadeArgs& a, uint32_t pid, uint32_t pix, uint32_t sidx, uint32_t len,
                                  V3 beta_store, int32_t htri, float4* stage, bool occ_on, bool no_cont) {
     const DevScene& sc = a.scene;
-    const uint2 none = make_uint2(kOccEmpty, kOccEmpty);
     MatOut mo{};
-    mo.el = mo.eb = none;
+#pragma unroll
+    for (uint32_t k = 0; k < kOccWays; k++) mo.el.w[k] = mo.eb.w[k] = kOccEmpty;
     MCPT_MARK("m_hit");
     const Rng r{rng_key(a.seed, pix, sidx), len};
     const V3 ro = xyz(ld_s(a.p.ray_o + pid)), rdir = xyz(ld_s(a.p.ray_d + pid));
@@ -481,7 +514,7 @@
             stage[0 * kBlock + threadIdx.x] = f4(so_l, __uint_as_float(2 * pid));
             stage[1 * kBlock + threadIdx.x] = f4(ldir, 0.f);
             mo.want_l = true;
-            if (occ_on) mo.el = occ_entry(sc, occ_index(sc, so_l, ldir));
+            if (occ_on) mo.el = occ_entry(sc, occ_index(sc, so_l, ldir, &mo.kl));
         }
     }
     MCPT_MARK("m_bsdir");
@@ -496,7 +529,7 @@
             a.p.vis[2 * pid + 1] = 1;
             mo.trivial_any++;
         } else {
-            if (occ_on) mo.eb = occ_entry(sc, occ_index(sc, so_b, wi_b));
+            if (occ_on) mo.eb = occ_entry(sc, occ_index(sc, so_b, wi_b, &mo.kb));
             stage[2 * kBlock + threadIdx.x] = f4(so_b, __uint_as_float(2 * pid + 1));
             stage[3 * kBlock + threadIdx.x] = f4(wi_b, 0.f);
             mo.want_b = true;
@@ -833,7 +866,7 @@
     uint32_t* sc_ctr = a.cnt->shard[shard];
     const uint32_t n = sc_ctr[C_MAT];
     const int lane = threadIdx.x & 63;
-    uint32_t n_ext = 0, n_any = 0, n_vis = 0, n_occ = 0, occ_try = 0, n_skip = 0, n_inpl = 0;
+    uint32_t n_ext = 0, n_any = 0, n_vis = 0, n_occ = 0, occ_try = 0, n_skip = 0, n_inpl = 0, n_dvis = 0, n_docc = 0;
     const bool occ_on = a.scene.occ && a.scene.occ_gate[0] == 0 && a.scene.occ_gate[2] != 0;
     __shared__ float4 s_any[4][kBlock];
     for (uint32_t base = w_in * kBlock; base < n; base += bps * kBlock) {
@@ -842,6 +875,7 @@
         MatOut mo{};
         uint32_t mpid = 0;
         bool occ_l = false, occ_b = false, try_l = false, try_b = false;
+        bool done_l = false, done_b = false, clr_l = false, clr_b = false;
         if (i < n) {
             const uint4 q = ld_s(a.mat_rec + shard * a.ext_cap + i);
             const float4 b4 = ld_s(a.mat_beta + shard * a.ext_cap + i);
@@ -854,8 +888,32 @@
                 try_b = mo.want_b;
                 const V3 ol = xyz(s_any[0][threadIdx.x]), dl = xyz(s_any[1][threadIdx.x]);
                 const V3 ob = xyz(s_any[2][threadIdx.x]), db = xyz(s_any[3][threadIdx.x]);
-                if (mo.want_l) occ_l = occ_hit1(a.scene, ol, dl, mo.el);
-                if (mo.want_b) occ_b = occ_hit1(a.scene, ob, db, mo.eb);
+                if (mo.want_l) {
+                    const int r = occ_hit1(a.scene, ol, dl, mo.el, done_l);
+                    occ_l = r == kOccHit;
+                    clr_l = r == kOccMaybe;
+                }
+                if (mo.want_b) {
+                    const int r = occ_hit1(a.scene, ob, db, mo.eb, done_b);
+                    occ_b = r == kOccHit;
+                    clr_b = r == kOccMaybe;
+                }
+                if (clr_l || clr_b) {
+                    bool m_l, m_b;
+                    occ_member2(a.scene, ol, dl, mo.kl, ob, db, mo.kb, m_l, m_b);
+                    clr_l = clr_l && m_l;
+                    clr_b = clr_b && m_b;
+                }
+                if (clr_l) {
+                    a.p.vis[2 * mpid] = 1;
+                    mo.want_l = false;
+                    mo.trivial_any++;
+                }
+                if (clr_b) {
+                    a.p.vis[2 * mpid + 1] = 1;
+                    mo.want_b = false;
+                    mo.trivial_any++;
+                }
                 if (occ_l) {
                     a.p.vis[2 * mpid] = 0;
                     mo.want_l = false;
@@ -900,6 +958,8 @@
         MCPT_MARK("m_count");
         n_occ += (uint32_t)(__popcll(__ballot(occ_l)) + __popcll(__ballot(occ_b)));
         occ_try += (uint32_t)(__popcll(__ballot(try_l)) + __popcll(__ballot(try_b)));
+        n_dvis += (uint32_t)(__popcll(__ballot(clr_l)) + __popcll(__ballot(clr_b)));
+        n_docc += (uint32_t)(__popcll(__ballot(occ_l && done_l)) + __popcll(__ballot(occ_b && done_b)));
         n_ext += (uint32_t)__popcll(__ballot(mo.want_ext || mo.trivial_ext || mo.skip_ext));
         n_skip += (uint32_t)__popcll(__ballot(mo.skip_ext));
         n_inpl += (uint32_t)__popcll(__ballot(mo.doomed_inplace));
@@ -913,6 +973,8 @@
         if (n_vis) atomicAdd(sc_ctr + C_VIS, n_vis);
         if (n_occ) atomicAdd(sc_ctr + C_OCC, n_occ);
         if (occ_try) atomicAdd(sc_ctr + C_OCC_TRY, occ_try);
+        if (n_dvis) atomicAdd(sc_ctr + C_OCC_DONE_VIS, n_dvis);
+        if (n_docc) atomicAdd(sc_ctr + C_OCC_DONE_OCC, n_docc);
         if (n_skip) atomicAdd(sc_ctr + C_SKIP_EXT, n_skip);
         if (n_inpl) atomicAdd(sc_ctr + C_SKIP_INPLACE, n_inpl);
     }
@@ -1748,7 +1810,8 @@
         for (int off = 32; off > 0; off >>= 1) phw[k] += __shfl_xor(phw[k], off);
     }
     uint32_t er = c->shard[t][C_EXT_RAYS], ar = c->shard[t][C_ANY_RAYS], oc = c->shard[t][C_OCC],
-             ot = c->shard[t][C_OCC_TRY], pr = c->shard[t][C_PRIM_RAYS];
+             ot = c->shard[t][C_OCC_TRY], pr = c->shard[t][C_PRIM_RAYS], dv = c->shard[t][C_OCC_DONE_VIS],
+             dc = c->shard[t][C_OCC_DONE_OCC];
     const int skw[4] = {C_SKIP_EXT, C_SKIP_ANY, C_SKIP_MAT, C_SKIP_INPLACE};
     uint32_t sk[4];
 #pragma unroll
@@ -1764,7 +1827,11 @@
     c->shard[t][C_MAT] = 0;
     c->shard[t][C_OCC] = 0;
     c->shard[t][C_OCC_TRY] = 0;
+    if (dv) c->shard[t][C_OCC_DONE_VIS] = 0;
+    if (dc) c->shard[t][C_OCC_DONE_OCC] = 0;
     for (int off = 32; off > 0; off >>= 1) {
+        dv += __shfl_xor(dv, off);
+        dc += __shfl_xor(dc, off);
         er += __shfl_xor(er, off);
         ar += __shfl_xor(ar, off);
         oc += __shfl_xor(oc, off);
@@ -1777,13 +1844,15 @@
         for (int k = 0; k < 4; k++) c->tot_skip[k] += sk[k];
         c->tot_any += ar;
         c->tot_occ += oc;
+        c->tot_done[0] += dv;
+        c->tot_done[1] += dc;
         if (occ_gate) {
             if (occ_gate[0]) {
                 occ_gate[0]--;
             } else if (!occ_gate[2]) {
                 if (v[C_ANY]) occ_gate[2] = 1;
             } else if (ot >= 4096u) {
-                if ((unsigned long long)oc * kOccMinRate < ot) {
+                if (((unsigned long long)oc + dv) * kOccMinRate < ot) {
                     occ_gate[1] = occ_gate[1] ? min(2u * occ_gate[1] + 1u, 255u) : (uint32_t)MCPT_OCC_BACKOFF0;
                     occ_gate[0] = occ_gate[1];
                 } else {
@@ -2065,6 +2134,35 @@
     ro[key] = make_float4(o[0], o[1], o[2], 0.f);
     rd[key] = make_float4(d[0] * inv_n, d[1] * inv_n, d[2] * inv_n, 0.f);
 }
+__global__ void k_occ_complete(DevScene sc, mcpt::OccTree tree, uint32_t nkeys, uint32_t* ndone) {
+    const uint32_t key = blockIdx.x * blockDim.x + threadIdx.x;
+    bool done = false;
+    if (key < nkeys) {
+        const uint32_t G = (uint32_t)sc.occ_g, B = (uint32_t)sc.occ_b;
+        uint32_t t = key, cx, cy, cz, face, ub, vb;
+#if MCPT_OCC_LAYOUT == 1
+        cx = t % G; t /= G; cy = t % G; t /= G; cz = t % G; t /= G; vb = t % B; t /= B; ub = t % B; face = t / B;
+#else
+        vb = t % B; t /= B; ub = t % B; t /= B; face = t % 6u; t /= 6u; cx = t % G; t /= G; cy = t % G; cz = t / G;
+#endif
+        const mcpt::OccGrid g{{sc.root_mn[0], sc.root_mn[1], sc.root_mn[2]}, {sc.occ_cell[0], sc.occ_cell[1], sc.occ_cell[2]},
+                              sc.occ_g, sc.occ_b, sc.occ_dir};
+        const mcpt::Beam b = mcpt::occ_key_beam(g, cx, cy, cz, (face * B + ub) * B + vb);
+        uint32_t list[kOccWays];
+        const int n = mcpt::occ_key_list(tree, b, (int)kOccWays, list);
+        if (n >= 0) {
+            done = true;
+            for (uint32_t w = 0; w < kOccWays; w++)
+                sc.occ[(size_t)key * kOccWays + w] = (int)w < n ? (mcpt::kOccDoneBit | list[w]) : mcpt::kOccDoneNone;
+        }
+    }
+    const uint32_t cnt = (uint32_t)__popcll(__ballot(done));
+    if ((threadIdx.x & 63) == 0 && cnt) atomicAdd(ndone, cnt);
+}
+void launch_occ_complete(const DevScene& sc, const mcpt::OccTree& tree, uint32_t nkeys, uint32_t* ndone, hipStream_t s) {
+    if (nkeys == 0) return;
+    hipLaunchKernelGGL(k_occ_complete, dim3((nkeys + 255) / 256), dim3(256), 0, s, sc, tree, nkeys, ndone);
+}
 void launch_occ_probes(const DevScene& sc, float4* ro, float4* rd, uint32_t nkeys, hipStream_t s) {
     if (nkeys == 0) return;
     hipLaunchKernelGGL(k_occ_probes, dim3((nkeys + 255) / 256), dim3(256), 0, s, sc, ro, rd, nkeys);
diff --git a/mc-path-tracer_amd/csrc/kernels.hpp b/mc-path-tracer_amd/csrc/kernels.hpp
--- a/mc-path-tracer_amd/csrc/kernels.hpp
+++ b/mc-path-tracer_amd/csrc/kernels.hpp
@@ -5,6 +5,7 @@
 #include "device/adaptive.hpp"
 #include "device/denoise.hpp"
 #include "device/mcpt_core.hpp"
+#include "device/occ_beam.hpp"
 #include "device/temporal.hpp"
 #include "device/variance.hpp"
 
@@ -69,11 +70,18 @@
     uint32_t ntri;
     int occ_g, occ_b;
     float occ_inv[3];
+    const float4* occ_dir;
+    float occ_cell[3];
     float cull_p, root_w;
     int cull_ok;
 };
+constexpr char kOccCompleteEnv[] = "MCPT_OCC_COMPLETE";
 constexpr uint32_t kOccEmpty = 0xffffffffu;
-constexpr uint32_t kOccWays = 2;
+#ifndef MCPT_OCC_WAYS
+#define MCPT_OCC_WAYS 2
+#endif
+constexpr uint32_t kOccWays = MCPT_OCC_WAYS;
+static_assert(kOccWays == 2 || kOccWays == 4, "an entry is one 8-B or 16-B load");
 constexpr uint32_t kOccGateWords = 3;
 constexpr uint32_t kOccMinRate = 10;
 __host__ __device__ constexpr size_t occ_entries(int g, int b) { return (size_t)g * g * g * 6 * b * b * kOccWays; }
@@ -89,7 +97,7 @@
 constexpr int kMaxParts = kShards;
 enum : int { C_EXT = 0, C_ANY = 1, C_VIS = 2, C_STATS = 3, C_EXT_RAYS = 9, C_ANY_RAYS = 10, C_MAT = 11, C_OCC = 12,
               C_OCC_TRY = 13, C_PH = 14, C_SKIP_INPLACE = 25, C_PRIM = 26, C_PRIM_RAYS = 27, C_SKIP_EXT = 28,
-              C_SKIP_ANY = 29, C_SKIP_MAT = 30, C_WORDS = 32 };
+              C_SKIP_ANY = 29, C_SKIP_MAT = 30, C_OCC_DONE_VIS = 31, C_OCC_DONE_OCC = 32, C_WORDS = 64 };
 enum : int {
     PH_TRIPS = 0,
     PH_REFILLS = 1,
@@ -118,6 +126,7 @@
     unsigned long long tot_phase[kPhaseWords];
     unsigned long long tot_prim;
     unsigned long long tot_skip[4];
+    unsigned long long tot_done[2];
 };
 static_assert(C_PH + kPhaseWords <= C_SKIP_INPLACE, "counter words overlap");
 
@@ -220,6 +229,7 @@
 constexpr int kOccRecF4 = 4;
 void launch_occ_records(const DevScene& sc, uint32_t nnodes, float4* rec, hipStream_t s);
 void launch_occ_probes(const DevScene& sc, float4* ro, float4* rd, uint32_t nkeys, hipStream_t s);
+void launch_occ_complete(const DevScene& sc, const mcpt::OccTree& tree, uint32_t nkeys, uint32_t* ndone, hipStream_t s);
 void launch_cull_margins(float4* nodes, uint32_t npairs, const float4* tri, uint32_t ntri, float* tri_w,
                          uint32_t* pmax, int passes, bool plane, hipStream_t s);
 void launch_env_pack(float4* tex, const float* pdf, size_t n, hipStream_t s);
diff --git a/mc-path-tracer_amd/csrc/runtime.cpp b/mc-path-tracer_amd/csrc/runtime.cpp
--- a/mc-path-tracer_amd/csrc/runtime.cpp
+++ b/mc-path-tracer_amd/csrc/runtime.cpp
@@ -574,6 +574,10 @@
     s.ntri = (uint32_t)d->ntri;
     s.occ = nullptr;
     s.occ_rec = nullptr;
+    s.occ_dir = nullptr;
+    for (int k = 0; k < 3; k++) s.occ_cell[k] = 0.f;
+    c->occ_done_keys = 0;
+    c->occ_done_ms = 0.f;
     {
         int G = 24, B = 12;
         if (const char* e = getenv("MCPT_OCC_G")) G = atoi(e);
@@ -612,6 +616,15 @@
             for (int k = 0; k < 3; k++) {
                 const float ext = s.root_mx[k] - s.root_mn[k];
                 s.occ_inv[k] = ext > 0.f && ext < 3.4e38f ? (float)G / ext : 0.f;
+                s.occ_cell[k] = s.occ_inv[k] > 0.f ? ext / (float)G : 0.f;
+            }
+            const char* ce = getenv(kOccCompleteEnv);
+            if (!(ce && ce[0] == '0' && ce[1] == 0) && cull_ok && G <= 32 && s.occ_cell[0] > 0.f && s.occ_cell[1] > 0.f && s.occ_cell[2] > 0.f) {
+                std::vector<float4> dirs((size_t)6 * B * B * mcpt::kOccDirF4);
+                mcpt::occ_dir_table(B, dirs.data());
+                float4* dd2;
+                if ((rc = dupload(c, c->scene_bufs, &dd2, dirs.data(), dirs.size()))) return rc;
+                s.occ_dir = dd2;
             }
         }
     }
@@ -622,13 +635,15 @@
     c->occ_init = nullptr;
     if (s.occ) {
         const char* pe = getenv("MCPT_OCC_PREFILL");
-        if (!(pe && pe[0] == '0' && pe[1] == 0)) {
-            const uint32_t nkeys = (uint32_t)(c->occ_entries_n / kOccWays);
+        const bool prefill = !(pe && pe[0] == '0' && pe[1] == 0), complete = s.occ_dir != nullptr;
+        const uint32_t nkeys = (uint32_t)(c->occ_entries_n / kOccWays);
+        if ((prefill || complete) && (rc = dalloc(c, c->scene_bufs, &c->occ_init, c->occ_entries_n))) return rc;
+        if (prefill) {
             float4 *pro, *prd;
             uint8_t* pvis;
             free_list(c->tmp_bufs);
             if ((rc = dalloc(c, c->tmp_bufs, &pro, nkeys)) || (rc = dalloc(c, c->tmp_bufs, &prd, nkeys)) ||
-                (rc = dalloc(c, c->tmp_bufs, &pvis, nkeys)) || (rc = dalloc(c, c->scene_bufs, &c->occ_init, c->occ_entries_n)))
+                (rc = dalloc(c, c->tmp_bufs, &pvis, nkeys)))
                 return rc;
             launch_occ_probes(s, pro, prd, nkeys, c->stream);
             TraceArgs ta{};
@@ -643,6 +658,33 @@
             ta.grab = &c->cnt->grab[0][0];
             launch_trace(ta, c->geom, c->stream);
             HIPCHK(c, hipMemsetAsync(c->cnt->grab, 0, sizeof(c->cnt->grab), c->stream));
+            HIPCHK(c, hipGetLastError());
+        }
+        if (complete) {
+            mcpt::OccTree tr{};
+            tr.nodes = c->pair_nodes;
+            tr.tri = s.tri;
+            tr.tri_f4 = kTriF4;
+            tr.ntri = s.ntri;
+            tr.root_ref = c->pair_root;
+            for (int k = 0; k < 3; k++) { tr.root_mn[k] = s.root_mn[k]; tr.root_mx[k] = s.root_mx[k]; }
+            tr.root_w = s.root_w;
+            tr.cull_p = s.cull_p;
+            uint32_t* dn;
+            if ((rc = dalloc(c, c->tmp_bufs, &dn, 1))) return rc;
+            HIPCHK(c, hipMemsetAsync(dn, 0, sizeof(uint32_t), c->stream));
+            HIPCHK(c, hipEventRecord(ev(c, 0), c->stream));
+            launch_occ_complete(s, tr, nkeys, dn, c->stream);
+            HIPCHK(c, hipGetLastError());
+            HIPCHK(c, hipEventRecord(ev(c, 1), c->stream));
+            uint32_t nd = 0;
+            HIPCHK(c, hipMemcpyAsync(&nd, dn, sizeof(nd), hipMemcpyDeviceToHost, c->stream));
+            HIPCHK(c, hipEventSynchronize(c->events[1]));
+            HIPCHK(c, hipStreamSynchronize(c->stream));
+            HIPCHK(c, hipEventElapsedTime(&c->occ_done_ms, c->events[0], c->events[1]));
+            c->occ_done_keys = nd;
+        }
+        if (prefill || complete) {
             HIPCHK(c, hipMemcpyAsync(c->occ_init, s.occ, c->occ_entries_n * sizeof(uint32_t), hipMemcpyDeviceToDevice,
                                      c->stream));
             const uint32_t warm[kOccGateWords] = {0u, 0u, 1u};
@@ -729,6 +771,14 @@
 int mcpt_debug_discard_stats(const mcpt_ctx* c, uint64_t* out4) {
     if (!c || !out4) return MCPT_E_INVALID;
     for (int k = 0; k < 4; k++) out4[k] = c->totals_ok ? c->totals.tot_skip[k] : 0;
+    return MCPT_OK;
+}
+int mcpt_debug_occ_complete_stats(const mcpt_ctx* c, double* out4) {
+    if (!c || !out4) return MCPT_E_INVALID;
+    out4[0] = (double)c->occ_done_keys;
+    out4[1] = c->totals_ok ? (double)c->totals.tot_done[0] : 0.0;
+    out4[2] = c->totals_ok ? (double)c->totals.tot_done[1] : 0.0;
+    out4[3] = (double)c->occ_done_ms;
     return MCPT_OK;
 }
 int mcpt_debug_occ_stats(const mcpt_ctx* c, uint64_t* resolved, int32_t* enabled) {
diff --git a/mc-path-tracer_amd/csrc/runtime_internal.hpp b/mc-path-tracer_amd/csrc/runtime_internal.hpp
--- a/mc-path-tracer_amd/csrc/runtime_internal.hpp
+++ b/mc-path-tracer_amd/csrc/runtime_internal.hpp
@@ -152,6 +152,8 @@
     int32_t ntri = 0;
     size_t occ_entries_n = 0;
     uint32_t* occ_init = nullptr;
+    uint64_t occ_done_keys = 0;
+    float occ_done_ms = 0.f;
     int pair_depth = 0;
     bool cull_ok = true, occ_nest_ok = true;
     bool count_work = getenv("MCPT_WORK_COUNTERS") != nullptr;
diff --git a/mc-path-tracer_amd/mcpt/__init__.py b/mc-path-tracer_amd/mcpt/__init__.py
--- a/mc-path-tracer_amd/mcpt/__init__.py
+++ b/mc-path-tracer_amd/mcpt/__init__.py
@@ -195,6 +195,7 @@
     "mcpt_debug_node_layout": (C.c_int, [C.c_void_p]),
     "mcpt_debug_bvh_read": (C.c_int, [C.c_void_p, _f, _f, C.POINTER(BvhInfo)]),
     "mcpt_debug_occ_stats": (C.c_int, [C.c_void_p, C.POINTER(C.c_uint64), C.POINTER(C.c_int32)]),
+    "mcpt_debug_occ_complete_stats": (C.c_int, [C.c_void_p, C.POINTER(C.c_double)]),
     "mcpt_debug_ray_counts": (C.c_int, [C.c_void_p, C.POINTER(C.c_uint64)]),
     "mcpt_debug_primary_stats": (C.c_int, [C.c_void_p, C.POINTER(C.c_double)]),
     "mcpt_set_work_counters": (C.c_int, [C.c_void_p, C.c_int32]),
@@ -487,6 +488,12 @@
         self._ck(lib().mcpt_debug_occ_stats(self.h, C.byref(r), C.byref(e)))
         return int(r.value), bool(e.value)
 
+    def occ_complete_stats(self) -> dict:
+        v = (C.c_double * 4)()
+        if hasattr(lib(), "mcpt_debug_occ_complete_stats") or not os.environ.get("MCPT_LIB"):
+            self._ck(lib().mcpt_debug_occ_complete_stats(self.h, v))
+        return dict(keys=int(v[0]), unoccluded=int(v[1]), occluded=int(v[2]), build_ms=float(v[3]))
+
     @property
     def last_build_ms(self) -> float:
         return lib().mcpt_debug_last_build_ms(self.h)
```
